# srvk/eesen

Measured on AMD Instinct MI355X. Metric: CTC training frames/sec (whole node), 4x512 BiLSTM, higher is better.
Workload: dtype f32

## Files before the change

eesen_amd/_lib.py:

```python
from __future__ import annotations

import ctypes as C
import os

_DIR = os.path.dirname(os.path.abspath(__file__))
LIB_PATH = os.environ.get("EESEN_HIP_LIBRARY") or os.path.join(_DIR, "lib", "libeesen_hip.so")

OK = 0
LAYER_AFFINE, LAYER_SOFTMAX, LAYER_LSTM_PARALLEL, LAYER_BILSTM_PARALLEL, LAYER_SIGMOID, LAYER_TANH = 1, 2, 3, 4, 5, 6
KIND_OF = {"AffineTransform": LAYER_AFFINE, "Softmax": LAYER_SOFTMAX, "LstmParallel": LAYER_LSTM_PARALLEL,
           "BiLstmParallel": LAYER_BILSTM_PARALLEL, "Lstm": LAYER_LSTM_PARALLEL, "BiLstm": LAYER_BILSTM_PARALLEL,
           "Sigmoid": LAYER_SIGMOID, "Tanh": LAYER_TANH}
NAME_OF = {LAYER_AFFINE: "AffineTransform", LAYER_SOFTMAX: "Softmax", LAYER_LSTM_PARALLEL: "LstmParallel",
           LAYER_BILSTM_PARALLEL: "BiLstmParallel", LAYER_SIGMOID: "Sigmoid", LAYER_TANH: "Tanh"}

_vp, _i, _f, _l = C.c_void_p, C.c_int, C.c_float, C.c_long
_pi, _pf, _pl, _pd = C.POINTER(C.c_int), C.POINTER(C.c_float), C.POINTER(C.c_long), C.POINTER(C.c_double)
SIGNATURES = {
    "eesen_last_error": (C.c_char_p, []),
    "eesen_version": (C.c_char_p, []),
    "eesen_device_count": (_i, [_pi]),
    "eesen_net_create": (_i, [_i, _vp, C.POINTER(_vp)]),
    "eesen_net_destroy": (_i, [_vp]),
    "eesen_net_add_layer": (_i, [_vp, _i, _i, _i, _f, _f]),
    "eesen_net_finalize": (_i, [_vp]),
    "eesen_net_read": (_i, [_vp, C.c_char_p]),
    "eesen_net_write": (_i, [_vp, C.c_char_p, _i]),
    "eesen_net_num_layers": (_i, [_vp, _pi]),
    "eesen_net_layer_info": (_i, [_vp, _i, _pi, _pi, _pi, _pf, _pf]),
    "eesen_net_input_dim": (_i, [_vp, _pi]),
    "eesen_net_output_dim": (_i, [_vp, _pi]),
    "eesen_net_num_params": (_i, [_vp, _pl]),
    "eesen_net_get_params": (_i, [_vp, _vp, _l]),
    "eesen_net_set_params": (_i, [_vp, _vp, _l]),
    "eesen_net_set_train_options": (_i, [_vp, _f, _f]),
    "eesen_net_set_update_algorithm": (_i, [_vp, C.c_char_p]),
    "eesen_net_set_adaptive_options": (_i, [_vp, _f, _f]),
    "eesen_net_get_accumulators": (_i, [_vp, _vp, _l]),
    "eesen_net_set_accumulators": (_i, [_vp, _vp, _l]),
    "eesen_net_set_seq_lengths": (_i, [_vp, _vp, _i]),
    "eesen_net_propagate": (_i, [_vp, _vp, _i, _i, _i, C.POINTER(_vp), _pi, _pi]),
    "eesen_net_get_output": (_i, [_vp, _vp, _l]),
    "eesen_net_backpropagate": (_i, [_vp, _vp, _i, _vp, _i]),
    "eesen_net_grad_buffer": (_i, [_vp, C.POINTER(_vp), _pl]),
    "eesen_net_get_grads": (_i, [_vp, _vp, _l]),
    "eesen_net_update": (_i, [_vp]),
    "eesen_net_set_forward_precision": (_i, [_vp, _i]),
    "eesen_net_bf16_recurrence_layers": (_i, [_vp, _vp]),
    "eesen_net_recurrence_info": (_i, [_vp, _pi]),
    "eesen_net_debug_set_error_word": (_i, [_vp, C.c_uint]),
    "eesen_net_synchronize": (_i, [_vp]),
    "eesen_net_set_profiling": (_i, [_vp, _i]),
    "eesen_net_get_phase_times": (_i, [_vp, _vp]),
    "eesen_net_get_phase_spans": (_i, [_vp, _pi, _pf, _i, _pi]),
    "eesen_device_synchronize": (_i, [_i]),
    "eesen_set_gemm_mode": (_i, [_i]),
    "eesen_get_gemm_mode": (_i, [_pi]),
    "eesen_comm_get_unique_id": (_i, [_vp]),
    "eesen_comm_exchange": (_i, [C.c_char_p, _i, _i, _i, _vp, _i, _i]),
    "eesen_comm_create": (_i, [_i, _vp, _i, _i, C.POINTER(_vp)]),
    "eesen_comm_create_tcp": (_i, [_i, C.c_char_p, _i, _i, _i, _i, C.POINTER(_vp)]),
    "eesen_comm_destroy": (_i, [_vp]),
    "eesen_comm_info": (_i, [_vp, _pi, _pi]),
    "eesen_comm_describe": (_i, [_vp, C.c_char_p, _i]),
    "eesen_net_plan_string": (_i, [_vp, C.c_char_p, _i]),
    "eesen_comm_allreduce_host": (_i, [_vp, _pd, _i, _i]),
    "eesen_net_set_comm": (_i, [_vp, _vp]),
    "eesen_net_allreduce_grads": (_i, [_vp, _vp]),
    "eesen_net_backpropagate_zero": (_i, [_vp]),
    "eesen_net_bucket_order": (_i, [_vp, _pi, _i, _pi]),
    "eesen_net_live_ranks": (_i, [_vp, _pi]),
    "eesen_net_layer_marker": (_i, [_vp, _i, C.c_char_p, _i]),
    "eesen_net_tensor_moments": (_i, [_vp, _i, _i, _pd, _i, _pi]),
    "eesen_ctc_set_guard": (_i, [_vp, _vp]),
    "eesen_ctc_dropped": (_i, [_vp, _pl]),
    "eesen_ctc_create": (_i, [_i, _vp, C.POINTER(_vp)]),
    "eesen_ctc_destroy": (_i, [_vp]),
    "eesen_ctc_eval_parallel": (_i, [_vp, _vp, _i, _vp, _i, _i, _i, _vp, _vp, _vp, _i, _vp]),
    "eesen_ctc_error_rate_mseq": (_i, [_vp, _vp, _i, _vp, _i, _i, _i, _vp, _vp, _pi, _pi]),
    "eesen_ctc_stats": (_i, [_vp, _pd, _pl, _pl, _pl, _pl]),
    "eesen_ctc_get_alpha_beta": (_i, [_vp, _vp, _vp, _pi]),
    "eesen_ctc_set_profiling": (_i, [_vp, _i]),
    "eesen_ctc_set_sequence_out_file": (_i, [_vp, C.c_char_p]),
    "eesen_ctc_get_phase_times": (_i, [_vp, _vp]),
    "eesen_ce_create": (_i, [_i, _vp, C.POINTER(_vp)]),
    "eesen_ce_destroy": (_i, [_vp]),
    "eesen_ce_eval_parallel": (_i, [_vp, _vp, _i, _vp, _i, _i, _i, _vp, _vp, _i, _vp]),
    "eesen_ce_set_report_step": (_i, [_vp, _i]),
    "eesen_ce_stats": (_i, [_vp, _pd, _pl, _pl, _pl]),
    "eesen_ce_report": (_i, [_vp, C.c_char_p, _i]),
    "eesen_ce_progress": (_i, [_vp, _i, C.c_char_p, _i]),
    "eesen_ce_set_guard": (_i, [_vp, _vp]),
    "eesen_ce_dropped": (_i, [_vp, _pl]),
    "eesen_ce_set_profiling": (_i, [_vp, _i]),
    "eesen_ce_get_phase_times": (_i, [_vp, _vp]),
    "eesen_net_set_train_mode": (_i, [_vp, _i]),
    "eesen_net_set_dropout_seed": (_i, [_vp, C.c_ulonglong]),
    "eesen_net_set_layer_dropout": (_i, [_vp, _i, _pf]),
    "eesen_net_get_layer_dropout": (_i, [_vp, _i, _pf]),
    "eesen_net_set_dropout_masks": (_i, [_vp, _i, _vp, _l, _vp, _i, _l, _i]),
    "eesen_net_get_dropout_masks": (_i, [_vp, _i, _vp, _vp, _pi]),
    "eesen_feeder_create": (_i, [_i, _vp, _i, C.POINTER(_vp)]),
    "eesen_feeder_destroy": (_i, [_vp]),
    "eesen_feeder_submit": (_i, [_vp, C.POINTER(_vp), _pi, _pi, _i, _i, _pi]),
    "eesen_feeder_acquire": (_i, [_vp, _i, C.POINTER(_vp), _pi, _pi, _pi]),
    "eesen_feeder_release": (_i, [_vp, _i]),
    "eesen_feeder_set_pipeline": (_i, [_vp, _vp, _i]),
    "eesen_feeder_pipeline_shape": (_i, [_vp, _i, _i, _pi, _pi]),
    "eesen_feeder_submit_raw": (_i, [_vp, C.POINTER(_vp), _pi, _pi, C.POINTER(_vp), _i, _i, _pi]),
    "eesen_cmvn_norm": (_i, [_pd, _i, _i, _i, _pf]),
    "eesen_dev_alloc": (_i, [_i, _l, C.POINTER(_vp)]),
    "eesen_dev_free": (_i, [_i, _vp]),
    "eesen_dev_copy": (_i, [_i, _vp, _vp, _l, _i]),
    "eesen_op_log_sub_prior": (_i, [_i, _vp, _vp, _i, _i, _i, _i, _vp, _f]),
    "eesen_op_amax_rows_cols": (_i, [_i, _vp, C.c_long, _i, _i, _vp, _vp]),
    "eesen_op_gemm_bench": (_i, [_i, _i, _i, _i, _i, _i, _vp, _i, _vp, _i, _vp, _i, _i, _pf]),
    "eesen_op_gemm": (_i, [_i, _vp, _i, _i, _i, _i, _i, _f, _vp, _i, _vp, _i, _f, _vp, _i, _vp]),
    "eesen_op_gemm_async": (_i, [_i, _vp, _i, _i, _i, _i, _i, _vp, _i, _vp, _i, _vp, _i, _vp, C.c_long, _i]),
}


class EesenError(RuntimeError):

    def __init__(self, code: int, msg: str):
        super().__init__(f"[{code}] {msg}")
        self.code = code


_lib = None


def load() -> C.CDLL:
    global _lib
    if _lib is None:
        if not os.path.exists(LIB_PATH):
            raise EesenError(-2, f"{LIB_PATH} is missing: build it with `python -m eesen_amd.build` "
                                 "(there is no CPU fallback for the HIP path)")
        os.environ.setdefault("HSA_ENABLE_IPC_MODE_LEGACY", "0")
        lib = C.CDLL(LIB_PATH)
        for name, (res, args) in SIGNATURES.items():
            fn = getattr(lib, name)
            fn.restype, fn.argtypes = res, args
        _lib = lib
    return _lib


def check(rc: int):
    if rc != OK:
        raise EesenError(rc, load().eesen_last_error().decode(errors="replace"))


def device_count() -> int:
    n = C.c_int(0)
    check(load().eesen_device_count(C.byref(n)))
    return n.value
```

eesen_amd/csrc/capi.cpp:

```cpp
#include <cstdio>
#include <cstring>

#include <algorithm>

#include "guard.h"
#include "net.h"

using namespace eesen;

#include "handles.h"

namespace eesen {
std::string& last_error_slot() {
  thread_local std::string g_err;
  return g_err;
}
}

extern "C" {

const char* eesen_last_error(void) { return last_error_slot().c_str(); }
const char* eesen_version(void) { return "eesen_hip 0.1.0 (gfx950)"; }

int eesen_device_count(int* count) {
// ... 291 lines not shown
    REQ_PTR(ce);
    ce->flush();
    if (obj) *obj = ce->obj;
    if (correct) *correct = ce->correct;
    if (frames) *frames = ce->frames;
    if (sequences) *sequences = ce->sequences;
  });
}
int eesen_ce_report(eesen_ce_t* ce, char* buf, int cap) {
  return guard([&] {
    REQ_PTR(ce); REQ_PTR(buf);
    const std::string s = ce->report();
    EESEN_REQUIRE(cap > (int)s.size(), EESEN_ERR_INVALID, "eesen_ce_report: buffer too small (" + std::to_string(s.size() + 1) + " bytes needed)");
    std::memcpy(buf, s.c_str(), s.size() + 1);
  });
}
int eesen_ce_progress(eesen_ce_t* ce, int wait, char* buf, int cap) {
  return guard([&] {
    REQ_PTR(ce); REQ_PTR(buf);
    EESEN_REQUIRE(cap > 0, EESEN_ERR_INVALID, "eesen_ce_progress: no buffer");
    if (wait) ce->flush();
    if (ce->progress.empty()) { buf[0] = 0; return; }
    const std::string& s = ce->progress.front();
    EESEN_REQUIRE(cap > (int)s.size(), EESEN_ERR_INVALID, "eesen_ce_progress: buffer too small (" + std::to_string(s.size() + 1) + " bytes needed)");
    std::memcpy(buf, s.c_str(), s.size() + 1);
    ce->progress.erase(ce->progress.begin());
  });
}
int eesen_ce_set_guard(eesen_ce_t* ce, eesen_net_t* net) {
  return guard([&] {
    REQ_PTR(ce);
    ce->flush();
    if (net) EESEN_REQUIRE(net->device == ce->device && net->st == ce->st, EESEN_ERR_INVALID, "eesen_ce_set_guard: the CE and the Net must live on the same device and stream");
    if (ce->guard_net) {
      auto& g = ce->guard_net->ce_guards;
      g.erase(std::remove(g.begin(), g.end(), static_cast<CeLoss*>(ce)), g.end());
    }
    ce->guard = net && net->ctl.p ? net->ctl.p + kCtlWords - 1 : nullptr;
    ce->guard_net = ce->guard ? net : nullptr;
    if (ce->guard_net) net->ce_guards.push_back(ce);
  });
}
int eesen_ce_dropped(eesen_ce_t* ce, long* minibatches) {
  return guard([&] { REQ_PTR(ce); REQ_PTR(minibatches); ce->flush(); *minibatches = ce->dropped; });
}
int eesen_ce_set_profiling(eesen_ce_t* ce, int mode) {
  return guard([&] { REQ_PTR(ce); ce->timer.enable(mode == 2); ce->timer.set_accumulate(mode == 2); });
}
int eesen_ce_get_phase_times(eesen_ce_t* ce, float* out1) {
  return guard([&] { REQ_PTR(ce); REQ_PTR(out1); ce->phase_times(out1); });
}

int eesen_dev_alloc(int device, long bytes, void** dev_ptr) {
  return guard([&] {
    REQ_PTR(dev_ptr);
    EESEN_HIP_CHECK(hipSetDevice(device));
    EESEN_HIP_CHECK(hipMalloc(dev_ptr, (size_t)bytes));
  });
}
int eesen_dev_free(int device, void* dev_ptr) {
  return guard([&] {
    EESEN_HIP_CHECK(hipSetDevice(device));
    EESEN_HIP_CHECK(hipFree(dev_ptr));
  });
}
int eesen_dev_copy(int device, void* dst, const void* src, long bytes, int kind) {
  return guard([&] {
    EESEN_HIP_CHECK(hipSetDevice(device));
    const hipMemcpyKind k = kind == 1 ? hipMemcpyHostToDevice : kind == 2 ? hipMemcpyDeviceToHost : hipMemcpyDeviceToDevice;
    EESEN_HIP_CHECK(hipMemcpy(dst, src, (size_t)bytes, k));
  });
}

int eesen_op_gemm(int device, void* stream, int a_kc, int b_kc, int M, int N, int K, float alpha, const float* A, int lda,
                  const float* B, int ldb, float beta, float* C, int ldc, const float* bias) {
  return guard([&] {
    EESEN_HIP_CHECK(hipSetDevice(device));
    hipStream_t st = reinterpret_cast<hipStream_t>(stream);
    DevBuf<float> ws;
    ws.reserve((size_t)8 << 20);
    gemm_f32(st, a_kc != 0, b_kc != 0, M, N, K, alpha, A, lda, B, ldb, beta, C, ldc, bias, ws.p, ws.cap);
    EESEN_HIP_CHECK(hipStreamSynchronize(st));
  });
}

int eesen_op_gemm_async(int device, void* stream, int a_kc, int b_kc, int M, int N, int K, const float* A, int lda, const float* B, int ldb,
                        float* C, int ldc, float* ws, long ws_floats, int extra_lds_bytes) {
  return guard([&] {
    REQ_PTR(A); REQ_PTR(B); REQ_PTR(C);
    EESEN_REQUIRE(ws_floats >= 0 && (ws || ws_floats == 0) && extra_lds_bytes >= 0, EESEN_ERR_INVALID, "bad workspace / LDS cap");
    EESEN_HIP_CHECK(hipSetDevice(device));
    gemm_f32(reinterpret_cast<hipStream_t>(stream), a_kc != 0, b_kc != 0, M, N, K, 1.f, A, lda, B, ldb, 0.f, C, ldc, nullptr, ws, (size_t)ws_floats,
             extra_lds_bytes);
  });
}

int eesen_op_log_sub_prior(int device, void* stream, float* m_dev, int rows, int cols, int ld, int apply_log,
                           const float* log_priors_host, float prior_scale) {
  return guard([&] {
    REQ_PTR(m_dev);
    EESEN_HIP_CHECK(hipSetDevice(device));
    hipStream_t st = reinterpret_cast<hipStream_t>(stream);
    DevBuf<float> pri;
    if (log_priors_host) {
      pri.reserve(cols);
      EESEN_HIP_CHECK(hipMemcpyAsync(pri.p, log_priors_host, sizeof(float) * cols, hipMemcpyHostToDevice, st));
    }
    log_sub_prior(st, m_dev, ld, rows, cols, apply_log != 0, log_priors_host ? pri.p : nullptr, prior_scale);
    EESEN_HIP_CHECK(hipStreamSynchronize(st));
  });
}

int eesen_op_gemm_bench(int device, int a_kc, int b_kc, int M, int N, int K, const float* A, int lda, const float* B, int ldb,
                        float* C, int ldc, int iters, float* avg_ms) {
  return guard([&] {
    REQ_PTR(avg_ms);
    EESEN_HIP_CHECK(hipSetDevice(device));
    DevBuf<float> ws;
    ws.reserve((size_t)16 << 20);
    hipEvent_t e0, e1;
    EESEN_HIP_CHECK(hipEventCreate(&e0));
    EESEN_HIP_CHECK(hipEventCreate(&e1));
    DevBuf<float> am;
    am.reserve((size_t)M + N + (size_t)kAmaxBlocks * 16384);
    GemmBound ba{am.p, 1}, bb{am.p + M, 1};
    float* aws = am.p + M + N;
    if (a_kc) amax_rows_cols(nullptr, A, M, K, lda, am.p, nullptr, nullptr); else amax_rows_cols(nullptr, A, K, M, lda, nullptr, am.p, aws);
    if (b_kc) amax_rows_cols(nullptr, B, N, K, ldb, am.p + M, nullptr, nullptr); else amax_rows_cols(nullptr, B, K, N, ldb, nullptr, am.p + M, aws);
    for (int i = 0; i < 2; ++i) gemm_f32(nullptr, a_kc != 0, b_kc != 0, M, N, K, 1.f, A, lda, B, ldb, 0.f, C, ldc, nullptr, ws.p, ws.cap, 0, false, ba, bb);
    EESEN_HIP_CHECK(hipEventRecord(e0, nullptr));
    for (int i = 0; i < iters; ++i) gemm_f32(nullptr, a_kc != 0, b_kc != 0, M, N, K, 1.f, A, lda, B, ldb, 0.f, C, ldc, nullptr, ws.p, ws.cap, 0, false, ba, bb);
    EESEN_HIP_CHECK(hipEventRecord(e1, nullptr));
    EESEN_HIP_CHECK(hipEventSynchronize(e1));
    float ms = 0.f;
    EESEN_HIP_CHECK(hipEventElapsedTime(&ms, e0, e1));
    *avg_ms = ms / iters;
    (void)hipEventDestroy(e0);
    (void)hipEventDestroy(e1);
  });
}

int eesen_op_amax_rows_cols(int device, const float* m_dev, long rows, int cols, int ld, float* out_rows_dev, float* out_cols_dev) {
  return guard([&] {
    REQ_PTR(m_dev);
    EESEN_REQUIRE(rows > 0 && cols > 0 && ld >= cols, EESEN_ERR_INVALID, "bad matrix shape");
    EESEN_HIP_CHECK(hipSetDevice(device));
    DevBuf<float> ws;
    if (out_cols_dev) ws.reserve((size_t)kAmaxBlocks * 16384);
    amax_rows_cols(nullptr, m_dev, rows, cols, ld, out_rows_dev, out_cols_dev, ws.p);
    EESEN_HIP_CHECK(hipStreamSynchronize(nullptr));
  });
}

}
```

eesen_amd/csrc/gemm.hip:

```cpp
#include <cstring>
#include <mutex>
#include <type_traits>

#include "kernels.h"

namespace eesen {
namespace {

constexpr int BM = 128, BN = 128, BK = 16, LDP = 4;
constexpr int NLD = BM * BK / 4 / 256;
constexpr int KQ_BITS = BK == 16 ? 2 : 3;
typedef float f32x16 __attribute__((ext_vector_type(16)));

struct GemmParams {
  const float* A;
  const float* B;
  float* C;
  const float* bias;
  int M, N, K;
  int lda, ldb, ldc;
  float alpha, beta;
  int splits;
  int k_chunk;
  int tiles_n;
// ... 615 lines not shown
    const long gw = (long)blockIdx.x * kAmaxWaves + wave, nw = (long)gridDim.x * kAmaxWaves;
    const int slab = (int)(gw % nslab);
    const int c0 = slab * 1024 + lane * 4;
    uint4 cm[4];
#pragma unroll
    for (int j = 0; j < 4; ++j) cm[j] = make_uint4(0u, 0u, 0u, 0u);
    const long rstep = nw / nslab;
    for (long r = gw / nslab; r < R; r += 2 * rstep) {
      const bool two = r + rstep < R;
      const float* row0 = P + r * ld;
      const float* row1 = P + (two ? r + rstep : r) * ld;
      uint4 v[8];
#pragma unroll
      for (int j = 0; j < 4; ++j) {
        const int c = c0 + 256 * j;
        v[j] = c < C ? *reinterpret_cast<const uint4*>(row0 + c) : make_uint4(0u, 0u, 0u, 0u);
        v[4 + j] = c < C ? *reinterpret_cast<const uint4*>(row1 + c) : make_uint4(0u, 0u, 0u, 0u);
      }
      unsigned m0 = 0u, m1 = 0u;
#pragma unroll
      for (int j = 0; j < 8; ++j) {
        v[j].x &= 0x7fffffffu; v[j].y &= 0x7fffffffu; v[j].z &= 0x7fffffffu; v[j].w &= 0x7fffffffu;
        const unsigned mj = max(max(v[j].x, v[j].y), max(v[j].z, v[j].w));
        if (j < 4) m0 = max(m0, mj); else m1 = max(m1, mj);
        if (COLS) { uint4& q = cm[j & 3]; q.x = max(q.x, v[j].x); q.y = max(q.y, v[j].y); q.z = max(q.z, v[j].z); q.w = max(q.w, v[j].w); }
      }
      if (ROWS || ALL) {
#pragma unroll
        for (int o = 32; o > 0; o >>= 1) { m0 = max(m0, (unsigned)__shfl_xor((int)m0, o)); m1 = max(m1, (unsigned)__shfl_xor((int)m1, o)); }
        if (ROWS && lane == 0) {
          if (nslab > 1 || row_acc) { atomicMax(&out_rows[r], m0); if (two) atomicMax(&out_rows[r + rstep], m1); }
          else { out_rows[r] = m0; if (two) out_rows[r + rstep] = m1; }
        }
        all = max(all, max(m0, m1));
      }
    }
    if (COLS) {
#pragma unroll
      for (int j = 0; j < 4; ++j) {
        const int c = c0 + 256 * j;
        if (c < C) { atomicMax(&smax[c], cm[j].x); atomicMax(&smax[c + 1], cm[j].y); atomicMax(&smax[c + 2], cm[j].z); atomicMax(&smax[c + 3], cm[j].w); }
      }
    }
  } else {
    for (long r = (long)blockIdx.x * kAmaxWaves + wave; r < R; r += (long)gridDim.x * kAmaxWaves) {
      const float* row = P + r * ld;
      unsigned m = 0u;
      for (int c = lane; c < C; c += 64) {
        const unsigned v = __builtin_bit_cast(unsigned, row[c]) & 0x7fffffffu;
        m = max(m, v);
        if (COLS) atomicMax(&smax[c], v);
      }
      if (ROWS || ALL) {
#pragma unroll
        for (int o = 32; o > 0; o >>= 1) m = max(m, (unsigned)__shfl_xor((int)m, o));
        if (ROWS && lane == 0) { if (row_acc) atomicMax(&out_rows[r], m); else out_rows[r] = m; }
        all = max(all, m);
      }
    }
  }
  if (COLS) {
    __syncthreads();
    for (int c = tid; c < Cp; c += kAmaxWaves * 64) part_cols[(size_t)blockIdx.x * Cp + c] = smax[c];
  }
  if (ALL) {
    unsigned* red = smax + (COLS ? Cp : 0);
    __syncthreads();
    if (lane == 0) red[wave] = all;
    __syncthreads();
    if (tid == 0) {
      unsigned m = 0u;
      for (int w = 0; w < kAmaxWaves; ++w) m = max(m, red[w]);
      if (m) atomicMax(out_all, m);
    }
  }
}
__global__ __launch_bounds__(256) void amax_fold_kernel(const unsigned* __restrict__ part, int nb, int Cp, int C, unsigned* __restrict__ out) {
  __shared__ uint4 red[16][16];
  const int cq = threadIdx.x & 15, g = threadIdx.x >> 4;
  const int c = blockIdx.x * 64 + cq * 4;
  uint4 m = make_uint4(0u, 0u, 0u, 0u);
  if (c < Cp)
    for (int b = g; b < nb; b += 16 * 8) {
      uint4 v[8];
#pragma unroll
      for (int k = 0; k < 8; ++k) v[k] = b + 16 * k < nb ? *reinterpret_cast<const uint4*>(part + (size_t)(b + 16 * k) * Cp + c) : make_uint4(0u, 0u, 0u, 0u);
#pragma unroll
      for (int k = 0; k < 8; ++k) { m.x = max(m.x, v[k].x); m.y = max(m.y, v[k].y); m.z = max(m.z, v[k].z); m.w = max(m.w, v[k].w); }
    }
  red[g][cq] = m;
  __syncthreads();
  if (g == 0 && c < Cp) {
#pragma unroll
    for (int k = 1; k < 16; ++k) { const uint4 o = red[k][cq]; m.x = max(m.x, o.x); m.y = max(m.y, o.y); m.z = max(m.z, o.z); m.w = max(m.w, o.w); }
    if (c + 0 < C) out[c + 0] = m.x;
    if (c + 1 < C) out[c + 1] = m.y;
    if (c + 2 < C) out[c + 2] = m.z;
    if (c + 3 < C) out[c + 3] = m.w;
  }
}

__global__ __launch_bounds__(256) void splitk_reduce_kernel(const float* __restrict__ ws, int splits, int M, int N,
                                                            float alpha, float beta, float* __restrict__ C, int ldc,
                                                            const float* __restrict__ bias) {
  const size_t total = (size_t)M * N;
  for (size_t i = (size_t)blockIdx.x * blockDim.x + threadIdx.x; i < total; i += (size_t)gridDim.x * blockDim.x) {
    float s = 0.f;
    for (int k = 0; k < splits; ++k) s += ws[(size_t)k * total + i];
    const int row = (int)(i / N), col = (int)(i % N);
    float v = alpha * s + (bias ? bias[col] : 0.f);
    float* dst = C + (size_t)row * ldc + col;
    if (beta != 0.f) v += beta * *dst;
    *dst = v;
  }
}

}

static int g_gemm_mode = -1;
int gemm_mode() {
  if (g_gemm_mode >= 0) return g_gemm_mode;
  const char* e = getenv("EESEN_GEMM_MODE");
  if (e && (!strcmp(e, "f32") || !strcmp(e, "0"))) return 0;
  if (e && (!strcmp(e, "split") || !strcmp(e, "1"))) return 1;
  if (e && (!strcmp(e, "half") || !strcmp(e, "2"))) return 2;
  return kDefaultGemmMode;
}
void set_gemm_mode(int mode) { g_gemm_mode = mode; }

void amax_abs(hipStream_t st, const float* P, long rows, int cols, int ld, float* out) {
  EESEN_HIP_CHECK(hipMemsetAsync(out, 0, sizeof(float), st));
  amax_abs_accumulate(st, P, rows, cols, ld, out);
}
static int amax_blocks(long rows, int slabs) { return (int)std::max<long>(1, std::min<long>((rows * slabs + 2 * kAmaxWaves - 1) / (2 * kAmaxWaves), kAmaxBlocks)); }
#define EESEN_AMAX_LAUNCH(R_, C_, A_, LDS)                                                                                                        \
  do {                                                                                                                                            \
    if (vec) hipLaunchKernelGGL((amax_kernel<R_, C_, A_, true>), dim3(nb), dim3(kAmaxWaves * 64), LDS, st, Pc, rows, cc, ld, r, w, a, racc);     \
    else hipLaunchKernelGGL((amax_kernel<R_, C_, A_, false>), dim3(nb), dim3(kAmaxWaves * 64), LDS, st, Pc, rows, cc, ld, r, w, a, racc);        \
  } while (0)
constexpr int kAmaxSlabCols = 16384;
void amax_abs_accumulate(hipStream_t st, const float* P, long rows, int cols, int ld, float* out) {
  if (rows <= 0 || cols <= 0) return;
  if (cols == ld && cols < 1024 && (rows * cols) % 1024 == 0) { rows = rows * cols / 1024; cols = ld = 1024; }
  unsigned *r = nullptr, *w = nullptr, *a = reinterpret_cast<unsigned*>(out);
  const int racc = 0;
  const bool vec = (cols & 3) == 0 && (ld & 3) == 0;
  for (int c0 = 0; c0 < cols; c0 += kAmaxSlabCols) {
    const float* Pc = P + c0;
    const int cc = std::min(kAmaxSlabCols, cols - c0), nb = amax_blocks(rows, vec ? (cc + 1023) / 1024 : 1);
    EESEN_AMAX_LAUNCH(false, false, true, kAmaxWaves * sizeof(unsigned));
  }
  check_launch("amax_abs");
}
void amax_rows_cols(hipStream_t st, const float* P, long rows, int cols, int ld, float* out_rows, float* out_cols, float* ws) {
  if (rows <= 0 || cols <= 0) return;
  EESEN_REQUIRE(!out_cols || ws, EESEN_ERR_INVALID, "amax: column bounds need a workspace");
  unsigned* r = reinterpret_cast<unsigned*>(out_rows);
  unsigned* w = reinterpret_cast<unsigned*>(ws);
  unsigned* a = nullptr;
  const bool vec = (cols & 3) == 0 && (ld & 3) == 0;
  const bool multi = out_rows && ((vec && cols > 1024) || cols > kAmaxSlabCols);
  if (multi) EESEN_HIP_CHECK(hipMemsetAsync(out_rows, 0, (size_t)rows * sizeof(float), st));
  for (int c0 = 0; c0 < cols; c0 += kAmaxSlabCols) {
    const float* Pc = P + c0;
    const int cc = std::min(kAmaxSlabCols, cols - c0), racc = multi ? 1 : 0;
    const int nb = amax_blocks(rows, vec ? (cc + 1023) / 1024 : 1);
    const int cp = (cc + 3) & ~3;
    if (out_rows && out_cols) EESEN_AMAX_LAUNCH(true, true, false, (size_t)cp * sizeof(unsigned));
    else if (out_cols) EESEN_AMAX_LAUNCH(false, true, false, (size_t)cp * sizeof(unsigned));
    else if (out_rows) EESEN_AMAX_LAUNCH(true, false, false, 0);
    check_launch("amax_rows_cols");
    if (out_cols) {
      hipLaunchKernelGGL(amax_fold_kernel, dim3((cp + 63) / 64), dim3(256), 0, st, w, nb, cp, cc, reinterpret_cast<unsigned*>(out_cols) + c0);
      check_launch("amax_fold");
    }
  }
}
#undef EESEN_AMAX_LAUNCH

static GemmBound arena_bound(hipStream_t st, const float* P, bool kc, int R, int K, int ld) {
  constexpr size_t kArena = (size_t)4 << 20, kDevs = 16;
  static std::mutex mu;
  static float* arena[kDevs] = {nullptr};
  static size_t next[kDevs] = {0};
  int dev = 0;
  EESEN_HIP_CHECK(hipGetDevice(&dev));
  EESEN_REQUIRE(dev >= 0 && dev < (int)kDevs, EESEN_ERR_INVALID, "gemm: device index beyond the bounds arena table");
  const size_t need = ((size_t)R + 3) & ~(size_t)3;
  EESEN_REQUIRE(need <= kArena / 8, EESEN_ERR_INVALID, "gemm: operand too large for the bounds arena");
  float* slot;
  {
    std::lock_guard<std::mutex> lk(mu);
    if (!arena[dev]) EESEN_HIP_CHECK(hipMalloc(reinterpret_cast<void**>(&arena[dev]), kArena * sizeof(float)));
    if (next[dev] + need > kArena) next[dev] = 0;
    slot = arena[dev] + next[dev];
    next[dev] += need;
  }
  if (kc) amax_rows_cols(st, P, R, K, ld, slot, nullptr, nullptr);
  else {
    float* ws = nullptr;
    EESEN_HIP_CHECK(hipMallocAsync(reinterpret_cast<void**>(&ws), (size_t)kAmaxBlocks * std::min<size_t>(need, kAmaxSlabCols) * sizeof(float), st));
    amax_rows_cols(st, P, K, R, ld, nullptr, slot, ws);
    EESEN_HIP_CHECK(hipFreeAsync(ws, st));
  }
  return GemmBound{slot, 1};
}

static int xcd_group_rows(int tiles_m, int tiles_n, unsigned* grid_x) {
  if (tiles_m < 8) return 0;
  int gm = 8;
  while (gm > 1 && cdiv(tiles_m, gm) < 16) gm >>= 1;
  const long groups = cdiv(tiles_m, gm), rounds = cdivl(groups, 8);
  const long gx = rounds * 8 * gm * tiles_n;
  if (gx > 0x7fffffffL) return 0;
  *grid_x = (unsigned)gx;
  return gm;
}

void gemm_f32(hipStream_t st, bool a_kc, bool b_kc, int M, int N, int K, float alpha, const float* A, int lda,
              const float* B, int ldb, float beta, float* C, int ldc, const float* bias, float* ws, size_t ws_floats,
              int extra_lds_bytes, bool bf16_operands, GemmBound bound_a, GemmBound bound_b) {
  if (M <= 0 || N <= 0) return;
  EESEN_REQUIRE((lda % 4) == 0 && (ldb % 4) == 0, EESEN_ERR_INVALID, "gemm: leading dimensions must be multiples of 4");
  EESEN_REQUIRE((((uintptr_t)A | (uintptr_t)B) & 15) == 0, EESEN_ERR_INVALID, "gemm: operands must be 16-byte aligned");
  const bool use_split = gemm_mode() >= 1 || bf16_operands;
  const bool half = gemm_mode() == 2 && !bf16_operands;
  GemmParams p;
  p.amax_a = p.amax_b = nullptr;
  p.a_vec = p.b_vec = 0;
  if (half) {
    if (!bound_a.p) bound_a = arena_bound(st, A, a_kc, M, K, lda);
    if (!bound_b.p) bound_b = arena_bound(st, B, b_kc, N, K, ldb);
    p.amax_a = bound_a.p; p.a_vec = bound_a.per_index;
    p.amax_b = bound_b.p; p.b_vec = bound_b.per_index;
  }
  p.A = A; p.B = B; p.C = C; p.bias = bias;
  p.M = M; p.N = N; p.K = K; p.lda = lda; p.ldb = ldb; p.ldc = ldc;
  p.alpha = alpha; p.beta = beta;
  p.gate = GemmGate{nullptr, nullptr, 0, 0, 0, 0, 0, 0};
  p.nprod = bf16_operands ? 1 : 6;
  const bool big = use_split && !bf16_operands && extra_lds_bytes == 0 && M % 256 == 0 && N % 256 == 0 && K % 16 == 0 &&
                   (long)(M / 256) * (N / 256) >= 16;
  const int TB = big ? 256 : BM;
  p.bm = p.bn = TB;
  const int tiles_m = cdiv(M, TB), tiles_n = cdiv(N, TB);
  p.tiles_n = tiles_n;
  p.tiles_m = tiles_m;
  const long tiles = (long)tiles_m * tiles_n;
  int splits = 1;
  const int target = big ? 256 : 1024;
  if (ws && tiles < target && K >= 2048) {
    splits = (int)std::min<long>((target + tiles - 1) / tiles, K / 1024);
    splits = std::max(1, std::min(splits, 64));
    while (splits > 1 && (size_t)splits * M * N > ws_floats) --splits;
  }
  int k_chunk = cdiv(cdiv(K, splits), 16) * 16;
  if (k_chunk < BK) k_chunk = BK;
  splits = std::max(1, cdiv(K, k_chunk));
  p.splits = splits;
  p.k_chunk = k_chunk;
  if (splits > 1) p.C = ws;
  unsigned gx = 0;
  p.gm = xcd_group_rows(tiles_m, tiles_n, &gx);
  dim3 grid(p.gm ? gx : (unsigned)tiles, (unsigned)splits), block(big ? 512 : 256);
  const bool guard = (M % BM) != 0 || (N % BN) != 0 || (K % k_chunk) != 0 || (k_chunk % BK) != 0 || !(a_kc && b_kc);
#define EESEN_GEMM_LAUNCH(AK, BKC)                                                                        \
  do {                                                                                                    \
    if (guard) hipLaunchKernelGGL((gemm_f32_mfma_kernel<AK, BKC, true>), grid, block, extra_lds_bytes, st, p); \
    else hipLaunchKernelGGL((gemm_f32_mfma_kernel<AK, BKC, false>), grid, block, extra_lds_bytes, st, p);     \
  } while (0)
  if (big && half) {
    if (a_kc && b_kc) hipLaunchKernelGGL((gemm_f32_split_f16_big_kernel<true, true>), grid, block, 0, st, p);
    else if (a_kc && !b_kc) hipLaunchKernelGGL((gemm_f32_split_f16_big_kernel<true, false>), grid, block, 0, st, p);
    else if (!a_kc && b_kc) hipLaunchKernelGGL((gemm_f32_split_f16_big_kernel<false, true>), grid, block, 0, st, p);
    else hipLaunchKernelGGL((gemm_f32_split_f16_big_kernel<false, false>), grid, block, 0, st, p);
  } else if (big) {
    if (a_kc && b_kc) hipLaunchKernelGGL((gemm_f32_split_bf16_big_kernel<true, true>), grid, block, 0, st, p);
    else if (a_kc && !b_kc) hipLaunchKernelGGL((gemm_f32_split_bf16_big_kernel<true, false>), grid, block, 0, st, p);
    else if (!a_kc && b_kc) hipLaunchKernelGGL((gemm_f32_split_bf16_big_kernel<false, true>), grid, block, 0, st, p);
    else hipLaunchKernelGGL((gemm_f32_split_bf16_big_kernel<false, false>), grid, block, 0, st, p);
  } else if (use_split) {
    const int extra = extra_lds_bytes > 0 ? std::max(0, extra_lds_bytes + 33792 - 2 * (half ? GeoSmallH::STAGE : GeoSmall::STAGE)) : 0;
    const bool sg = (M % BM) != 0 || (N % BN) != 0 || (K % k_chunk) != 0 || (k_chunk % 16) != 0;
#define EESEN_SPLIT_LAUNCH(AK, BKC)                                                                                   \
  do {                                                                                                                \
    if (half && sg) hipLaunchKernelGGL((gemm_f32_split_f16_kernel<AK, BKC, true>), grid, block, extra, st, p);        \
    else if (half) hipLaunchKernelGGL((gemm_f32_split_f16_kernel<AK, BKC, false>), grid, block, extra, st, p);        \
    else if (sg) hipLaunchKernelGGL((gemm_f32_split_bf16_kernel<AK, BKC, true>), grid, block, extra, st, p);          \
    else hipLaunchKernelGGL((gemm_f32_split_bf16_kernel<AK, BKC, false>), grid, block, extra, st, p);                 \
  } while (0)
    if (a_kc && b_kc) EESEN_SPLIT_LAUNCH(true, true);
    else if (a_kc && !b_kc) EESEN_SPLIT_LAUNCH(true, false);
    else if (!a_kc && b_kc) EESEN_SPLIT_LAUNCH(false, true);
    else EESEN_SPLIT_LAUNCH(false, false);
#undef EESEN_SPLIT_LAUNCH
  } else if (a_kc && b_kc) EESEN_GEMM_LAUNCH(true, true);
  else if (a_kc && !b_kc) EESEN_GEMM_LAUNCH(true, false);
  else if (!a_kc && b_kc) EESEN_GEMM_LAUNCH(false, true);
  else EESEN_GEMM_LAUNCH(false, false);
#undef EESEN_GEMM_LAUNCH
  check_launch("gemm_f32_mfma");
  if (splits > 1) {
    const size_t total = (size_t)M * N;
    const int blocks = (int)std::min<size_t>((total + 255) / 256, 2048);
    hipLaunchKernelGGL(splitk_reduce_kernel, dim3(blocks), dim3(256), 0, st, (const float*)ws, splits, M, N, alpha, beta,
                       C, ldc, bias);
    check_launch("splitk_reduce");
  }
}

void gemm_f32_nt_gated(hipStream_t st, int M, int N, int K, const float* A, int lda, const float* B, int ldb, float* C,
                       int ldc, const float* bias, const GemmGate& gate, GemmBound bound_a, GemmBound bound_b) {
  EESEN_REQUIRE((M % BM) == 0 && (N % BN) == 0 && (K % BK) == 0, EESEN_ERR_INVALID, "gated GEMM needs whole tiles");
  EESEN_REQUIRE(gate.ndir * gate.nz * kShards <= 64, EESEN_ERR_INVALID, "gated GEMM: too many counter groups");
  GemmParams p;
// ... 20 lines not shown
```

eesen_amd/csrc/kernels.h:

```cpp
#pragma once
#include "common.h"

namespace eesen {

struct GemmBound {
  const float* p = nullptr;
  int per_index = 0;
};
void gemm_f32(hipStream_t st, bool a_kc, bool b_kc, int M, int N, int K, float alpha, const float* A, int lda,
              const float* B, int ldb, float beta, float* C, int ldc, const float* bias, float* ws,
              size_t ws_floats, int extra_lds_bytes = 0,
              bool bf16_operands = false,
              GemmBound bound_a = {}, GemmBound bound_b = {});

constexpr int kDefaultGemmMode = 2;
int gemm_mode();
void set_gemm_mode(int mode);
void amax_abs(hipStream_t st, const float* P, long rows, int cols, int ld, float* out);
void amax_abs_accumulate(hipStream_t st, const float* P, long rows, int cols, int ld, float* out);
constexpr int kAmaxBlocks = 512;
void amax_rows_cols(hipStream_t st, const float* P, long rows, int cols, int ld, float* out_rows, float* out_cols, float* ws);

#ifndef EESEN_SHARDS
#define EESEN_SHARDS 8
#endif
constexpr int kShards = EESEN_SHARDS, kShardStride = 32;
constexpr int kCtlHalf = 2048 * kShards;

struct GemmGate {
  const unsigned* cnt;
  unsigned* err;
  int ndir, nz, nblk;
  int T, S;
  int spin_limit;
};
void gemm_f32_nt_gated(hipStream_t st, int M, int N, int K, const float* A, int lda, const float* B, int ldb, float* C,
                       int ldc, const float* bias, const GemmGate& gate, GemmBound bound_a = {}, GemmBound bound_b = {});

struct LstmLayerDev {
  int T, S, H, ndir;
  float* G;
  float* C;
  float* Y;
  float* X = nullptr;
  const float* Wm;
  const float* WmT;
  const float* peep;
  const int* lens;
  const float* rmask = nullptr;
  int drop_mode = 0;
  int s_begin = 0, s_count = 0;
  float* PX = nullptr;
  size_t px_floats = 0;
  int poll_delay = 0;
  int poll_raw = 0;
  unsigned* milestone = nullptr;
  int milestone_step = 0;
  int xcd_map = 1, fwd_mux = 1, bwd_q4 = 1, bwd_ksplit = 1, bwd_mux = 1;
  int fwd_t16_small = 1;
  int fwd_narrow2 = 1;
  int bwd_q4_st8 = 1;
  int fwd_bf16 = 0;
  int fwd_split = 0;
  int fwd_f16 = 0;
  const float* wm_amax = nullptr;
  int bwd_f16 = 0;
  unsigned char* DGH = nullptr;
  float* EX = nullptr;
};
float handoff_flight_ns();
void set_gpu_share(int n);
int gpu_share_value();
void wait_for_word(hipStream_t st, const unsigned* word, unsigned target, unsigned* err, double limit_s = 2.0);
void lstm_fwd_step(hipStream_t st, const LstmLayerDev& L, int step);
void lstm_bwd_step(hipStream_t st, const LstmLayerDev& L, int step, const float* dY, int lddy, float* DG, float* DCF);
void dropout_mask(hipStream_t st, float* out, long rows, int cols, int ld, float p, unsigned long long seed, bool per_column);
void activation_rows(hipStream_t st, bool tanh_, const float* x, int ldx, float* y, int ldy, long rows, int cols);
void activation_diff_rows(hipStream_t st, bool tanh_, const float* y, int ldy, float* d, int ldd, long rows, int cols);
void mul_elements(hipStream_t st, const float* a, int lda, const float* m, int ldm, float* out, int ldo, long rows, int cols);
enum { kRecNone = 0, kRecFwdBf = 1, kRecFwdMux = 2, kRecFwdF32 = 3, kRecBwdQ4 = 4, kRecBwdKsplit = 5, kRecBwdKsplitMux = 6, kRecBwdGeneric = 7 };
struct RecPlan {
  int kind = kRecNone;
  const char* kernel = "";
  int seq_tile = 0;
  int units = 0;
  int windows = 0;
  int grid[3] = {0, 0, 0};
  int wgs = 0;
  int wgs_per_cu = 0;
  int vgprs = 0, lds = 0;
  int free_vgprs = -1;
  int seq_tiles = 1;
  bool one_window = false;
  bool leaves_room = false;
  bool bf16 = false;
  bool light = false;
  size_t need_px = 0, need_ex = 0;
  bool need_dgh = false;
  size_t ctl_words = 0;
  int chunk = 0;
  const void* fn = nullptr;
};
RecPlan lstm_fwd_plan(const LstmLayerDev& L);
RecPlan lstm_bwd_plan(const LstmLayerDev& L);
void lstm_fwd_launch(hipStream_t st, const RecPlan& plan, const LstmLayerDev& L, unsigned* cnt, unsigned* err, int spin_limit,
                     unsigned long long* trace = nullptr, hipEvent_t after_reset = nullptr);
void lstm_bwd_launch(hipStream_t st, const RecPlan& plan, const LstmLayerDev& L, const float* dY, int lddy, float* DG, unsigned* cnt,
                     unsigned* err, int spin_limit, unsigned long long* trace = nullptr);
void lstm_bias_peep_grads(hipStream_t st, const LstmLayerDev& L, const float* DG, float* bias_grad, float* peep_grad,
                          float* ws, size_t ws_floats);
size_t lstm_bias_peep_ws_floats(int T, int S, int H, int ndir);

void col_sums(hipStream_t st, const float* M, int rows, int cols, int ld, float* out, float* ws, size_t ws_floats);
size_t col_sums_ws_floats(int rows, int cols);

void softmax_rows(hipStream_t st, const float* x, int ldx, float* y, int ldy, int rows, int K);
void log_rows(hipStream_t st, const float* in, int ldi, float* out, int ldo, int rows, int K);
void ctc_alpha_beta(hipStream_t st, const float* logp, int ld, int T, int S, int Lpad, const int* labx, const int* lens,
                    const int* lablens, float* alpha, float* beta, float* pzx, int waves = 0);
int ctc_sweep_waves(int Lpad, int waves = 0);
void ctc_error_diff(hipStream_t st, const float* probs, int ld, int T, int S, int K, int Lpad, int Lmax, const int* lens,
                    const int* lablens, const int* labx, const float* alpha, const float* beta,
                    const float* pzx, float* diff, int ldd);
void log_sub_prior(hipStream_t st, float* m, int ld, int rows, int K, bool apply_log, const float* log_prior, float prior_scale);
void row_argmax(hipStream_t st, const float* m, int ld, int rows, int K, int* ids);

struct CeSums {
  double obj;
  long long correct;
};
int ce_eval_blocks(int rows);
void ce_eval(hipStream_t st, const float* y, int ld, int rows, int K, int S, const int* lens, const int* tgt, float* diff,
             int ldd, CeSums* part, CeSums* out);

void sgd_update(hipStream_t st, float* param, float* corr, const float* fresh, long n, float mmt, float lr_coef,
                float max_grad, const unsigned* skip = nullptr, const float* live = nullptr);
void zero_if_set(hipStream_t st, float* p, long n, const unsigned* word);
void adaptive_update(hipStream_t st, float* param, float* corr, const float* fresh, float* accu, long n, float mmt, float lr,
                     float max_grad, float eps, float rho, float one_minus_rho, bool rmsprop, const unsigned* skip = nullptr,
                     const float* live = nullptr);
void tensor_moments(hipStream_t st, const float* base, long rows, int cols, long ld, double* out6, double* ws,
                    int nb = 0, int hf = 0, int hi = 0);
void transpose2d(hipStream_t st, const float* src, int rows, int cols, float* dst);
void copy2d(hipStream_t st, const float* src, int lds, float* dst, int ldd, int rows, int cols);

}
```

eesen_amd/csrc/net.cpp:

```cpp
#include "net.h"

#include <algorithm>
#include <cmath>
#include <cstdio>
#include <cstring>

namespace eesen {


PhaseTimer::~PhaseTimer() {
  for (auto& s : spans_) {
    (void)hipEventDestroy(s.a);
    (void)hipEventDestroy(s.b);
  }
}
int PhaseTimer::begin(hipStream_t st, int phase) {
  if (!on_) return -1;
  if (used_ == spans_.size()) {
    Span s;
    EESEN_HIP_CHECK(hipEventCreate(&s.a));
    EESEN_HIP_CHECK(hipEventCreate(&s.b));
    spans_.push_back(s);
  }
  spans_[used_].phase = phase;
  EESEN_HIP_CHECK(hipEventRecord(spans_[used_].a, st));
  return (int)used_++;
}
void PhaseTimer::end(hipStream_t st, int idx) {
  if (!on_ || idx < 0) return;
  EESEN_HIP_CHECK(hipEventRecord(spans_[idx].b, st));
}
void PhaseTimer::collect(float* out, int nphase) {
  for (int i = 0; i < nphase; ++i) out[i] = 0.f;
  for (size_t i = 0; i < used_; ++i) {
    EESEN_HIP_CHECK(hipEventSynchronize(spans_[i].b));
    float ms = 0.f;
    EESEN_HIP_CHECK(hipEventElapsedTime(&ms, spans_[i].a, spans_[i].b));
    if (spans_[i].phase >= 0 && spans_[i].phase < nphase) out[spans_[i].phase] += ms * 1e-3f;
  }
  if (accumulate_) used_ = 0;
}

int PhaseTimer::spans(int* phases, float* secs, int cap) {
  for (size_t i = 0; i < used_ && (int)i < cap; ++i) {
    EESEN_HIP_CHECK(hipEventSynchronize(spans_[i].b));
    float ms = 0.f;
    EESEN_HIP_CHECK(hipEventElapsedTime(&ms, spans_[i].a, spans_[i].b));
    if (phases) phases[i] = spans_[i].phase;
    if (secs) secs[i] = ms * 1e-3f;
  }
  return (int)used_;
}

long Layer::file_params() const {
  if (is_lstm()) return (long)ndir * ((long)4 * Hf * din_f + (long)4 * Hf * Hf + 4 * Hf + 3 * Hf);
  if (kind == EESEN_LAYER_AFFINE) return (long)dout_f * din_f + dout_f;
  return 0;
}

const char* Layer::marker() const {
  switch (kind) {
    case EESEN_LAYER_BILSTM_PARALLEL: return nonparallel ? "<BiLstm>" : "<BiLstmParallel>";
    case EESEN_LAYER_LSTM_PARALLEL: return nonparallel ? "<Lstm>" : "<LstmParallel>";
    case EESEN_LAYER_AFFINE: return "<AffineTransform>";
    case EESEN_LAYER_SOFTMAX: return "<Softmax>";
    case EESEN_LAYER_SIGMOID: return "<Sigmoid>";
    case EESEN_LAYER_TANH: return "<Tanh>";
  }
  return "<Unknown>";
}

template <class F>
static void for_each_param(const Layer& L, F f) {
  long fi = 0;
  if (L.is_lstm()) {
    const int H = L.H, Hf = L.Hf, D = L.din_f, D4 = pad4(L.din);
    for (int dir = 0; dir < L.ndir; ++dir) {
      for (int r = 0; r < 4 * Hf; ++r) {
        const int q = r / Hf, u = r % Hf;
        for (int d = 0; d < D; ++d) f(fi++, L.off_wx + ((size_t)dir * 4 * H + u * 4 + q) * D4 + L.in_col(d));
      }
      for (int r = 0; r < 4 * Hf; ++r) {
        const int q = r / Hf, u = r % Hf;
        for (int k = 0; k < Hf; ++k) f(fi++, L.off_wm + ((size_t)dir * 4 * H + u * 4 + q) * H + k);
      }
      for (int r = 0; r < 4 * Hf; ++r) f(fi++, L.off_bias + (size_t)dir * 4 * H + (r % Hf) * 4 + r / Hf);
      for (int g = 0; g < 3; ++g)
        for (int u = 0; u < Hf; ++u) f(fi++, L.off_peep + ((size_t)dir * 3 + g) * H + u);
    }
  } else if (L.kind == EESEN_LAYER_AFFINE) {
    const int D4 = pad4(L.din);
    for (int r = 0; r < L.dout; ++r)
      for (int d = 0; d < L.din_f; ++d) f(fi++, L.off_w + (size_t)r * D4 + L.in_col(d));
    for (int r = 0; r < L.dout; ++r) f(fi++, L.off_b + r);
  }
}

Net::Net(int dev, void* stream) : device(dev) {
  int n = 0;
  hipError_t e = hipGetDeviceCount(&n);
  if (e != hipSuccess || n <= 0)
    throw Error(EESEN_ERR_HIP, "no HIP device available: this library has no CPU fallback (hipGetDeviceCount: " +
                                   std::string(e == hipSuccess ? "0 devices" : hipGetErrorString(e)) + ")");
  EESEN_REQUIRE(dev >= 0 && dev < n, EESEN_ERR_INVALID, "device index out of range");
  EESEN_HIP_CHECK(hipSetDevice(dev));
  st = reinterpret_cast<hipStream_t>(stream);
  int lo = 0, hi = 0;
  EESEN_HIP_CHECK(hipDeviceGetStreamPriorityRange(&lo, &hi));
  EESEN_HIP_CHECK(hipStreamCreateWithPriority(&st2, hipStreamNonBlocking, lo));
  EESEN_HIP_CHECK(hipEventCreateWithFlags(&ev_rec, hipEventDisableTiming));
  for (auto& e : ev_grad) EESEN_HIP_CHECK(hipEventCreateWithFlags(&e, hipEventDisableTiming));
  EESEN_HIP_CHECK(hipEventCreateWithFlags(&ev_gate_reset, hipEventDisableTiming));
  EESEN_HIP_CHECK(hipEventCreateWithFlags(&ev_gate_done, hipEventDisableTiming));
  tn = Tuning::from_env();
  persistent = tn.persistent;
  gate_fwd = tn.gate_fwd >= 0 ? tn.gate_fwd != 0 : gemm_mode() == 0;
  overlap = tn.overlap >= 0 ? tn.overlap != 0 : persistent != 0;
  spin_limit = tn.spin_limit;
  if (tn.trace) {
    trace.reserve(1280);
    EESEN_HIP_CHECK(hipMemset(trace.p, 0, 1280 * sizeof(unsigned long long)));
  }
  ctl.reserve(kCtlWords);
  EESEN_HIP_CHECK(hipMemset(ctl.p, 0, kCtlWords * sizeof(unsigned)));
  {
    constexpr float kFwdNs = 400.f, kBwdNs = 280.f, kBwdSideNs = 420.f, kRefFlightNs = 400.f;
    flight_ns = handoff_flight_ns();
    const float fscale = flight_ns >= 300.f && flight_ns <= 700.f ? 1.f : flight_ns / kRefFlightNs;
    auto ticks = [&](float ns) { return std::min(300, std::max(0, (int)std::lround(fscale * ns / 10.f))); };
    delay_fwd = ticks(kFwdNs); delay_bwd = ticks(kBwdNs); delay_bwd_side = ticks(kBwdSideNs);
    if (const char* e = tn.poll_ns) {
      int a = -1, b2 = -1;
      if (sscanf(e, "%d,%d", &a, &b2) == 2) { delay_fwd = a / 10; delay_bwd = delay_bwd_side = b2 / 10; poll_raw = 1; }
    }
    if (tn.print_flight)
      fprintf(stderr, "eesen_hip: increment flight %.0f ns; first-poll delays forward %d0, backward %d0 (beside side-stream GEMMs %d0) ns\n", flight_ns, delay_fwd, delay_bwd, delay_bwd_side);
  }
}

Net::~Net() {
  (void)hipSetDevice(device);
  (void)hipStreamSynchronize(st);
  for (Ctc* c : guards) {
    (void)hipStreamSynchronize(c->st);
    c->guard = nullptr;
    c->guard_net = nullptr;
  }
  for (CeLoss* c : ce_guards) {
    (void)hipStreamSynchronize(c->st);
    c->guard = nullptr;
    c->guard_net = nullptr;
  }
  if (trace.p) {
    std::vector<unsigned long long> h(1280);
    if (hipMemcpy(h.data(), trace.p, h.size() * 8, hipMemcpyDeviceToHost) == hipSuccess)
      for (int pass = 0; pass < 2; ++pass) {
        double seg[5] = {0, 0, 0, 0, 0};
        int n = 0;
        for (int s = 8; s < 120; ++s) {
          const unsigned long long* a = h.data() + pass * 640 + s * 5;
          if (!a[0] || !a[5]) continue;
          seg[0] += (double)(a[1] - a[0]); seg[1] += (double)(a[2] - a[1]); seg[2] += (double)(a[3] - a[2]);
          seg[3] += (double)(a[4] - a[3]); seg[4] += (double)(a[5] - a[4]);
          ++n;
        }
        if (n) fprintf(stderr, "EESEN_TRACE %s: wait %.0f | A-load+MFMA+reduce %.0f | epilogue %.0f | drain+barrier %.0f | publish->next %.0f ticks/step (%d steps)\n",
                       pass ? "bwd" : "fwd", seg[0] / n, seg[1] / n, seg[2] / n, seg[3] / n, seg[4] / n, n);
      }
  }
  if (lens_pin) (void)hipHostFree(lens_pin);
  if (err_pin) (void)hipHostFree(err_pin);
  if (live_pin) (void)hipHostFree(live_pin);
  for (auto& h : in_stage) { if (h.p) (void)hipHostFree(h.p); if (h.ev) (void)hipEventDestroy(h.ev); }
  if (lens_ev) (void)hipEventDestroy(lens_ev);
  if (err_ev) (void)hipEventDestroy(err_ev);
  if (st2) { (void)hipStreamSynchronize(st2); (void)hipStreamDestroy(st2); }
  if (ev_rec) (void)hipEventDestroy(ev_rec);
  for (auto& e : ev_grad) if (e) (void)hipEventDestroy(e);
  if (ev_gate_reset) (void)hipEventDestroy(ev_gate_reset);
  if (ev_gate_done) (void)hipEventDestroy(ev_gate_done);
  for (auto& e : ev_ready) if (e) (void)hipEventDestroy(e);
  for (auto& e : ev_bucket) if (e) (void)hipEventDestroy(e);
  if (ev_bwd_done) (void)hipEventDestroy(ev_bwd_done);
  if (own_stream) (void)hipStreamDestroy(st);
}

void Net::sync() {
  EESEN_HIP_CHECK(hipSetDevice(device));
  EESEN_HIP_CHECK(hipStreamSynchronize(st));
  wait_buckets_host();
  comm_check_alive(comm);
  check_device_error(true);
}

void Net::check_device_error(bool consumer) {
  if (!ctl.p) return;
  unsigned e = 0;
  EESEN_HIP_CHECK(hipMemcpy(&e, ctl.p + kCtlWords - 1, sizeof(unsigned), hipMemcpyDeviceToHost));
  if (!e) { steps_since_clean = 0; return; }
  EESEN_HIP_CHECK(hipStreamSynchronize(st));
  EESEN_HIP_CHECK(hipMemset(ctl.p + kCtlWords - 1, 0, sizeof(unsigned)));
  const bool only_waiter = e == 2 && tn.fwd_mid;
  if (only_waiter) tn.fwd_mid = 0;
  else { persistent = 0; gate_fwd = false; overlap = false; }
  ++recoveries;
  const int lost = std::max(1, steps_since_clean);
  steps_since_clean = 0;
  const bool rerun = consumer && propagated && input.p && rows > 0;
  const char* what = comm ? "contributed a ZERO gradient to the data-parallel sum (the ranks' models stay identical)" : "were NOT applied";
  if (only_waiter)
    fprintf(stderr, "WARNING (eesen_hip) the side stream's wait for a forward-recurrence milestone gave up (kernels serialised by a tool?): "
                    "%d minibatch(es) in flight %s%s; continuing without the early input GEMM (EESEN_FWD_MID=0)\n", lost, what,
            rerun ? " and the last forward pass is re-run" : "");
  else
    fprintf(stderr, "WARNING (eesen_hip) a persistent recurrence kernel gave up waiting for a peer workgroup (GPU shared or preempted?): "
                    "%d minibatch(es) in flight %s%s; continuing with the one-launch-per-step kernels\n", lost, what,
            rerun ? " and the last forward pass is re-run" : "");
  if (rerun) {
    forward_pass();
    EESEN_HIP_CHECK(hipStreamSynchronize(st));
  }
}

void Net::arm_device_error_poll() {
  if (!ctl.p) return;
  if (!err_pin) {
    EESEN_HIP_CHECK(hipHostMalloc(reinterpret_cast<void**>(&err_pin), sizeof(unsigned), hipHostMallocDefault));
    *err_pin = 0;
    EESEN_HIP_CHECK(hipEventCreateWithFlags(&err_ev, hipEventDisableTiming));
  }
  EESEN_HIP_CHECK(hipMemcpyAsync(err_pin, ctl.p + kCtlWords - 1, sizeof(unsigned), hipMemcpyDeviceToHost, st));
  EESEN_HIP_CHECK(hipEventRecord(err_ev, st));
  err_armed = true;
}

void Net::poll_device_error() {
  if (!err_armed || hipEventQuery(err_ev) != hipSuccess) return;
  err_armed = false;
  if (*err_pin) check_device_error(false);
  else steps_since_clean = 0;
}

void Net::add_layer(int kind, int din, int dout, float coef, float max_grad) {
  EESEN_REQUIRE(!finalized, EESEN_ERR_STATE, "net already finalized");
  EESEN_REQUIRE(din > 0 && dout > 0, EESEN_ERR_INVALID, "layer dimensions must be positive");
  const Layer* prev = layers.empty() ? nullptr : &layers.back();
  if (prev)
    EESEN_REQUIRE(prev->dout_f == din, EESEN_ERR_INVALID, "Dimensionality mismatch between consecutive layers");
  Layer L;
  L.kind = kind; L.coef = coef; L.max_grad = max_grad;
  L.din_f = din; L.dout_f = dout;
  L.din = prev ? prev->dout : din;
  if (prev) { L.in_nb = prev->out_nb; L.in_hf = prev->out_hf; L.in_hi = prev->out_hi; }
  L.dout = dout;
  const char* sees_pad = "directly on an LSTM layer whose cell count per direction is not a multiple of 4 is not supported: it would see the "
                         "zero cells the library pads such a layer with";
  switch (kind) {
    case EESEN_LAYER_BILSTM_PARALLEL:
      EESEN_REQUIRE(dout % 2 == 0, EESEN_ERR_INVALID, "<CellDim> of a BiLstm layer must be even");
      L.ndir = 2; L.Hf = dout / 2;
      break;
    case EESEN_LAYER_LSTM_PARALLEL:
      L.ndir = 1; L.Hf = dout;
      break;
    case EESEN_LAYER_AFFINE:
      break;
    case EESEN_LAYER_SOFTMAX:
      EESEN_REQUIRE(din == dout, EESEN_ERR_INVALID, "Softmax needs InputDim == OutputDim");
      if (L.in_nb) throw Error(EESEN_ERR_INVALID, std::string("a <Softmax> ") + sees_pad);
      break;
    case EESEN_LAYER_SIGMOID:
    case EESEN_LAYER_TANH:
      EESEN_REQUIRE(din == dout, EESEN_ERR_INVALID, "an activation layer needs InputDim == OutputDim");
      if (L.in_nb && kind == EESEN_LAYER_SIGMOID) throw Error(EESEN_ERR_INVALID, std::string("a <Sigmoid> ") + sees_pad + " (sigmoid(0) = 1/2)");
      L.dout = L.din;
      L.out_nb = L.in_nb; L.out_hf = L.in_hf; L.out_hi = L.in_hi;
      break;
    default:
      throw Error(EESEN_ERR_INVALID, "unsupported layer kind " + std::to_string(kind));
  }
  if (L.is_lstm()) {
    L.H = pad4(L.Hf);
    L.dout = L.ndir * L.H;
    if (L.H != L.Hf) { L.out_nb = L.ndir; L.out_hf = L.Hf; L.out_hi = L.H; }
  }
  layers.push_back(std::move(L));
}

void Net::finalize() {
  EESEN_REQUIRE(!finalized, EESEN_ERR_STATE, "net already finalized");
  EESEN_REQUIRE(!layers.empty(), EESEN_ERR_INVALID, "empty net");
  EESEN_HIP_CHECK(hipSetDevice(device));
  size_t off = 0;
  for (Layer& L : layers) {
    L.p_off = off;
    size_t n = 0;
    if (L.is_lstm()) {
      const size_t H = L.H, D4 = pad4(L.din), nd = L.ndir;
      L.off_wx = n;   n += nd * 4 * H * D4;
      L.off_bias = n; n += nd * 4 * H;
      L.off_wm = n;   n += nd * 4 * H * H;
      L.off_peep = n; n += nd * 3 * H;
      L.WmT.reserve(nd * H * 4 * H);
    } else if (L.kind == EESEN_LAYER_AFFINE) {
      L.off_w = n; n += (size_t)L.dout * pad4(L.din);
      L.off_b = n; n += pad4(L.dout);
    }
    L.p_n = (n + 3) & ~(size_t)3;
    off += L.p_n;
  }
  P = off;
  if (P) {
    params.reserve(P); corr.reserve(P); fresh.reserve(P + kLiveWords);
    EESEN_HIP_CHECK(hipMemsetAsync(params.p, 0, P * sizeof(float), st));
    EESEN_HIP_CHECK(hipMemsetAsync(corr.p, 0, P * sizeof(float), st));
    EESEN_HIP_CHECK(hipMemsetAsync(fresh.p, 0, (P + kLiveWords) * sizeof(float), st));
  }
  if (tn.overlap < 0)
    for (const Layer& L : layers)
      if (L.is_lstm() && L.H > 512) overlap = false;
  amax.reserve(1 + layers.size());
  EESEN_HIP_CHECK(hipMemsetAsync(amax.p, 0, amax.cap * sizeof(float), st));
  EESEN_HIP_CHECK(hipMemsetD32Async(reinterpret_cast<hipDeviceptr_t>(amax.p), 0x3f800000, 1, st));
  finalized = true;
  refresh_derived();
  sync();
}

void Net::measure(const float* Pm, long nrows, int cols, int ld, DevBuf<float>& out_rows, DevBuf<float>& out_cols) {
  out_rows.reserve((size_t)nrows);
  out_cols.reserve((size_t)cols);
  amax_ws.reserve((size_t)kAmaxBlocks * std::min(16384, (cols + 3) & ~3));
  amax_rows_cols(st, Pm, nrows, cols, ld, out_rows.p, out_cols.p, amax_ws.p);
}
bool Net::x_is_bounded(int li) const {
  if (li == 0) return false;
  const Layer& Pv = layers[li - 1];
  return (Pv.is_lstm() && !Pv.cur_fwd_drop) || Pv.is_activation() || Pv.kind == EESEN_LAYER_SOFTMAX;
}
void Net::ensure_weight_amax() {
  const bool mode2 = gemm_mode() == 2;
  const bool need_w = mode2 && !wamax_valid;
  if (wm_valid && !need_w) return;
  if (!wm_valid) EESEN_HIP_CHECK(hipMemsetAsync(am_wm(0), 0, layers.size() * sizeof(float), st));
  for (size_t li = 0; li < layers.size(); ++li) {
    Layer& L = layers[li];
    if (L.is_lstm()) {
      if (need_w) measure(params.p + L.p_off + L.off_wx, (long)L.ndir * 4 * L.H, pad4(L.din), pad4(L.din), L.bw.rows, L.bw.cols);
      if (!wm_valid) amax_abs_accumulate(st, params.p + L.p_off + L.off_wm, (long)L.ndir * 4 * L.H, L.H, L.H, am_wm((int)li));
    } else if (L.kind == EESEN_LAYER_AFFINE && need_w) measure(params.p + L.p_off + L.off_w, L.dout, pad4(L.din), pad4(L.din), L.bw.rows, L.bw.cols);
  }
  wm_valid = true;
  if (mode2) wamax_valid = true;
}

long Net::num_params() const {
  long n = 0;
  for (const Layer& L : layers) n += L.file_params();
  return n;
}

void Net::init_accu() {
  if (accu_init) return;
  accu.reserve(P);
  EESEN_HIP_CHECK(hipMemsetAsync(accu.p, 0, P * sizeof(float), st));
  accu_init = true;
}

void Net::refresh_derived() {
  wamax_valid = wm_valid = false;
  for (Layer& L : layers)
    if (L.is_lstm())
      for (int dir = 0; dir < L.ndir; ++dir)
        transpose2d(st, params.p + L.p_off + L.off_wm + (size_t)dir * 4 * L.H * L.H, 4 * L.H, L.H,
                    L.WmT.p + (size_t)dir * L.H * 4 * L.H);
}

int Net::tensor_moments(int which, int layer, double* out6_host, int cap_tensors) {
  EESEN_REQUIRE(finalized, EESEN_ERR_STATE, "net not finalized");
  EESEN_REQUIRE(layer >= 0 && layer < (int)layers.size(), EESEN_ERR_INVALID, "layer index out of range");
  EESEN_REQUIRE(which >= 0 && which <= 2, EESEN_ERR_INVALID, "which: 0 parameters, 1 momentum buffers, 2 accumulators");
  const Layer& L = layers[layer];
  struct Region { size_t off; long rows; int cols; long ld; int nb, hf, hi; };
  std::vector<Region> reg;
  if (L.is_lstm()) {
    const int H = L.H, Hf = L.Hf, D4 = pad4(L.din);
    for (int dir = 0; dir < L.ndir; ++dir) {
      reg.push_back({L.off_wx + (size_t)dir * 4 * H * D4, 4L * Hf, L.din_f, D4, L.in_nb, L.in_hf, L.in_hi});
      reg.push_back({L.off_wm + (size_t)dir * 4 * H * H, 4L * Hf, Hf, H, 0, 0, 0});
      reg.push_back({L.off_bias + (size_t)dir * 4 * H, 1, 4 * Hf, 4L * H, 0, 0, 0});
      for (int g = 0; g < 3; ++g) reg.push_back({L.off_peep + ((size_t)dir * 3 + g) * H, 1, Hf, H, 0, 0, 0});
    }
  } else if (L.kind == EESEN_LAYER_AFFINE) {
    reg.push_back({L.off_w, L.dout, L.din_f, pad4(L.din), L.in_nb, L.in_hf, L.in_hi});
    reg.push_back({L.off_b, 1, L.dout, L.dout, 0, 0, 0});
  }
  const int n = (int)reg.size();
  if (!out6_host || n == 0) return n;
  EESEN_REQUIRE(cap_tensors >= n, EESEN_ERR_INVALID, "moments buffer too small");
  EESEN_HIP_CHECK(hipSetDevice(device));
  if (which == 2) init_accu();
  sync();
  const float* base = (which == 0 ? params.p : which == 1 ? corr.p : accu.p) + L.p_off;
  DevBuf<double> d;
  d.reserve((size_t)n * 6 + 8);
  for (int i = 0; i < n; ++i)
    eesen::tensor_moments(st, base + reg[i].off, reg[i].rows, reg[i].cols, reg[i].ld, d.p + (size_t)i * 6, d.p + (size_t)n * 6, reg[i].nb, reg[i].hf, reg[i].hi);
  EESEN_HIP_CHECK(hipStreamSynchronize(st));
  EESEN_HIP_CHECK(hipMemcpy(out6_host, d.p, (size_t)n * 6 * sizeof(double), hipMemcpyDeviceToHost));
  return n;
}

static void upload_flat(Net& net, DevBuf<float>& dst, const float* host, long n) {
  EESEN_REQUIRE(net.finalized, EESEN_ERR_STATE, "net not finalized");
  EESEN_REQUIRE(n == net.num_params(), EESEN_ERR_INVALID, "parameter count mismatch");
  EESEN_HIP_CHECK(hipSetDevice(net.device));
  std::vector<float> h(net.P, 0.f);
  long base = 0;
  for (const Layer& L : net.layers) {
    for_each_param(L, [&](long fi, size_t io) { h[L.p_off + io] = host[base + fi]; });
    base += L.file_params();
  }
  net.sync();
  if (net.P) EESEN_HIP_CHECK(hipMemcpy(dst.p, h.data(), net.P * sizeof(float), hipMemcpyHostToDevice));
}

void Net::set_params(const float* host, long n) {
  upload_flat(*this, params, host, n);
  refresh_derived();
  sync();
}

void Net::set_accu(const float* host, long n) {
  init_accu();
  upload_flat(*this, accu, host, n);
}

void Net::get_flat(const DevBuf<float>& buf, float* host, long n) {
  EESEN_REQUIRE(finalized, EESEN_ERR_STATE, "net not finalized");
  EESEN_REQUIRE(n == num_params(), EESEN_ERR_INVALID, "parameter count mismatch");
  sync();
  std::vector<float> h(P);
  if (P) EESEN_HIP_CHECK(hipMemcpy(h.data(), buf.p, P * sizeof(float), hipMemcpyDeviceToHost));
  long base = 0;
  for (const Layer& L : layers) {
    for_each_param(L, [&](long fi, size_t io) { host[base + fi] = h[L.p_off + io]; });
    base += L.file_params();
  }
}

void Net::set_seq_lengths(const int* l, int s) {
  EESEN_REQUIRE(s > 0, EESEN_ERR_INVALID, "need at least one sequence");
  EESEN_HIP_CHECK(hipSetDevice(device));
  lens.assign(l, l + s);
  for (int v : lens) EESEN_REQUIRE(v >= 0, EESEN_ERR_INVALID, "negative sequence length");
  poll_device_error();
  lens_d.reserve(s);
  if ((size_t)s > lens_pin_cap) {
    if (lens_pin) { EESEN_HIP_CHECK(hipStreamSynchronize(st)); EESEN_HIP_CHECK(hipHostFree(lens_pin)); }
    lens_pin = nullptr;
    lens_pin_cap = std::max<size_t>(64, (size_t)s * 2);
    EESEN_HIP_CHECK(hipHostMalloc(reinterpret_cast<void**>(&lens_pin), lens_pin_cap * sizeof(int), hipHostMallocDefault));
  }
  if (!lens_ev) EESEN_HIP_CHECK(hipEventCreateWithFlags(&lens_ev, hipEventDisableTiming));
  else EESEN_HIP_CHECK(hipEventSynchronize(lens_ev));
  std::copy(lens.begin(), lens.end(), lens_pin);
  EESEN_HIP_CHECK(hipMemcpyAsync(lens_d.p, lens_pin, s * sizeof(int), hipMemcpyHostToDevice, st));
  EESEN_HIP_CHECK(hipEventRecord(lens_ev, st));
  S = s;
  propagated = false;
}

static LstmLayerDev lstm_view(const Net& net, const Layer& L, int T) {
  LstmLayerDev d;
  d.T = T; d.S = net.S; d.H = L.H; d.ndir = L.ndir;
  d.G = L.G.p; d.C = L.C.p; d.Y = L.Y.p;
  d.X = L.X.p;
  d.Wm = net.params.p + L.p_off + L.off_wm;
  d.WmT = L.WmT.p;
  d.peep = net.params.p + L.p_off + L.off_peep;
  d.lens = net.lens_d.p;
  d.rmask = L.cur_drop_mode ? L.rmask.p : nullptr;
  d.drop_mode = L.cur_drop_mode;
  d.fwd_bf16 = net.fwd_bf16_rec ? 1 : 0;
  d.fwd_split = net.tn.fwd_split;
  d.fwd_f16 = net.tn.fwd_f16 && net.tn.fwd_split;
  d.bwd_f16 = net.tn.bwd_f16 && net.tn.fwd_split;
  d.wm_amax = net.amax.p ? const_cast<Net&>(net).am_wm((int)(&L - net.layers.data())) : nullptr;
  d.xcd_map = net.tn.xcd_map; d.fwd_mux = net.tn.fwd_mux; d.bwd_q4 = net.tn.bwd_q4; d.bwd_q4_st8 = net.tn.bwd_q4_st8; d.fwd_narrow2 = net.tn.fwd_narrow2; d.fwd_t16_small = net.tn.fwd_t16_small; d.bwd_ksplit = net.tn.bwd_ksplit; d.bwd_mux = net.tn.bwd_mux;
  return d;
}

void Net::set_layer_dropout(int layer, const float* nine) {
  EESEN_REQUIRE(layer >= 0 && layer < (int)layers.size(), EESEN_ERR_INVALID, "layer index out of range");
  Layer& L = layers[layer];
  bool any = false;
  for (int k = 0; k < 9; ++k) any |= nine[k] != 0.f;
  EESEN_REQUIRE(!any || L.kind == EESEN_LAYER_BILSTM_PARALLEL, EESEN_ERR_INVALID, "dropout options exist on BiLstm layers only");
  EESEN_REQUIRE(nine[0] >= 0.f && nine[0] < 1.f && nine[7] >= 0.f && nine[7] < 1.f, EESEN_ERR_INVALID, "dropout factor outside [0, 1)");
  for (int k = 0; k < 9; ++k) L.drop[k] = (k == 0 || k == 7) ? nine[k] : (nine[k] != 0.f ? 1.f : 0.f);
}

void Net::get_layer_dropout(int layer, float* nine) const {
  EESEN_REQUIRE(layer >= 0 && layer < (int)layers.size(), EESEN_ERR_INVALID, "layer index out of range");
  for (int k = 0; k < 9; ++k) nine[k] = layers[layer].drop[k];
}

static void widen_mask(const Layer& L, const float* src, long n, std::vector<float>& dst, const char* what) {
  dst.clear();
  if (!src) return;
  const long wf = (long)L.ndir * L.Hf, wi = (long)L.ndir * L.H;
  EESEN_REQUIRE(n > 0 && n % wf == 0, EESEN_ERR_INVALID, std::string(what) + ": the float count is not a multiple of the layer's ndir * H columns");
  if (wf == wi) { dst.assign(src, src + n); return; }
  const long rows = n / wf;
  dst.assign((size_t)rows * wi, 0.f);
  for (long r = 0; r < rows; ++r)
    for (int d = 0; d < L.ndir; ++d)
      std::copy(src + r * wf + (long)d * L.Hf, src + r * wf + (long)(d + 1) * L.Hf, dst.begin() + r * wi + (long)d * L.H);
}

void Net::set_dropout_masks(int layer, const float* fwd, long fwd_n, const float* rec, int rec_rows, long rec_n, int coin) {
  EESEN_REQUIRE(layer >= 0 && layer < (int)layers.size() && layers[layer].is_lstm(), EESEN_ERR_INVALID, "not an LSTM layer");
  Layer& L = layers[layer];
  if (rec) EESEN_REQUIRE(rec_rows > 0 && rec_n == (long)rec_rows * L.ndir * L.Hf, EESEN_ERR_INVALID, "recurrent mask: rec_floats must be rec_rows x ndir * H");
  widen_mask(L, fwd, fwd ? fwd_n : 0, L.inj_fmask, "forward mask");
  widen_mask(L, rec, rec ? rec_n : 0, L.inj_rmask, "recurrent mask");
  L.inj_rmask_rows = rec ? rec_rows : 0;
  L.inj_coin = coin;
}

void Net::get_dropout_masks(int layer, float* fwd_host, float* rec_host, int* info4) {
  EESEN_REQUIRE(layer >= 0 && layer < (int)layers.size() && layers[layer].is_lstm(), EESEN_ERR_INVALID, "not an LSTM layer");
  EESEN_REQUIRE(propagated, EESEN_ERR_STATE, "no Propagate yet");
  Layer& L = layers[layer];
  EESEN_HIP_CHECK(hipSetDevice(device));
  sync();
  const size_t ldY = (size_t)L.ndir * L.H, wf = (size_t)L.ndir * L.Hf;
  auto fetch = [&](float* host, const float* dev, size_t nrows) {
    if (wf == ldY) { EESEN_HIP_CHECK(hipMemcpy(host, dev, nrows * ldY * sizeof(float), hipMemcpyDeviceToHost)); return; }
    std::vector<float> tmp(nrows * ldY);
    EESEN_HIP_CHECK(hipMemcpy(tmp.data(), dev, tmp.size() * sizeof(float), hipMemcpyDeviceToHost));
    for (size_t r = 0; r < nrows; ++r)
      for (int d = 0; d < L.ndir; ++d)
        std::copy(tmp.begin() + r * ldY + (size_t)d * L.H, tmp.begin() + r * ldY + (size_t)d * L.H + L.Hf, host + r * wf + (size_t)d * L.Hf);
  };
  if (fwd_host && L.cur_fwd_drop) fetch(fwd_host, L.fmask.p, (size_t)rows);
  if (rec_host && L.cur_drop_mode) fetch(rec_host, L.rmask.p, (size_t)(T + 2) * S);
  if (info4) { info4[0] = L.cur_fwd_drop; info4[1] = L.cur_drop_mode; info4[2] = L.cur_twiddle_coin; info4[3] = (int)wf; }
}

static void prepare_dropout(Net& net, Layer& L) {
  L.cur_fwd_drop = false; L.cur_drop_mode = 0; L.cur_twiddle_coin = false;
  const bool want = net.in_train && L.has_dropout();
  if (!want) { L.inj_fmask.clear(); L.inj_rmask.clear(); L.inj_rmask_rows = 0; L.inj_coin = -1; return; }
  const float fwd_p = L.drop[0], rec_p = L.drop[7];
  const bool fw_seq = L.drop[2] != 0.f, rec_step = L.drop[3] != 0.f, rec_seq = L.drop[4] != 0.f;
  const bool rnndrop = L.drop[5] != 0.f, nml = L.drop[6] != 0.f, twiddle = L.drop[8] != 0.f;
  const int T = net.T, S = net.S, ldY = L.ndir * L.H;
  bool coin = false;
  if (twiddle) {
    if (L.inj_coin >= 0) coin = L.inj_coin != 0;
    else {
      unsigned long long z = net.drop_seed + (++net.drop_counter) * 0x9E3779B97F4A7C15ull;
      z = (z ^ (z >> 30)) * 0xBF58476D1CE4E5B9ull; z = (z ^ (z >> 27)) * 0x94D049BB133111EBull; z ^= z >> 31;
      coin = (z >> 63) != 0;
    }
  }
  L.cur_twiddle_coin = coin;
  const bool rec = (rnndrop || nml) && (!twiddle || !coin);
  const bool fwd = fwd_p > 0.f && (!twiddle || coin);
  if (rec) {
    EESEN_REQUIRE(rec_step != rec_seq, EESEN_ERR_INVALID,
                  "recurrent dropout needs exactly one of RecurrentTimeStepDropout / RecurrentSequenceDropout (bilstm-layer.h:102-113)");
    EESEN_REQUIRE(!(rnndrop && nml), EESEN_ERR_INVALID, "RNNDrop and NoMemLossDropout are mutually exclusive");
    const long mrows = (long)(T + 2) * S;
    L.rmask.reserve((size_t)mrows * ldY);
    if (!L.inj_rmask.empty()) {
      EESEN_REQUIRE((L.inj_rmask_rows == mrows || L.inj_rmask_rows == S) && (long)L.inj_rmask.size() == (long)L.inj_rmask_rows * ldY,
                    EESEN_ERR_INVALID, "injected recurrent mask has the wrong shape");
      const size_t chunk = (size_t)L.inj_rmask_rows * ldY;
      for (long r0 = 0; r0 < mrows; r0 += L.inj_rmask_rows)
        EESEN_HIP_CHECK(hipMemcpyAsync(L.rmask.p + (size_t)r0 * ldY, L.inj_rmask.data(), chunk * sizeof(float), hipMemcpyHostToDevice, net.st));
      EESEN_HIP_CHECK(hipStreamSynchronize(net.st));
    } else {
      dropout_mask(net.st, L.rmask.p, mrows, ldY, ldY, rec_p, net.drop_seed + (++net.drop_counter) * 0x632BE59BD9B4E019ull, rec_seq);
    }
    L.cur_drop_mode = rnndrop ? 2 : 1;
  }
  if (fwd) {
    L.fmask.reserve((size_t)net.rows * ldY);
    L.Yd.reserve((size_t)net.rows * ldY);
    if (!L.inj_fmask.empty()) {
      EESEN_REQUIRE((long)L.inj_fmask.size() == (long)net.rows * ldY, EESEN_ERR_INVALID, "injected forward mask has the wrong shape");
      EESEN_HIP_CHECK(hipMemcpyAsync(L.fmask.p, L.inj_fmask.data(), L.inj_fmask.size() * sizeof(float), hipMemcpyHostToDevice, net.st));
      EESEN_HIP_CHECK(hipStreamSynchronize(net.st));
    } else {
      dropout_mask(net.st, L.fmask.p, net.rows, ldY, ldY, fwd_p, net.drop_seed + (++net.drop_counter) * 0x632BE59BD9B4E019ull, fw_seq);
    }
    L.cur_fwd_drop = true;
  }
  L.inj_fmask.clear(); L.inj_rmask.clear(); L.inj_rmask_rows = 0; L.inj_coin = -1;
}

void Net::propagate(const float* in, int nrows, int ld, bool is_device) {
  EESEN_REQUIRE(finalized, EESEN_ERR_STATE, "net not finalized");
  EESEN_REQUIRE(S > 0, EESEN_ERR_STATE, "SetSeqLengths must precede Propagate");
  EESEN_REQUIRE(nrows > 0 && nrows % S == 0, EESEN_ERR_INVALID, "row count must be a positive multiple of the sequence count");
  const int D = layers[0].din, D4 = pad4(D);
  EESEN_REQUIRE(ld >= D, EESEN_ERR_INVALID, "input leading dimension smaller than InputDim");
  EESEN_HIP_CHECK(hipSetDevice(device));
  rows = nrows;
  T = rows / S;
  for (int v : lens) EESEN_REQUIRE(v <= T, EESEN_ERR_INVALID, "sequence length exceeds the number of frames");
  timer.reset();

  if (input.reserve((size_t)rows * D4) || D4 != D) EESEN_HIP_CHECK(hipMemsetAsync(input.p, 0, (size_t)rows * D4 * sizeof(float), st));
  if (is_device) {
    EESEN_HIP_CHECK(hipMemcpy2DAsync(input.p, (size_t)D4 * sizeof(float), in, (size_t)ld * sizeof(float), (size_t)D * sizeof(float), rows,
                                     hipMemcpyDeviceToDevice, st));
  } else {
    HostStage& hs = in_stage[in_stage_idx++ & 1];
    const size_t bytes = (size_t)rows * D * sizeof(float);
    if (!hs.ev) EESEN_HIP_CHECK(hipEventCreateWithFlags(&hs.ev, hipEventDisableTiming));
    if (hs.busy) { EESEN_HIP_CHECK(hipEventSynchronize(hs.ev)); hs.busy = false; }
    if (bytes > hs.cap) {
      if (hs.p) EESEN_HIP_CHECK(hipHostFree(hs.p));
      hs.p = nullptr;
      hs.cap = bytes + bytes / 4;
      EESEN_HIP_CHECK(hipHostMalloc(reinterpret_cast<void**>(&hs.p), hs.cap, hipHostMallocDefault));
    }
    for (int r = 0; r < rows; ++r) std::memcpy(hs.p + (size_t)r * D, in + (size_t)r * ld, (size_t)D * sizeof(float));
    EESEN_HIP_CHECK(hipMemcpy2DAsync(input.p, (size_t)D4 * sizeof(float), hs.p, (size_t)D * sizeof(float), (size_t)D * sizeof(float), rows,
                                     hipMemcpyHostToDevice, st));
    EESEN_HIP_CHECK(hipEventRecord(hs.ev, st));
    hs.busy = true;
  }
  forward_pass();
}

void Net::forward_pass() {
  const float* x = input.p;
  int ldx = pad4(layers[0].din);
  ++steps_since_clean;
  info_fwd_persistent = info_lstm_layers = info_fwd_bf16 = 0;
  bool g_gated = false;
  int gated_rows = 0;
  int mid_r0 = 0, mid_r1 = 0;
  const bool half = gemm_mode() == 2;
  ensure_weight_amax();
  amx_valid = half;
  for (Layer& L : layers) {
    const int li_ = (int)(&L - layers.data());
    GemmBound x_amax, w_amax;
    if (half && L.trainable()) {
      if (x_is_bounded(li_)) x_amax = bound_one();
      else { measure(x, rows, L.din, ldx, L.bx.rows, L.bx.cols); x_amax = GemmBound{L.bx.rows.p, 1}; }
      w_amax = GemmBound{L.bw.rows.p, 1};
    }
    if (L.is_lstm()) {
      const int H = L.H, nd = L.ndir, ldY = nd * H, ldG = nd * 4 * H;
      L.G.reserve((size_t)rows * ldG);
      const size_t state = (size_t)(T + 2) * S * ldY;
      L.C.reserve(state);
      L.Y.reserve(state);
      if (persistent && H % 32 == 0) L.X.reserve((size_t)T * nd * ((S + 15) / 16) * (size_t)(H / 32) * 768);
      const size_t blk = (size_t)S * ldY * sizeof(float);
      EESEN_HIP_CHECK(hipMemsetAsync(L.C.p, 0, blk, st));
      EESEN_HIP_CHECK(hipMemsetAsync(L.Y.p, 0, blk, st));
      EESEN_HIP_CHECK(hipMemsetAsync(L.C.p + (size_t)(T + 1) * S * ldY, 0, blk, st));
      EESEN_HIP_CHECK(hipMemsetAsync(L.Y.p + (size_t)(T + 1) * S * ldY, 0, blk, st));
      prepare_dropout(*this, L);
      if (g_gated) {
        if (gated_rows < rows) {
          const int ti_ = timer.begin(st, 0);
          gemm_f32(st, true, true, rows - gated_rows, ldG, L.din, 1.f, x + (size_t)gated_rows * ldx, ldx, params.p + L.p_off + L.off_wx,
                   pad4(L.din), 0.f, L.G.p + (size_t)gated_rows * ldG, ldG, params.p + L.p_off + L.off_bias, nullptr, 0, 0, fwd_bf16, x_amax, w_amax);
          timer.end(st, ti_);
        }
        EESEN_HIP_CHECK(hipStreamWaitEvent(st, ev_gate_done, 0));
        g_gated = false;
      } else if (mid_r1 > mid_r0) {
        const int ti_ = timer.begin(st, 0);
        const int parts[2][2] = {{0, mid_r0}, {mid_r1, rows}};
        for (const auto& pr : parts)
          if (pr[1] > pr[0])
            gemm_f32(st, true, true, pr[1] - pr[0], ldG, L.din, 1.f, x + (size_t)pr[0] * ldx, ldx, params.p + L.p_off + L.off_wx, pad4(L.din),
                     0.f, L.G.p + (size_t)pr[0] * ldG, ldG, params.p + L.p_off + L.off_bias, nullptr, 0, 0, fwd_bf16, x_amax, w_amax);
        timer.end(st, ti_);
        EESEN_HIP_CHECK(hipStreamWaitEvent(st, ev_gate_done, 0));
        mid_r0 = mid_r1 = 0;
      } else {
        const int ti_ = timer.begin(st, 0);
        gemm_f32(st, true, true, rows, ldG, L.din, 1.f, x, ldx, params.p + L.p_off + L.off_wx, pad4(L.din), 0.f, L.G.p, ldG,
                 params.p + L.p_off + L.off_bias, nullptr, 0, 0, fwd_bf16, x_amax, w_amax);
        timer.end(st, ti_);
      }
      Layer* nxt = (&L - layers.data()) + 1 < (long)layers.size() ? &layers[(&L - layers.data()) + 1] : nullptr;
      LstmLayerDev v = lstm_view(*this, L, T);
      const RecPlan fp = persistent ? lstm_fwd_plan(v) : RecPlan{};
      const bool pers = fp.kind != kRecNone;
      const bool plan_gate = pers && overlap && gate_fwd && !fwd_bf16 && !L.cur_fwd_drop && fp.units <= 8 && nxt && nxt->is_lstm() && T >= 2 && rows >= 128 &&
                             fp.one_window &&
                             (nxt->ndir * 4 * nxt->H) % 128 == 0 && ldY % 16 == 0 && nd * fp.seq_tiles * kShards <= 64;
      const int mile_step = (3 * T) / 4;
      const bool plan_mid = pers && overlap && tn.fwd_mid && !plan_gate && !L.cur_fwd_drop && fp.leaves_room && nd == 2 && nxt && nxt->is_lstm() &&
                            T >= 32 && mile_step + 1 < T && fp.one_window;
      { const int ti_ = timer.begin(st, 1);
      v.poll_delay = delay_fwd;
      v.poll_raw = poll_raw;
      if (plan_mid) {
        mile.reserve(32);
        EESEN_HIP_CHECK(hipMemsetAsync(mile.p, 0, 2 * sizeof(unsigned), st));
        EESEN_HIP_CHECK(hipEventRecord(ev_gate_reset, st));
        v.milestone = mile.p;
        v.milestone_step = mile_step;
      }
      if (pers) lstm_fwd_launch(st, fp, v, ctl.p, ctl.p + kCtlWords - 1, spin_limit, trace.p, plan_gate ? ev_gate_reset : nullptr);
      else
        for (int step = 0; step < T; ++step) lstm_fwd_step(st, v, step);
      info_fwd_persistent += pers ? 1 : 0;
      info_fwd_bf16 += fp.bf16 ? 1 : 0;
      ++info_lstm_layers;
      check_launch("lstm_fwd");
      timer.end(st, ti_);
      if (pers && plan_gate) {
        const int ldG2 = nxt->ndir * 4 * nxt->H;
        nxt->G.reserve((size_t)rows * ldG2);
        EESEN_HIP_CHECK(hipStreamWaitEvent(st2, ev_gate_reset, 0));
        const int tj_ = timer.begin(st2, 0);
        GemmGate gate{ctl.p, ctl.p + kCtlWords - 1, nd, fp.seq_tiles, fp.grid[0], T, S, spin_limit};
        gated_rows = rows / 128 * 128;
        gemm_f32_nt_gated(st2, gated_rows, ldG2, ldY, L.Y.p + (size_t)S * ldY, ldY, params.p + nxt->p_off + nxt->off_wx, pad4(nxt->din),
                          nxt->G.p, ldG2, params.p + nxt->p_off + nxt->off_bias, gate, half ? bound_one() : GemmBound{}, half ? GemmBound{nxt->bw.rows.p, 1} : GemmBound{});
        timer.end(st2, tj_);
        EESEN_HIP_CHECK(hipEventRecord(ev_gate_done, st2));
        g_gated = true;
      }
      if (plan_mid) {
        EESEN_HIP_CHECK(hipMemsetD32Async(reinterpret_cast<hipDeviceptr_t>(mile.p + 1), 1, 1, st));
        const int ldG2 = nxt->ndir * 4 * nxt->H;
        nxt->G.reserve((size_t)rows * ldG2);
        mid_r0 = ((T - 1 - mile_step) * S + 255) / 256 * 256;
        mid_r1 = (mile_step + 1) * S / 256 * 256;
        if (mid_r1 <= mid_r0) mid_r0 = mid_r1 = 0;
      }
      if (plan_mid && mid_r1 > mid_r0) {
        const int ldG2 = nxt->ndir * 4 * nxt->H;
        EESEN_HIP_CHECK(hipStreamWaitEvent(st2, ev_gate_reset, 0));
        wait_for_word(st2, mile.p + 1, 1u, ctl.p + kCtlWords - 1, 2.0 * std::max(1.0, T / 1000.0) * std::max(1.0, spin_limit / 400000.0));
        const int tj_ = timer.begin(st2, 0);
        gemm_f32(st2, true, true, mid_r1 - mid_r0, ldG2, nxt->din, 1.f, L.Y.p + (size_t)S * ldY + (size_t)mid_r0 * ldY, ldY,
                 params.p + nxt->p_off + nxt->off_wx, pad4(nxt->din), 0.f, nxt->G.p + (size_t)mid_r0 * ldG2, ldG2,
                 params.p + nxt->p_off + nxt->off_bias, nullptr, 0,  64, fwd_bf16,
                 half ? bound_one() : GemmBound{}, half ? GemmBound{nxt->bw.rows.p, 1} : GemmBound{});
        timer.end(st2, tj_);
        EESEN_HIP_CHECK(hipEventRecord(ev_gate_done, st2));
      } }
      if (L.cur_fwd_drop)
        mul_elements(st, L.Y.p + (size_t)S * ldY, ldY, L.fmask.p, ldY, L.Yd.p, ldY, rows, ldY);
      x = L.output(S);
      ldx = ldY;
    } else if (L.kind == EESEN_LAYER_AFFINE) {
      const int ldo = pad4(L.dout);
      if (L.out.reserve((size_t)rows * ldo)) EESEN_HIP_CHECK(hipMemsetAsync(L.out.p, 0, L.out.cap * sizeof(float), st));
      { const int ti_ = timer.begin(st, 2);
      gemm_f32(st, true, true, rows, L.dout, L.din, 1.f, x, ldx, params.p + L.p_off + L.off_w, pad4(L.din), 0.f, L.out.p, ldo,
               params.p + L.p_off + L.off_b, nullptr, 0, 0, fwd_bf16, x_amax, w_amax);
      timer.end(st, ti_); }
      x = L.out.p;
      ldx = ldo;
    } else if (L.is_activation()) {
      const int ldo = pad4(L.dout);
      if (L.out.reserve((size_t)rows * ldo)) EESEN_HIP_CHECK(hipMemsetAsync(L.out.p, 0, L.out.cap * sizeof(float), st));
      { const int ti_ = timer.begin(st, 2);
      activation_rows(st, L.kind == EESEN_LAYER_TANH, x, ldx, L.out.p, ldo, rows, L.dout);
      timer.end(st, ti_); }
      x = L.out.p;
      ldx = ldo;
    } else {
      const int ldo = pad4(L.dout);
      if (L.out.reserve((size_t)rows * ldo)) EESEN_HIP_CHECK(hipMemsetAsync(L.out.p, 0, L.out.cap * sizeof(float), st));
      { const int ti_ = timer.begin(st, 2);
      softmax_rows(st, x, ldx, L.out.p, ldo, rows, L.dout);
      timer.end(st, ti_); }
      x = L.out.p;
      ldx = ldo;
    }
  }
  out_ptr = x;
  out_cols = layers.back().dout;
  out_ld = ldx;
  if (const Layer& Lb = layers.back(); Lb.out_nb) {
    const int ldo = pad4(Lb.dout_f);
    if (out_f.reserve((size_t)rows * ldo) && ldo != Lb.dout_f) EESEN_HIP_CHECK(hipMemsetAsync(out_f.p, 0, out_f.cap * sizeof(float), st));
    for (int b = 0; b < Lb.out_nb; ++b) copy2d(st, x + (size_t)b * Lb.out_hi, ldx, out_f.p + (size_t)b * Lb.out_hf, ldo, rows, Lb.out_hf);
    out_ptr = out_f.p; out_cols = Lb.dout_f; out_ld = ldo;
  }
  propagated = true;
  if (persistent) arm_device_error_poll();
}

void Net::backpropagate(const float* out_diff, int ldd, float* in_diff, int ldi) {
  bucket_log.clear();
  deferred_buckets.clear();
  try {
    backpropagate_impl(out_diff, ldd, in_diff, ldi);
  } catch (...) {
    fail_step_buckets();
    throw;
  }
}

void Net::backpropagate_impl(const float* out_diff, int ldd, float* in_diff, int ldi) {
  EESEN_REQUIRE(propagated, EESEN_ERR_STATE, "Backpropagate needs a preceding Propagate");
  EESEN_HIP_CHECK(hipSetDevice(device));
  int maxdim = 0, max_g = 0, max_y = 0;
  size_t need_ws = 0;
  for (const Layer& L : layers) {
    maxdim = std::max(maxdim, std::max(pad4(L.din), pad4(L.dout)));
    if (L.is_lstm()) {
      max_g = std::max(max_g, L.ndir * 4 * L.H);
      max_y = std::max(max_y, L.ndir * L.H);
      need_ws = std::max(need_ws, lstm_bias_peep_ws_floats(T, S, L.H, L.ndir));
    }
    need_ws = std::max(need_ws, col_sums_ws_floats(rows, L.dout));
  }
  need_ws = std::max(need_ws, (size_t)16 << 20);
  ws.reserve(need_ws);
  ws_floats = need_ws;
  dA.reserve((size_t)rows * maxdim);
  dB.reserve((size_t)rows * maxdim);
  if (max_g) {
    DGb[0].reserve((size_t)rows * max_g);
    DGb[1].reserve((size_t)rows * max_g);
  }
  if (max_y) DCF.reserve((size_t)S * max_y);
  ws2.reserve(need_ws);
  int dg_slot = 0;
  bool side_pending[2] = {false, false};
  deferred_buckets.clear();
  const std::vector<RecPlan> bwd = bwd_plans(T);
  const bool overlap = overlap_for_minibatch(bwd);
  exchange_deferred = comm && exchange_deferred_for_minibatch(bwd);
  bucket_log.clear();
  info_bwd_persistent = 0;
  live_valid = comm != nullptr;
  if (comm) {
    comm_check_alive(comm);
    EESEN_HIP_CHECK(hipMemsetD32Async(reinterpret_cast<hipDeviceptr_t>(fresh.p + P), 0x3f800000, 1, st));
  }

  const int Kout = layers.back().dout;
  float* d = dA.p;
  int ld_d = pad4(Kout);
  float* dn = dB.p;
  const bool half = gemm_mode() == 2;
  ensure_weight_amax();
  auto x_cols = [&](int li) -> GemmBound {
    if (!half || !amx_valid) return GemmBound{};
    return x_is_bounded(li) ? bound_one() : GemmBound{layers[li].bx.cols.p, 1};
  };
  if (const Layer& Lb = layers.back(); Lb.out_nb) {
    EESEN_HIP_CHECK(hipMemsetAsync(d, 0, (size_t)rows * ld_d * sizeof(float), st));
    for (int b = 0; b < Lb.out_nb; ++b) copy2d(st, out_diff + (size_t)b * Lb.out_hf, ldd, d + (size_t)b * Lb.out_hi, ld_d, rows, Lb.out_hf);
  } else {
    if (ld_d != Kout) EESEN_HIP_CHECK(hipMemsetAsync(d, 0, (size_t)rows * ld_d * sizeof(float), st));
    copy2d(st, out_diff, ldd, d, ld_d, rows, Kout);
  }

  for (int li = (int)layers.size() - 1; li >= 0; --li) {
    Layer& L = layers[li];
    const float* x;
    int ldx;
    if (li == 0) { x = input.p; ldx = pad4(L.din); }
    else {
      const Layer& Pv = layers[li - 1];
      if (Pv.is_lstm()) { ldx = Pv.ndir * Pv.H; x = Pv.output(S); }
      else { ldx = pad4(Pv.dout); x = Pv.out.p; }
    }
    const bool want_in = li > 0 || in_diff != nullptr;
    const int ld_n = pad4(L.din);
    float* fr = fresh.p + L.p_off;
    if (L.kind == EESEN_LAYER_SOFTMAX) {
      continue;
    } else if (L.is_activation()) {
      { const int ti_ = timer.begin(st, 4);
      activation_diff_rows(st, L.kind == EESEN_LAYER_TANH, L.out.p, pad4(L.dout), d, ld_d, rows, L.dout);
      timer.end(st, ti_); }
      continue;
    } else if (L.kind == EESEN_LAYER_AFFINE) {
      { const int ti_ = timer.begin(st, 4);
      if (half) measure(d, rows, L.dout, ld_d, L.bd.rows, L.bd.cols);
      if (want_in) {
        if (ld_n != L.din) EESEN_HIP_CHECK(hipMemsetAsync(dn, 0, (size_t)rows * ld_n * sizeof(float), st));
        gemm_f32(st, true, false, rows, L.din, L.dout, 1.f, d, ld_d, params.p + L.p_off + L.off_w, pad4(L.din), 0.f, dn, ld_n,
                 nullptr, nullptr, 0, 0, false, half ? GemmBound{L.bd.rows.p, 1} : GemmBound{}, half ? GemmBound{L.bw.cols.p, 1} : GemmBound{});
      }
      gemm_f32(st, false, false, L.dout, L.din, rows, 1.f, d, ld_d, x, ldx, 0.f, fr + L.off_w, pad4(L.din), nullptr, ws.p, ws_floats, 0, false,
               half ? GemmBound{L.bd.cols.p, 1} : GemmBound{}, x_cols(li));
      col_sums(st, d, rows, L.dout, ld_d, fr + L.off_b, ws.p, ws_floats);
      timer.end(st, ti_); }
      bucket_allreduce(li, st);
    } else {
      const int H = L.H, nd = L.ndir, ldG = nd * 4 * H, ldY = nd * H;
      LstmLayerDev v = lstm_view(*this, L, T);
      v.poll_delay = overlap ? delay_bwd_side : delay_bwd;
      v.poll_raw = poll_raw;
      const RecPlan& bp = bwd[li];
      if (bp.need_px) { bwd_px.reserve(bp.need_px); v.PX = bwd_px.p; v.px_floats = bwd_px.cap; }
      if (bp.need_dgh) {
        bwd_dgh.reserve((size_t)rows * ldG);
        bwd_ex.reserve(bp.need_ex);
        v.DGH = reinterpret_cast<unsigned char*>(bwd_dgh.p);
        v.EX = bwd_ex.p;
      }
      EESEN_REQUIRE(in_train || !L.has_dropout(), EESEN_ERR_STATE, "Can't backpropagate a dropout layer in test mode (bilstm-parallel-layer.h:425)");
      if (L.cur_fwd_drop) mul_elements(st, d, ld_d, L.fmask.p, ldY, d, ld_d, rows, ldY);
      float* DGl = DGb[dg_slot].p;
      if (side_pending[dg_slot]) {
        EESEN_HIP_CHECK(hipStreamWaitEvent(st, ev_grad[dg_slot], 0));
        side_pending[dg_slot] = false;
      }
      { const int ti_ = timer.begin(st, 3);
      if (bp.kind != kRecNone) {
        lstm_bwd_launch(st, bp, v, d, ld_d, DGl, ctl.p + kCtlHalf, ctl.p + kCtlWords - 1, spin_limit, trace.p ? trace.p + 640 : nullptr);
        ++info_bwd_persistent;
      } else
        for (int step = 0; step < T; ++step) lstm_bwd_step(st, v, step, d, ld_d, DGl, DCF.p);
      check_launch("lstm_bwd");
      timer.end(st, ti_); }
      if (half) { const int ti_ = timer.begin(st, 4); measure(DGl, rows, ldG, ldG, L.bd.rows, L.bd.cols); timer.end(st, ti_); }
      EESEN_HIP_CHECK(hipEventRecord(ev_rec, st));
      if (want_in) {
        const int ti_ = timer.begin(st, 4);
        if (ld_n != L.din) EESEN_HIP_CHECK(hipMemsetAsync(dn, 0, (size_t)rows * ld_n * sizeof(float), st));
        gemm_f32(st, true, false, rows, L.din, ldG, 1.f, DGl, ldG, params.p + L.p_off + L.off_wx, pad4(L.din), 0.f, dn, ld_n,
                 nullptr, nullptr, 0, 0, false, half ? GemmBound{L.bd.rows.p, 1} : GemmBound{}, half ? GemmBound{L.bw.cols.p, 1} : GemmBound{});
        timer.end(st, ti_);
        EESEN_HIP_CHECK(hipEventRecord(ev_rec, st));
      }
      hipStream_t sg = overlap ? st2 : st;
      const int side_lds_env = (tn.side_lds_kb >= 0 ? tn.side_lds_kb : (gemm_mode() >= 1 ? 48 : 32)) * 1024;
      bool lstm_below = false;
      for (int lj = 0; lj < li; ++lj) lstm_below |= layers[lj].is_lstm();
      const int side_lds = overlap && lstm_below ? side_lds_env : 0;
      if (overlap) EESEN_HIP_CHECK(hipStreamWaitEvent(st2, ev_rec, 0));
      { const int ti_ = timer.begin(sg, 4);
      gemm_f32(sg, false, false, ldG, L.din, rows, 1.f, DGl, ldG, x, ldx, 0.f, fr + L.off_wx, pad4(L.din), nullptr, ws2.p, need_ws, side_lds, false,
               half ? GemmBound{L.bd.cols.p, 1} : GemmBound{}, x_cols(li));
      for (int dir = 0; dir < nd; ++dir)
        gemm_f32(sg, false, false, 4 * H, H, rows, 1.f, DGl + (size_t)dir * 4 * H, ldG,
                 L.Y.p + (size_t)(dir == 0 ? 0 : 2 * S) * ldY + (size_t)dir * H, ldY, 0.f,
                 fr + L.off_wm + (size_t)dir * 4 * H * H, H, nullptr, ws2.p, need_ws, side_lds, false,
                 half ? GemmBound{L.bd.cols.p + (size_t)dir * 4 * H, 1} : GemmBound{}, half ? bound_one() : GemmBound{});
      lstm_bias_peep_grads(sg, v, DGl, fr + L.off_bias, fr + L.off_peep, ws2.p, need_ws);
      timer.end(sg, ti_); }
      bucket_allreduce(li, sg);
      if (overlap) {
        EESEN_HIP_CHECK(hipEventRecord(ev_grad[dg_slot], st2));
        side_pending[dg_slot] = true;
      }
      dg_slot ^= 1;
    }
    if (want_in) {
      std::swap(d, dn);
      ld_d = ld_n;
    }
  }
  if (in_diff) copy2d(st, d, ld_d, in_diff, ldi, rows, layers[0].din);
  flush_deferred_buckets();
  for (int k = 0; k < 2; ++k)
    if (side_pending[k]) EESEN_HIP_CHECK(hipStreamWaitEvent(st, ev_grad[k], 0));
}

std::vector<RecPlan> Net::bwd_plans(int T) const {
  std::vector<RecPlan> plans(layers.size());
  for (size_t li = 0; li < layers.size(); ++li)
    if (persistent && layers[li].is_lstm()) plans[li] = lstm_bwd_plan(lstm_view(*this, layers[li], T));
  return plans;
}
bool Net::overlap_for_minibatch(const std::vector<RecPlan>& bwd) const {
  bool ov = overlap;
  if (ov && tn.overlap < 0 && persistent)
    for (size_t li = 0; li < layers.size(); ++li)
      if (const Layer& L = layers[li]; L.is_lstm() && L.H > 320 && L.H <= 512 && S > 32 && !bwd[li].light) ov = false;
  return ov;
}
bool Net::exchange_deferred_for_minibatch(const std::vector<RecPlan>& bwd) const {
  if (tn.comm_defer >= 0) return tn.comm_defer != 0;
  if (!persistent) return false;
  for (const RecPlan& bp : bwd)
    if (bp.kind != kRecNone && bp.free_vgprs < kRcclVgprsPerSimdLane) return true;
  return false;
}

std::string Net::plan_string() const {
  EESEN_REQUIRE(finalized, EESEN_ERR_STATE, "net not finalized");
  EESEN_REQUIRE(S > 0, EESEN_ERR_STATE, "call eesen_net_set_seq_lengths first: the plan depends on the minibatch shape");
  EESEN_HIP_CHECK(hipSetDevice(device));
  int T = this->T;
  if (!propagated) { T = 0; for (int v : lens) T = std::max(T, v); }
  auto one = [](const RecPlan& P) {
    char b[512];
    if (P.kind == kRecNone) { snprintf(b, sizeof(b), "{\"kernel\": \"per-step kernels (lstm.hip)\", \"persistent\": false}"); return std::string(b); }
    snprintf(b, sizeof(b), "{\"kernel\": \"%s\", \"persistent\": true, \"sequences_per_workgroup\": %d, \"units_per_workgroup\": %d, \"grid\": [%d, %d, %d], "
             "\"workgroups\": %d, \"workgroups_per_cu\": %d, \"launches\": %d, \"vgprs\": %d, \"lds_bytes\": %d, \"free_vgprs_per_simd_lane\": %d}",
             P.kernel, P.seq_tile, P.units, P.grid[0], P.grid[1], P.grid[2], P.wgs, P.wgs_per_cu, P.windows, P.vgprs, P.lds, P.free_vgprs);
    return std::string(b);
  };
  const std::vector<RecPlan> bwd = bwd_plans(T);
  std::string o = "{\"T\": " + std::to_string(T) + ", \"S\": " + std::to_string(S) + ", \"persistent\": " + (persistent ? "true" : "false") + ", \"layers\": [";
  bool first = true;
  for (size_t li = 0; li < layers.size(); ++li) {
    const Layer& L = layers[li];
    if (!L.is_lstm()) continue;
    const RecPlan fp = persistent && T >= 1 ? lstm_fwd_plan(lstm_view(*this, L, T)) : RecPlan{}, &bp = bwd[li];
    o += std::string(first ? "" : ", ") + "{\"layer\": " + std::to_string(li) + ", \"cells\": " + std::to_string(L.H) + ", \"directions\": " + std::to_string(L.ndir) +
         ", \"forward\": " + one(fp) + ", \"backward\": " + one(bp) + "}";
    first = false;
  }
  const bool ov = overlap_for_minibatch(bwd);
  o += std::string("], \"weight_gradient_gemms\": \"") + (ov ? "side stream, under the next-lower recurrence" : "main stream, serial") + "\"";
  o += std::string(", \"gemm_arithmetic\": \"") + (gemm_mode() == 2 ? "two fp16 planes, three products (fp32-class)" : gemm_mode() == 1 ? "3-way bf16 split (fp32-class)" : "f32-input MFMA") + "\"";
  o += std::string(", \"exchange\": ") + (comm ? (exchange_deferred_for_minibatch(bwd) ? "\"deferred: every bucket behind the backward pass's last recurrence\""
                                                                                      : "\"overlapped: each bucket as soon as its layer's gradients are enqueued\"") : "null");
  o += std::string(", \"exchange_rule\": \"") + (tn.comm_defer >= 0 ? "EESEN_COMM_DEFER" : "auto: deferred when a persistent backward grid leaves < 256 registers per SIMD lane") + "\"";
  o += ", \"gpu_share\": " + std::to_string(gpu_share_value()) + "}";
  return o;
}

void Net::update() {
  EESEN_REQUIRE(finalized, EESEN_ERR_STATE, "net not finalized");
  EESEN_HIP_CHECK(hipSetDevice(device));
  const unsigned* skip = persistent && !grads_sanitized ? ctl.p + kCtlWords - 1 : nullptr;
  const float* live = comm && live_valid ? fresh.p + P : nullptr;
  comm_check_alive(comm);
  { const int ti_ = timer.begin(st, 5);
  for (int li = (int)layers.size() - 1; li >= 0; --li) {
    Layer& L = layers[li];
    if (L.p_n) {
      if (comm && li < (int)bucket_pending.size() && bucket_pending[li]) {
        const int tw_ = timer.begin(st, 7);
        EESEN_HIP_CHECK(hipStreamWaitEvent(st, ev_bucket[li], 0));
        timer.end(st, tw_);
        bucket_pending[li] = 0;
      }
      if (rule == 0) {
        sgd_update(st, params.p + L.p_off, corr.p + L.p_off, fresh.p + L.p_off, (long)L.p_n, mmt, lr * L.coef, L.max_grad, skip, live);
      } else {
        init_accu();
        adaptive_update(st, params.p + L.p_off, corr.p + L.p_off, fresh.p + L.p_off, accu.p + L.p_off, (long)L.p_n, mmt, lr,
                        L.max_grad, ada_eps, rms_rho, rms_one_minus_rho, rule == 2, skip, live);
      }
    }
  }
  refresh_derived();
  timer.end(st, ti_); }
  grads_sanitized = false;
  live_valid = false;
  if (persistent) arm_device_error_poll();
}

}
```

eesen_amd/csrc/net.h:

```cpp
#pragma once
#include <string>
#include <vector>

#include "kernels.h"
#include "tuning.h"

namespace eesen {

inline int pad4(int x) { return (x + 3) & ~3; }
constexpr size_t kCtlWords = 2 * kCtlHalf + 32;

struct Layer {
  int kind = 0, din = 0, dout = 0;
  float coef = 1.f, max_grad = 0.f;
  size_t p_off = 0, p_n = 0;
  int H = 0, ndir = 0;
  int din_f = 0, dout_f = 0, Hf = 0;
  int in_nb = 0, in_hf = 0, in_hi = 0, out_nb = 0, out_hf = 0, out_hi = 0;
  int in_col(int d) const { return in_nb ? (d / in_hf) * in_hi + d % in_hf : d; }
  size_t off_wx = 0, off_bias = 0, off_wm = 0, off_peep = 0;
  DevBuf<float> WmT;
  DevBuf<float> G, C, Y;
  DevBuf<float> X;
  size_t off_w = 0, off_b = 0;
  DevBuf<float> out;
  struct Bounds { DevBuf<float> rows, cols; } bw, bx, bd;
  float drop[9] = {0, 0, 0, 0, 0, 0, 0, 0, 0};
  bool has_dropout() const { return drop[0] > 0.f || drop[5] != 0.f || drop[6] != 0.f; }
  DevBuf<float> fmask;
  DevBuf<float> rmask;
  DevBuf<float> Yd;
  bool cur_fwd_drop = false;
  int cur_drop_mode = 0;
  bool cur_twiddle_coin = false;
  std::vector<float> inj_fmask, inj_rmask;
  int inj_rmask_rows = 0, inj_coin = -1;
  const float* output(int S) const { return cur_fwd_drop ? Yd.p : Y.p + (size_t)S * ndir * H; }
  bool is_lstm() const { return kind == EESEN_LAYER_LSTM_PARALLEL || kind == EESEN_LAYER_BILSTM_PARALLEL; }
  bool nonparallel = false;
  bool is_activation() const { return kind == EESEN_LAYER_SIGMOID || kind == EESEN_LAYER_TANH; }
  bool trainable() const { return is_lstm() || kind == EESEN_LAYER_AFFINE; }
  long file_params() const;
  const char* marker() const;
};

class PhaseTimer {
 public:
  ~PhaseTimer();
  void enable(bool on) { on_ = on; }
  bool enabled() const { return on_; }
  void set_accumulate(bool a) { accumulate_ = a; used_ = 0; }
  void reset() { if (!accumulate_) used_ = 0; }
  int begin(hipStream_t st, int phase);
  void end(hipStream_t st, int idx);
  void collect(float* out, int nphase);
  int spans(int* phases, float* secs, int cap);
 private:
  struct Span { hipEvent_t a, b; int phase; };
  std::vector<Span> spans_;
  size_t used_ = 0;
  bool on_ = false, accumulate_ = false;
};

struct Comm;
void comm_check_alive(const Comm* c);
constexpr size_t kLiveWords = 4;
constexpr int kRcclVgprsPerSimdLane = 256;

struct Net {
  int device = 0;
  hipStream_t st = nullptr;
  bool own_stream = false;
  std::vector<Layer> layers;
  bool finalized = false;
  size_t P = 0;
  DevBuf<float> params, corr, fresh;
  float lr = 0.f, mmt = 0.f;
  int rule = 0;
  float ada_eps = 1e-6f, rms_rho = 0.9f, rms_one_minus_rho = 0.1f;
  DevBuf<float> accu;
  bool accu_init = false;
  void init_accu();
  void set_accu(const float* host, long n);
  std::vector<int> lens;
  DevBuf<int> lens_d;
  int T = 0, S = 0, rows = 0;
  bool propagated = false;
  DevBuf<float> input;
  struct HostStage { float* p = nullptr; size_t cap = 0; hipEvent_t ev = nullptr; bool busy = false; } in_stage[2];
  unsigned in_stage_idx = 0;
  const float* out_ptr = nullptr;
  int out_cols = 0, out_ld = 0;
  DevBuf<float> out_f;
  DevBuf<float> DGb[2], DCF, dA, dB, ws, ws2;
  DevBuf<float> bwd_px;
  DevBuf<float> bwd_dgh, bwd_ex;
  hipStream_t st2 = nullptr;
  hipEvent_t ev_rec = nullptr, ev_grad[2] = {nullptr, nullptr};
  bool overlap = true;
  hipEvent_t ev_gate_reset = nullptr, ev_gate_done = nullptr;
  DevBuf<unsigned> mile;
  bool gate_fwd = true;
  bool fwd_bf16 = false;
  bool fwd_bf16_rec = false;
  int info_fwd_bf16 = 0;
  DevBuf<unsigned> ctl;
  Tuning tn;
  int persistent = 1;
  int info_fwd_persistent = 0, info_bwd_persistent = 0, info_lstm_layers = 0;
  int spin_limit = 400000;
  float flight_ns = 0.f;
  int delay_fwd = 61, delay_bwd = 43, delay_bwd_side = 64, poll_raw = 0;
  int recoveries = 0;
  DevBuf<unsigned long long> trace;
  void check_device_error(bool consumer);
  int steps_since_clean = 0;
  int* lens_pin = nullptr;
  size_t lens_pin_cap = 0;
  hipEvent_t lens_ev = nullptr, err_ev = nullptr;
  unsigned* err_pin = nullptr;
  bool err_armed = false;
  void poll_device_error();
  void arm_device_error_poll();
  bool in_train = true;
  unsigned long long drop_seed = 777, drop_counter = 0;
  void set_train_mode(bool train) { in_train = train; }
  void set_layer_dropout(int layer, const float* nine);
  void get_layer_dropout(int layer, float* nine) const;
  void set_dropout_masks(int layer, const float* fwd, long fwd_n, const float* rec, int rec_rows, long rec_n, int coin);
  void get_dropout_masks(int layer, float* fwd_host, float* rec_host, int* info4);
  size_t ws_floats = 0;
  DevBuf<float> amax, amax_ws;
  bool wamax_valid = false, wm_valid = false;
  bool amx_valid = false;
  float* am_wm(int li) { return amax.p + 1 + li; }
  GemmBound bound_one() const { return GemmBound{amax.p, 0}; }
  bool x_is_bounded(int li) const;
  void measure(const float* P, long rows, int cols, int ld, DevBuf<float>& out_rows, DevBuf<float>& out_cols);
  void ensure_weight_amax();
  PhaseTimer timer;
  Comm* comm = nullptr;
  std::vector<hipEvent_t> ev_ready, ev_bucket;
  std::vector<char> bucket_pending;
  std::vector<int> deferred_buckets;
  bool exchange_deferred = false;
  std::vector<RecPlan> bwd_plans(int T) const;
  bool overlap_for_minibatch(const std::vector<RecPlan>& bwd) const;
  bool exchange_deferred_for_minibatch(const std::vector<RecPlan>& bwd) const;
  std::string plan_string() const;
  hipEvent_t ev_bwd_done = nullptr;
  void issue_bucket(int li);
  void fail_step_buckets() noexcept;
  void flush_deferred_buckets();
  std::vector<struct Ctc*> guards;
  std::vector<struct CeLoss*> ce_guards;
  bool grads_sanitized = false;
  bool live_valid = false;
  std::vector<int> bucket_log;
  float* live_pin = nullptr;
  void set_comm(Comm* c);
  int top_trainable() const;
  int live_ranks();
  void bucket_allreduce(int li, hipStream_t producer);
  void wait_buckets_host();
  void backpropagate_zero();
  void allreduce_grads(Comm* c);

  Net(int device, void* stream);
  ~Net();
  void add_layer(int kind, int din, int dout, float coef, float max_grad);
  void finalize();
  long num_params() const;
  void set_params(const float* host, long n);
  void get_flat(const DevBuf<float>& buf, float* host, long n);
  void set_seq_lengths(const int* lens, int S);
  void propagate(const float* in, int rows, int ld, bool is_device);
  void forward_pass();
  void backpropagate(const float* out_diff, int ldd, float* in_diff, int ldi);
  void backpropagate_impl(const float* out_diff, int ldd, float* in_diff, int ldi);
  void update();
  void refresh_derived();
  int tensor_moments(int which, int layer, double* out6_host, int cap_tensors);
  void read(const std::string& path);
  void write(const std::string& path, bool binary);
  void sync();
};

struct Ctc {
  int device = 0;
  hipStream_t st = nullptr;
  bool own_stream = false;
  DevBuf<float> logp, alpha, beta, pzx_d;
  DevBuf<int> labx, lens_d, lablens_d, cls_off, cls_pos, ids_d;
  std::vector<int> last_lens;
  int last_T = 0, last_S = 0, last_Lpad = 0, last_Lprime = 0;
  int sweep_waves = 0;
  double obj_sum = 0;
  long sequences = 0, frames = 0, err_tokens = 0, ref_tokens = 0;
  hipEvent_t ev[4] = {nullptr, nullptr, nullptr, nullptr};
  PhaseTimer timer;
  struct Pin {
    void* p = nullptr;
    size_t cap = 0;
    hipEvent_t ev = nullptr;
    bool busy = false;
  };
  Pin stage[2];
  unsigned stage_idx = 0;
  struct PendingPzx { Pin pin; int S = 0; long nframes = 0; bool active = false; } ppzx[2];
  struct PendingErr { Pin pin, probs; int S = 0, K = 0, rows = 0; bool active = false, with_probs = false, guarded = false; std::vector<int> frames, ids, off; } perr[2];
  const unsigned* guard = nullptr;
  struct Net* guard_net = nullptr;
  long dropped = 0;
  std::string seq_out;
  unsigned ppzx_idx = 0, perr_idx = 0;
  static void* pin_reserve(Pin& pin, size_t bytes);
  void flush_pzx(PendingPzx& q);
  void flush_err(PendingErr& q, int* num_err, int* num_ref);
  void flush();

  Ctc(int device, void* stream);
  ~Ctc();
  void eval_parallel(const int* frame_num_utt, int S, const float* net_out, int rows, int K, int ld, const int* label_ids,
                     const int* label_off, float* diff, int ldd, float* pzx_host);
  void error_rate_mseq(const int* frame_num_utt, int S, const float* net_out, int rows, int K, int ld,
                       const int* label_ids, const int* label_off, int* num_err, int* num_ref);
  void get_alpha_beta(float* alpha_host, float* beta_host, int* Lprime);
  void phase_times(float* out3);
};

struct CeLoss {
  int device = 0;
  hipStream_t st = nullptr;
  DevBuf<int> tg;
  DevBuf<CeSums> part, res;
  Ctc::Pin stage[2];
  unsigned stage_idx = 0;
  struct Pending { Ctc::Pin pin; int S = 0; long rows = 0; bool active = false; } pend[2];
  unsigned pend_idx = 0;
  double obj = 0, obj_progress = 0;
  long correct = 0, frames = 0, sequences = 0, correct_progress = 0, frames_progress = 0, sequences_progress = 0;
  int report_step = 100;
  std::vector<std::string> progress;
  const unsigned* guard = nullptr;
  struct Net* guard_net = nullptr;
  long dropped = 0;
  hipEvent_t ev[2] = {nullptr, nullptr};
  PhaseTimer timer;

  CeLoss(int device, void* stream);
  ~CeLoss();
  void fold(Pending& q, double* obj_out);
  void flush();
  void eval_parallel(const int* frame_num_utt, int S, const float* net_out, int rows, int K, int ld, const int* targets,
                     float* diff, int ldd, double* obj_host);
  std::string report();
  void phase_times(float* out1);
};

}
```

eesen_amd/csrc/optim.hip:

```cpp
#include "kernels.h"

namespace eesen {
namespace {

__global__ __launch_bounds__(256) void sgd_update_kernel(float* __restrict__ param, float* __restrict__ corr,
                                                         const float* __restrict__ fresh, long n, float mmt,
                                                         float lr_coef, float max_grad, const unsigned* __restrict__ skip,
                                                         const float* __restrict__ live) {
  if (skip && *skip) return;
  if (live && *live == 0.f) return;
  const long n4 = n >> 2;
  const long stride = (long)gridDim.x * blockDim.x;
  for (long i = (long)blockIdx.x * blockDim.x + threadIdx.x; i < n4; i += stride) {
    float4 p = reinterpret_cast<float4*>(param)[i];
    float4 c = reinterpret_cast<float4*>(corr)[i];
    const float4 g = reinterpret_cast<const float4*>(fresh)[i];
    c.x = mmt * c.x + g.x; c.y = mmt * c.y + g.y; c.z = mmt * c.z + g.z; c.w = mmt * c.w + g.w;
    if (max_grad > 0.f) {
      c.x = fminf(fmaxf(c.x, -max_grad), max_grad); c.y = fminf(fmaxf(c.y, -max_grad), max_grad);
      c.z = fminf(fmaxf(c.z, -max_grad), max_grad); c.w = fminf(fmaxf(c.w, -max_grad), max_grad);
    }
    p.x -= lr_coef * c.x; p.y -= lr_coef * c.y; p.z -= lr_coef * c.z; p.w -= lr_coef * c.w;
    reinterpret_cast<float4*>(corr)[i] = c;
    reinterpret_cast<float4*>(param)[i] = p;
  }
  for (long i = (n4 << 2) + (long)blockIdx.x * blockDim.x + threadIdx.x; i < n; i += stride) {
    float c = mmt * corr[i] + fresh[i];
    if (max_grad > 0.f) c = fminf(fmaxf(c, -max_grad), max_grad);
    corr[i] = c;
    param[i] -= lr_coef * c;
  }
}

__global__ __launch_bounds__(256) void adaptive_update_kernel(float* __restrict__ param, float* __restrict__ corr,
                                                              const float* __restrict__ fresh, float* __restrict__ accu,
                                                              long n, float mmt, float lr, float max_grad, float eps,
                                                              float rho, float one_minus_rho, int rmsprop,
                                                              const unsigned* __restrict__ skip, const float* __restrict__ live) {
  if (skip && *skip) return;
  if (live && *live == 0.f) return;
  const long stride = (long)gridDim.x * blockDim.x;
  for (long i = (long)blockIdx.x * blockDim.x + threadIdx.x; i < n; i += stride) {
    float c = mmt * corr[i] + fresh[i];
    if (max_grad > 0.f) c = fminf(fmaxf(c, -max_grad), max_grad);
    const float g2 = c * c;
    float a = accu[i];
    a = rmsprop ? (rho * a + one_minus_rho * g2) : (a + g2);
    const float scale = 1.0f / sqrtf(a + eps);
    corr[i] = c;
    accu[i] = a;
    param[i] += -lr * scale * c;
  }
}

__global__ __launch_bounds__(256) void zero_if_set_kernel(float* __restrict__ p, long n, const unsigned* __restrict__ word) {
  if (*word == 0u) return;
  const long stride = (long)gridDim.x * blockDim.x;
  for (long i = (long)blockIdx.x * blockDim.x + threadIdx.x; i < n; i += stride) p[i] = 0.f;
}

__global__ __launch_bounds__(256) void transpose2d_kernel(const float* __restrict__ src, int rows, int cols,
                                                          float* __restrict__ dst) {
  __shared__ float tile[32][33];
  const int tx = threadIdx.x & 31, ty = threadIdx.x >> 5;
  const int c0 = blockIdx.x * 32, r0 = blockIdx.y * 32;
#pragma unroll
  for (int i = 0; i < 32; i += 8) {
    const int r = r0 + ty + i, c = c0 + tx;
    if (r < rows && c < cols) tile[ty + i][tx] = src[(size_t)r * cols + c];
  }
  __syncthreads();
#pragma unroll
  for (int i = 0; i < 32; i += 8) {
    const int c = c0 + ty + i, r = r0 + tx;
    if (r < rows && c < cols) dst[(size_t)c * rows + r] = tile[tx][ty + i];
  }
}

__global__ __launch_bounds__(256) void copy2d_kernel(const float* __restrict__ src, int lds, float* __restrict__ dst,
                                                     int ldd, int rows, int cols) {
  const size_t total = (size_t)rows * cols;
  for (size_t i = (size_t)blockIdx.x * blockDim.x + threadIdx.x; i < total; i += (size_t)gridDim.x * blockDim.x) {
    const size_t r = i / cols, c = i % cols;
    dst[r * ldd + c] = src[r * lds + c];
  }
}

}

void sgd_update(hipStream_t st, float* param, float* corr, const float* fresh, long n, float mmt, float lr_coef,
                float max_grad, const unsigned* skip, const float* live) {
  if (n <= 0) return;
  const int blocks = (int)std::min<long>(cdivl(n / 4 + 1, 256), 2048);
  hipLaunchKernelGGL(sgd_update_kernel, dim3(blocks), dim3(256), 0, st, param, corr, fresh, n, mmt, lr_coef, max_grad, skip, live);
  check_launch("sgd_update");
}

void zero_if_set(hipStream_t st, float* p, long n, const unsigned* word) {
  if (n <= 0 || !word) return;
  hipLaunchKernelGGL(zero_if_set_kernel, dim3(256), dim3(256), 0, st, p, n, word);
  check_launch("zero_if_set");
}

void adaptive_update(hipStream_t st, float* param, float* corr, const float* fresh, float* accu, long n, float mmt, float lr,
                     float max_grad, float eps, float rho, float one_minus_rho, bool rmsprop, const unsigned* skip, const float* live) {
  if (n <= 0) return;
  const int blocks = (int)std::min<long>(cdivl(n, 256), 4096);
  hipLaunchKernelGGL(adaptive_update_kernel, dim3(blocks), dim3(256), 0, st, param, corr, fresh, accu, n, mmt, lr, max_grad, eps,
                     rho, one_minus_rho, rmsprop ? 1 : 0, skip, live);
  check_launch("adaptive_update");
}

void transpose2d(hipStream_t st, const float* src, int rows, int cols, float* dst) {
  hipLaunchKernelGGL(transpose2d_kernel, dim3(cdiv(cols, 32), cdiv(rows, 32)), dim3(256), 0, st, src, rows, cols, dst);
  check_launch("transpose2d");
}

void copy2d(hipStream_t st, const float* src, int lds, float* dst, int ldd, int rows, int cols) {
  if (rows <= 0 || cols <= 0) return;
  const size_t total = (size_t)rows * cols;
  const int blocks = (int)std::min<size_t>((total + 255) / 256, 4096);
  hipLaunchKernelGGL(copy2d_kernel, dim3(blocks), dim3(256), 0, st, src, lds, dst, ldd, rows, cols);
  check_launch("copy2d");
}


namespace {
__device__ __forceinline__ float hash_uniform(unsigned long long seed, unsigned long long idx) {
  unsigned long long z = seed + (idx + 1ull) * 0x9E3779B97F4A7C15ull;
  z = (z ^ (z >> 30)) * 0xBF58476D1CE4E5B9ull;
  z = (z ^ (z >> 27)) * 0x94D049BB133111EBull;
  z ^= z >> 31;
  return (float)(z >> 40) * (1.0f / 16777216.0f);
}
__global__ __launch_bounds__(256) void dropout_mask_kernel(float* __restrict__ out, long rows, int cols, int ld, float p, float scale,
                                                           unsigned long long seed, int per_column) {
  const long n = rows * cols;
  for (long i = (long)blockIdx.x * blockDim.x + threadIdx.x; i < n; i += (long)gridDim.x * blockDim.x) {
    const long r = i / cols;
    const int c = (int)(i % cols);
    const float u = hash_uniform(seed, per_column ? (unsigned long long)c : (unsigned long long)i);
    out[r * ld + c] = (u - p > 0.f) ? scale : 0.f;
  }
}
__global__ __launch_bounds__(256) void mul_elements_kernel(const float* __restrict__ a, int lda, const float* __restrict__ m, int ldm,
                                                           float* __restrict__ out, int ldo, long rows, int cols) {
  const long n = rows * cols;
  for (long i = (long)blockIdx.x * blockDim.x + threadIdx.x; i < n; i += (long)gridDim.x * blockDim.x) {
    const long r = i / cols;
    const int c = (int)(i % cols);
    out[r * ldo + c] = a[r * lda + c] * m[r * ldm + c];
  }
}
template <bool TANH>
__global__ __launch_bounds__(256) void activation_kernel(const float* __restrict__ x, int ldx, float* __restrict__ y, int ldy, long rows, int cols) {
  const long n = rows * cols;
  for (long i = (long)blockIdx.x * blockDim.x + threadIdx.x; i < n; i += (long)gridDim.x * blockDim.x) {
    const long r = i / cols;
    const int c = (int)(i % cols);
    const float v = x[r * ldx + c];
    float o;
    if (TANH) {
      const float e = expf(2.0f * v);
      o = isinf(e) ? 1.0f : (e - 1.0f) / (e + 1.0f);
    } else {
      o = 1.0f / (1.0f + expf(-v));
    }
    y[r * ldy + c] = o;
  }
}
template <bool TANH>
__global__ __launch_bounds__(256) void activation_diff_kernel(const float* __restrict__ y, int ldy, float* __restrict__ d, int ldd, long rows, int cols) {
  const long n = rows * cols;
  for (long i = (long)blockIdx.x * blockDim.x + threadIdx.x; i < n; i += (long)gridDim.x * blockDim.x) {
    const long r = i / cols;
    const int c = (int)(i % cols);
    const float o = y[r * ldy + c];
    d[r * ldd + c] *= TANH ? (1.0f - o * o) : o * (1.0f - o);
  }
}
}

void activation_rows(hipStream_t st, bool tanh_, const float* x, int ldx, float* y, int ldy, long rows, int cols) {
  if (rows <= 0 || cols <= 0) return;
  const int blocks = (int)std::min<long>(cdivl(rows * cols, 256), 256L * 16);
  if (tanh_) hipLaunchKernelGGL(activation_kernel<true>, dim3(blocks), dim3(256), 0, st, x, ldx, y, ldy, rows, cols);
  else hipLaunchKernelGGL(activation_kernel<false>, dim3(blocks), dim3(256), 0, st, x, ldx, y, ldy, rows, cols);
  check_launch("activation_rows");
}

void activation_diff_rows(hipStream_t st, bool tanh_, const float* y, int ldy, float* d, int ldd, long rows, int cols) {
  if (rows <= 0 || cols <= 0) return;
  const int blocks = (int)std::min<long>(cdivl(rows * cols, 256), 256L * 16);
  if (tanh_) hipLaunchKernelGGL(activation_diff_kernel<true>, dim3(blocks), dim3(256), 0, st, y, ldy, d, ldd, rows, cols);
  else hipLaunchKernelGGL(activation_diff_kernel<false>, dim3(blocks), dim3(256), 0, st, y, ldy, d, ldd, rows, cols);
  check_launch("activation_diff_rows");
}

void dropout_mask(hipStream_t st, float* out, long rows, int cols, int ld, float p, unsigned long long seed, bool per_column) {
  if (rows <= 0 || cols <= 0) return;
  const int blocks = (int)std::min<long>(cdivl(rows * cols, 256), 256L * 16);
  hipLaunchKernelGGL(dropout_mask_kernel, dim3(blocks), dim3(256), 0, st, out, rows, cols, ld, p, 1.0f / (1.0f - p), seed, per_column ? 1 : 0);
  check_launch("dropout_mask");
}

void mul_elements(hipStream_t st, const float* a, int lda, const float* m, int ldm, float* out, int ldo, long rows, int cols) {
  if (rows <= 0 || cols <= 0) return;
  const int blocks = (int)std::min<long>(cdivl(rows * cols, 256), 256L * 16);
  hipLaunchKernelGGL(mul_elements_kernel, dim3(blocks), dim3(256), 0, st, a, lda, m, ldm, out, ldo, rows, cols);
  check_launch("mul_elements");
}

namespace {
template <int PASS>
__global__ __launch_bounds__(1024) void tensor_moments_kernel(const float* __restrict__ base, long rows, int cols, long ld,
                                                              double* __restrict__ out6, double* __restrict__ ws, int nb, int hf, int hi) {
  __shared__ double red[4][16];
  const long n = rows * cols;
  const int tid = threadIdx.x, lane = tid & 63, wave = tid >> 6;
  double a = PASS == 0 ? 1e300 : 0.0, b = PASS == 0 ? -1e300 : 0.0, c = 0.0, d = 0.0;
  const double mean = PASS == 1 ? ws[2] / (double)n : 0.0;
  for (long i = tid; i < n; i += 1024) {
    const int cf = (int)(i % cols);
    const double v = (double)base[(i / cols) * ld + (nb ? (cf / hf) * hi + cf % hf : cf)];
    if (PASS == 0) { a = fmin(a, v); b = fmax(b, v); c += v; }
    else { const double e = v - mean, e2 = e * e; a += e2; b += e2 * e; c += e2 * e2; }
  }
  for (int off = 32; off > 0; off >>= 1) {
    const double a2 = __shfl_down(a, off), b2 = __shfl_down(b, off), c2 = __shfl_down(c, off);
    if (PASS == 0) { a = fmin(a, a2); b = fmax(b, b2); c += c2; }
    else { a += a2; b += b2; c += c2; }
  }
  if (lane == 0) { red[0][wave] = a; red[1][wave] = b; red[2][wave] = c; red[3][wave] = d; }
  __syncthreads();
  if (tid == 0) {
    for (int w = 1; w < 16; ++w) {
      if (PASS == 0) { a = fmin(a, red[0][w]); b = fmax(b, red[1][w]); c += red[2][w]; }
      else { a += red[0][w]; b += red[1][w]; c += red[2][w]; }
    }
    if (PASS == 0) { ws[0] = a; ws[1] = b; ws[2] = c; }
    else {
      const double var = a / (double)n;
      out6[0] = ws[0]; out6[1] = ws[1]; out6[2] = mean; out6[3] = var;
      out6[4] = b / pow(var, 1.5) / (double)n;
      out6[5] = c / (var * var) / (double)n - 3.0;
    }
  }
}
}

void tensor_moments(hipStream_t st, const float* base, long rows, int cols, long ld, double* out6, double* ws, int nb, int hf, int hi) {
  hipLaunchKernelGGL(tensor_moments_kernel<0>, dim3(1), dim3(1024), 0, st, base, rows, cols, ld, out6, ws, nb, hf, hi);
  hipLaunchKernelGGL(tensor_moments_kernel<1>, dim3(1), dim3(1024), 0, st, base, rows, cols, ld, out6, ws, nb, hf, hi);
  check_launch("tensor_moments");
}

}
```

eesen_amd/csrc/rec_plan.cpp:

```cpp
#include "rec_kernels.h"

#include <atomic>
#include <map>
#include <mutex>
#include <tuple>

namespace eesen {
namespace {

constexpr int NW = kRecWaves;

std::atomic<int> g_share_override{0};
int gpu_share() {
  static const int env = [] { const char* e = getenv("EESEN_GPU_SHARE"); const int v = e && *e ? atoi(e) : 0; return v < 1 ? 0 : v; }();
  if (env) return env;
  const int o = g_share_override.load(std::memory_order_relaxed);
  return o > 0 ? o : 1;
}
int share_of_cus() {
  int ncu = 256, dev = 0;
  (void)hipGetDevice(&dev);
  (void)hipDeviceGetAttribute(&ncu, hipDeviceAttributeMultiprocessorCount, dev);
  return std::max(1, ncu / gpu_share());
}

template <class... Args>
void plan_launch(hipStream_t st, const void* fn, int wgs, Args... args) {
  void* argv[] = {static_cast<void*>(&args)...};
  EESEN_HIP_CHECK(hipLaunchKernel(fn, dim3(wgs), dim3(NW * 64), argv, 0, st));
}

bool bf_census(const RecKernel& k, int wgs) {
  static std::mutex mu;
  static std::map<std::tuple<int, const void*, int>, bool> seen;
  int dev = 0;
  if (hipGetDevice(&dev) != hipSuccess) return false;
  if (gpu_share() > 1) return false;
  std::lock_guard<std::mutex> lock(mu);
  const auto key = std::make_tuple(dev, k.fn, wgs);
  if (auto it = seen.find(key); it != seen.end()) return it->second;
  bool ok = false;
  unsigned* w = nullptr;
  if (hipDeviceSynchronize() == hipSuccess && hipMalloc(reinterpret_cast<void**>(&w), 2 * sizeof(unsigned)) == hipSuccess) {
    for (int take = 0; take < 3 && !ok; ++take) {
      if (hipMemset(w, 0, 2 * sizeof(unsigned)) != hipSuccess) break;
      LstmLayerDev L{};
      L.T = -1;
      unsigned* err = w + 1;
      int spin_limit = 0;
      unsigned long long* trace = nullptr;
      RecRole role{1, 1, 1, 0};
      void* argv[] = {&L, &w, &err, &spin_limit, &trace, &role};
      if (hipLaunchKernel(k.fn, dim3(wgs), dim3(NW * 64), argv, 0, nullptr) != hipSuccess) { (void)hipGetLastError(); break; }
      unsigned e = 1;
      ok = hipMemcpy(&e, w + 1, sizeof(unsigned), hipMemcpyDeviceToHost) == hipSuccess && e == 0;
    }
    (void)hipFree(w);
  }
  seen[key] = ok;
  if (getenv("EESEN_PRINT_PLAN")) fprintf(stderr, "LOG (eesen_hip) residency census: %d workgroups of %s on device %d: %s\n", wgs, k.name, dev, ok ? "seen co-resident" : "NOT seen");
  return ok;
}

bool fits(const RecKernel& k, dim3 grid, bool census = false) {
  int dev = 0, ncu = 0, nb = 0;
  if (hipGetDevice(&dev) != hipSuccess) return false;
  if (hipDeviceGetAttribute(&ncu, hipDeviceAttributeMultiprocessorCount, dev) != hipSuccess) return false;
  {
    static std::mutex mu;
    static std::map<std::pair<int, const void*>, int> cache;
    std::lock_guard<std::mutex> lock(mu);
    const auto key = std::make_pair(dev, k.fn);
    auto it = cache.find(key);
    if (it == cache.end()) {
      if (hipOccupancyMaxActiveBlocksPerMultiprocessor(&nb, k.fn, NW * 64, 0) != hipSuccess) return false;
      it = cache.emplace(key, nb).first;
    }
    nb = it->second;
  }
  const long wgs = (long)grid.x * grid.y * grid.z;
  if (wgs <= (long)ncu * std::max(1, nb - 1) / gpu_share()) return true;
  return census && wgs <= (long)ncu * nb / gpu_share() && bf_census(k, (int)wgs);
}


size_t ctl_words(size_t groups) { return groups * kShards * kShardStride; }

bool line_aligned(int seqs, int cols) { return ((size_t)seqs * cols * sizeof(float)) % 128 == 0; }

template <class F>
int pick_windows(int S, int seq_tile, F fits_with) {
  for (int nwin = 1; nwin <= 8; nwin *= 2) {
    if (S % nwin != 0 || (S / nwin) % seq_tile != 0) { if (nwin == 1 && fits_with(S)) return 1; continue; }
    if (fits_with(S / nwin)) return nwin;
  }
  return 0;
}

void take(RecPlan& P, const RecKernel& k, const dim3& grid, size_t words, int seq_tile, int units, int windows) {
  P.kind = k.kind; P.fn = k.fn; P.kernel = k.name;
  P.seq_tile = seq_tile; P.units = units; P.windows = windows; P.ctl_words = words;
  P.grid[0] = (int)grid.x; P.grid[1] = (int)grid.y; P.grid[2] = (int)grid.z;
  P.wgs = (int)(grid.x * grid.y * grid.z);
  P.wgs_per_cu = std::max(1, cdiv(P.wgs, share_of_cus()));
  static std::mutex mu;
  static std::map<const void*, std::pair<int, int>> cache;
  std::lock_guard<std::mutex> lock(mu);
  auto it = cache.find(P.fn);
  if (it == cache.end()) {
    hipFuncAttributes a{};
    if (hipFuncGetAttributes(&a, P.fn) != hipSuccess) { (void)hipGetLastError(); return; }
    it = cache.emplace(P.fn, std::make_pair((int)a.numRegs, (int)a.sharedSizeBytes)).first;
  }
  P.vgprs = it->second.first;
  P.lds = it->second.second;
  if (P.vgprs > 0) P.free_vgprs = 512 - P.wgs_per_cu * (NW / 4) * ((P.vgprs + 7) & ~7);
}

struct FwdTile { int mt, nt; };
struct BfPlan { bool on; int cpw, nt, ap, wp; bool f16; };

bool small_xchg(const LstmLayerDev& L, int bytes_per_unit_row) {
  return (size_t)L.T * L.ndir * cdiv(L.S, 16) * (size_t)(L.H / 32) * bytes_per_unit_row < ((size_t)1 << 31);
}
bool bf_fits(const LstmLayerDev& L, const BfPlan& P, int Sw) {
  const RecKernel* k = rec_kernel(kFwdBf, P.cpw, P.nt, P.ap, P.wp, P.f16);
  return k && fits(*k, dim3(L.H / (4 * P.nt), L.ndir, cdiv(Sw, 16)),  true);
}
bool narrow2_ok(const LstmLayerDev& L, int need) {
  const bool f16 = L.fwd_f16 && L.wm_amax != nullptr;
  if (!L.fwd_narrow2 || !(L.fwd_split || f16) || L.fwd_bf16 || L.X == nullptr || L.drop_mode || L.T < 2 || L.H % 32 != 0) return false;
  if (!small_xchg(L, 1024 * 3)) return false;
  return bf_fits(L, f16 ? BfPlan{true, need, 2, 2, 2, true} : BfPlan{true, need, 2, 3, 3, false}, L.S);
}
FwdTile fwd_tile(const LstmLayerDev& L) {
  const int need = ((L.H + 31) / 32 + NW - 1) / NW;
  const int ncu = share_of_cus();
  const bool t16_ok = L.H % 8 == 0 && (L.S > 16 || need > 2 || (L.fwd_t16_small && L.fwd_split && !L.drop_mode && L.X && L.H % 32 == 0));
  const long narrow_wgs = (long)(L.H / 8) * L.ndir * cdiv(L.S, 16);
  const bool narrow_full = narrow_wgs > ncu && !(narrow_wgs <= 2L * ncu && need <= 2 && narrow2_ok(L, need));
  if (t16_ok && L.H % 16 == 0 && need <= 4 && (need > 2 || narrow_full)) return {1, 4};
  if (t16_ok && need <= 2) return {1, 2};
  return {2, 1};
}

BfPlan bf_plan_shape(const LstmLayerDev& L, const FwdTile& ft) {
  const BfPlan off{false, 0, 0, 0, 0, false};
  if (L.X == nullptr || L.drop_mode || L.T < 2 || L.H % 32 != 0) return off;
  if (L.fwd_bf16) {
    if (L.H % 256 != 0 || L.H / 256 > 4 || !small_xchg(L, 1024)) return off;
    return {true, L.H / 256, 4, 1, 2, false};
  }
  const bool f16 = L.fwd_f16 && L.wm_amax != nullptr;
  if (L.fwd_split || f16) {
    const int need = (L.H / 32 + NW - 1) / NW;
    if (f16 && ft.mt == 1 && ft.nt == 4 && L.H % 256 == 0 && L.H / 256 <= 4 && small_xchg(L, 1024 * 2)) return {true, L.H / 256, 4, 2, 2, true};
    if (ft.mt != 1 || ft.nt != 2 || need > 2 || L.H % 8 != 0 || !small_xchg(L, 1024 * 3)) return off;
    if (f16) return {true, need, 2, 2, 2, true};
    if (L.fwd_split) return {true, need, 2, 3, 3, false};
  }
  return off;
}

bool bwd_ksplit_shape(const LstmLayerDev& L, int stile) {
  return L.bwd_ksplit && stile == 16 && !L.drop_mode && L.H % 256 == 0 && L.H >= 768 && L.H <= 1024 && L.T >= 2;
}
bool bwd_planes_shape(const LstmLayerDev& L, int stile) {
  const int cpw = L.H / (32 * NW);
  return L.bwd_f16 && L.wm_amax != nullptr && bwd_ksplit_shape(L, stile) && (cpw == 2 || cpw == 4) && L.H % (32 * NW) == 0;
}

}

void set_gpu_share(int n) { g_share_override.store(n < 1 ? 1 : n, std::memory_order_relaxed); }
int gpu_share_value() { return gpu_share(); }

float handoff_flight_ns() {
  static float cache[64] = {0};
  static std::mutex mu;
  std::lock_guard<std::mutex> lock(mu);
  int dev = 0;
  if (hipGetDevice(&dev) != hipSuccess || dev < 0 || dev >= 64) return 0.f;
  if (cache[dev] > 0.f) return cache[dev];
  unsigned* flags = nullptr;
  unsigned long long* out = nullptr;
  EESEN_HIP_CHECK(hipMalloc(reinterpret_cast<void**>(&flags), 64 * sizeof(unsigned)));
  EESEN_HIP_CHECK(hipMalloc(reinterpret_cast<void**>(&out), sizeof(unsigned long long)));
  int rounds = 2000;
  double ns[5];
  for (int rep = 0; rep < 5; ++rep) {
    EESEN_HIP_CHECK(hipMemset(flags, 0, 64 * sizeof(unsigned)));
    void* argv[] = {&flags, &out, &rounds};
    (void)hipLaunchKernel(handoff_pingpong_fn(), dim3(2), dim3(64), argv, 0, nullptr);
    unsigned long long ticks = 0;
    EESEN_HIP_CHECK(hipMemcpy(&ticks, out, sizeof(ticks), hipMemcpyDeviceToHost));
    ns[rep] = ticks ? 10.0 * (double)ticks / (2.0 * rounds) : 500.0;
  }
  std::sort(ns, ns + 5);
  (void)hipFree(flags);
  (void)hipFree(out);
  cache[dev] = (float)std::min(2000.0, std::max(100.0, ns[2]));
  return cache[dev];
}

void wait_for_word(hipStream_t st, const unsigned* word, unsigned target, unsigned* err, double limit_s) {
  unsigned long long ticks = (unsigned long long)(std::max(0.05, limit_s) * 1e8);
  void* argv[] = {&word, &target, &err, &ticks};
  (void)hipLaunchKernel(wait_for_word_fn(), dim3(1), dim3(64), argv, 0, st);
  check_launch("wait_for_word");
}

RecPlan lstm_fwd_plan(const LstmLayerDev& L) {
  RecPlan P;
  const int need = ((L.H + 31) / 32 + NW - 1) / NW;
  const FwdTile ft = fwd_tile(L);
  if (need > 4 || (ft.nt == 2 && need > 2) || L.H % (4 * ft.nt) != 0 || L.T < 2) return P;
  if (!line_aligned(L.S, L.ndir * L.H)) return P;
  if ((size_t)(L.T + 2) * L.S * L.ndir * L.H * sizeof(float) >= ((size_t)1 << 31)) return P;
  BfPlan B = bf_plan_shape(L, ft);
  const bool drop = L.drop_mode != 0;
  const int cpw32 = ft.nt == 2 ? std::min(need, 2) : need <= 2 ? need : 4;
  int nwin = B.on ? pick_windows(L.S, 16, [&](int Sw) { return bf_fits(L, B, Sw); }) : 0;
  if (nwin == 0) {
    B.on = false;
    const RecKernel* probe = rec_kernel(kFwdF32, cpw32, ft.mt, ft.nt, drop, false);
    nwin = pick_windows(L.S, 16 * ft.mt, [&](int Sw) { return probe && fits(*probe, dim3(L.H / (4 * ft.nt), L.ndir, cdiv(Sw, 16 * ft.mt))); });
  }
  if (nwin == 0) return P;
  if (nwin > 1 && !line_aligned(L.S / nwin, L.ndir * L.H)) return P;
  const int mt = B.on ? 1 : ft.mt, nt = B.on ? B.nt : ft.nt, nz = cdiv(L.S, 16 * mt);
  auto answer = [&](const RecKernel& k, const dim3& grid, size_t words, int seq_tile, int windows, bool one_window) {
    take(P, k, grid, words, seq_tile, 4 * nt, windows);
    P.seq_tiles = nz;
    P.one_window = one_window;
    P.leaves_room = nt <= 2 && (!B.on || (long)(L.H / (4 * nt)) * L.ndir * nz <= share_of_cus());
    P.bf16 = L.fwd_bf16 && k.kind == kRecFwdBf;
  };
  const dim3 grid(L.H / (4 * nt), L.ndir, cdiv(L.S / nwin, 16 * mt));
  const size_t words = ctl_words(grid.y * grid.z);
  if (B.on) {
    if (words <= (size_t)kCtlHalf) answer(*rec_kernel(kFwdBf, B.cpw, B.nt, B.ap, B.wp, B.f16), grid, words, 16, nwin, nwin == 1);
    return P;
  }
  const bool xchg = L.X != nullptr && ft.mt == 1 && L.H % 32 == 0 && !drop && small_xchg(L, 2048);
  if (L.fwd_mux && nwin == 2 && ft.mt == 1 && ft.nt == 4 && need > 2 && need <= 4 && !drop && L.H % 32 == 0) {
    const RecKernel& k = *rec_kernel(kFwdMux, 4, 4, xchg);
    const dim3 mgrid(L.H / 16, L.ndir, cdiv(nz, 2));
    if (fits(k, mgrid) && ctl_words((size_t)L.ndir * nz) <= (size_t)kCtlHalf) {
      answer(k, mgrid, ctl_words((size_t)L.ndir * nz), 32, 1, false);
      return P;
    }
  }
  if (words > (size_t)kCtlHalf) return P;
  const RecKernel* k = rec_kernel(kFwdF32, cpw32, ft.mt, ft.nt, drop, xchg);
  EESEN_REQUIRE(k != nullptr, EESEN_ERR_STATE, "no instantiation of the fp32 forward tile for this plan");
  answer(*k, grid, words, 16 * ft.mt, nwin, nwin == 1);
  return P;
}

void lstm_fwd_launch(hipStream_t st, const RecPlan& P, const LstmLayerDev& L0, unsigned* cnt, unsigned* err, int spin_limit,
                     unsigned long long* trace, hipEvent_t after_reset) {
  EESEN_REQUIRE(P.kind == kRecFwdBf || P.kind == kRecFwdMux || P.kind == kRecFwdF32, EESEN_ERR_STATE, "not a forward recurrence plan");
  const RecRole role{P.grid[0], P.grid[1], P.grid[2], L0.xcd_map};
  for (int w = 0; w < P.windows; ++w) {
    LstmLayerDev L = L0;
    if (P.kind == kRecFwdMux) { L.s_begin = 0; L.s_count = 0; }
    else { L.s_count = L0.S / P.windows; L.s_begin = w * L.s_count; }
    if (P.kind != kRecFwdMux && P.wgs_per_cu >= 2 && !L0.poll_raw) L.poll_delay = L0.poll_delay * 7 / 4;
    EESEN_HIP_CHECK(hipMemsetAsync(cnt, 0, sizeof(unsigned) * P.ctl_words, st));
    if (after_reset && P.one_window) EESEN_HIP_CHECK(hipEventRecord(after_reset, st));
    if (P.kind == kRecFwdMux) plan_launch(st, P.fn, P.wgs, L, cnt, err, spin_limit, role);
    else plan_launch(st, P.fn, P.wgs, L, cnt, err, spin_limit, trace, role);
  }
}

RecPlan lstm_bwd_plan(const LstmLayerDev& L) {
  RecPlan P;
  const int need = ((4 * L.H + 31) / 32 + NW - 1) / NW;
  const int ldG = L.ndir * 4 * L.H;
  const long blocks16 = (long)cdiv(L.H, 16) * L.ndir * cdiv(L.S, 16);
  const int stile = 2 * blocks16 <= share_of_cus() && L.S > 8 ? 8 : 16;
  P.light = stile == 8;
  if (need > 16 || L.T < 2) return P;
  if (!line_aligned(L.S, ldG)) return P;
  const size_t blk_bytes = (size_t)L.S * ldG * sizeof(float);
  const long max_blocks = (long)((((size_t)1 << 31) - 1) / blk_bytes);
  if (max_blocks < 3) return P;
  int chunk = (int)std::min<long>(L.T, max_blocks - 1);
  if (chunk < L.T) { int p2 = 1; while (p2 * 2 <= chunk) p2 *= 2; chunk = p2; }
  P.chunk = chunk;
  auto in_windows = [&](const RecKernel* k, int gx, int seq_tile, int units, int quarters) {
    if (!k) return false;
    auto grid_of = [&](int Sw) { return dim3(gx, L.ndir, cdiv(Sw, seq_tile)); };
    auto words_of = [&](const dim3& g) { return ctl_words((size_t)g.y * g.z * quarters); };
    const int nwin = pick_windows(L.S, seq_tile, [&](int Sw) { return words_of(grid_of(Sw)) <= (size_t)kCtlHalf && fits(*k, grid_of(Sw)); });
    if (nwin == 0 || (nwin > 1 && !line_aligned(L.S / nwin, ldG))) return false;
    take(P, *k, grid_of(L.S / nwin), words_of(grid_of(L.S / nwin)), seq_tile, units, nwin);
    return true;
  };
  for (int pass = 0; pass < 2; ++pass) {
    const int stq = (L.bwd_q4_st8 == 2) == (pass == 0) ? 8 : 4;
    if (!L.bwd_q4 || L.drop_mode || L.H % 32 != 0 || L.H > 512 || chunk < L.T) break;
    if (stq == 4 && stile != 8) continue;
    if (stq == 8 && !(L.bwd_q4_st8 && L.S > 8)) continue;
    const int cpw = 2 * ((L.H + 127) / 128);
    const dim3 grid(L.H / 32, L.ndir, cdiv(L.S, stq));
    const size_t words = ctl_words((size_t)grid.y * grid.z);
    const RecKernel& k = *rec_kernel(kBwdQ4, cpw, stq);
    if (fits(k, grid) && words <= (size_t)kCtlHalf) {
      take(P, k, grid, words, stq, 32, 1);
      return P;
    }
  }
  if (bwd_ksplit_shape(L, stile)) {
    const int cpw = L.H / (32 * NW), gx = L.H / 64 * 4;
    const size_t px = (size_t)2 * L.ndir * cdiv(L.S, 16) * (size_t)(L.H / 64) * 4096 * 2;
    if (bwd_planes_shape(L, stile) && in_windows(rec_kernel(kBwdKsplitH, cpw), gx, 16, 64, 4)) {
      P.need_px = px; P.need_dgh = true;
      P.need_ex = (size_t)L.T * L.ndir * cdiv(L.S, 16) * (size_t)(L.H / 16) * 16;
      return P;
    }
    const RecKernel* k = rec_kernel(kBwdKsplit, cpw);
    const int nwin = !k ? 0 : pick_windows(L.S, 16, [&](int Sw) {
      const dim3 grid(gx, L.ndir, cdiv(Sw, 16));
      return ctl_words((size_t)grid.y * grid.z * 4) <= (size_t)kCtlHalf && fits(*k, grid);
    });
    if (nwin == 2 && L.bwd_mux && cpw >= 2 && cpw <= 4) {
      const int nz = cdiv(L.S, 16);
      const dim3 grid(gx, L.ndir, cdiv(nz, 2));
      const size_t words = ctl_words((size_t)L.ndir * nz * 4);
      const RecKernel& km = *rec_kernel(kBwdKsplitMux, cpw);
      if (words <= (size_t)kCtlHalf && fits(km, grid)) {
        take(P, km, grid, words, 32, 64, 1);
        P.need_px = px;
        return P;
      }
    }
    if (nwin > 0 && (nwin == 1 || line_aligned(L.S / nwin, ldG))) {
      const dim3 grid(gx, L.ndir, cdiv(L.S / nwin, 16));
      take(P, *k, grid, ctl_words((size_t)grid.y * grid.z * 4), 16, 64, nwin);
      P.need_px = px;
      return P;
    }
  }
  in_windows(rec_kernel(kBwdGeneric, need <= 1 ? 1 : need <= 2 ? 2 : need <= 4 ? 4 : need <= 8 ? 8 : 16, stile, L.drop_mode != 0), cdiv(L.H, 16), stile, 16, 1);
  return P;
}

void lstm_bwd_launch(hipStream_t st, const RecPlan& P, const LstmLayerDev& L0, const float* dY, int lddy, float* DG, unsigned* cnt,
                     unsigned* err, int spin_limit, unsigned long long* trace) {
  EESEN_REQUIRE(P.kind == kRecBwdQ4 || P.kind == kRecBwdKsplit || P.kind == kRecBwdKsplitMux || P.kind == kRecBwdGeneric, EESEN_ERR_STATE, "not a backward recurrence plan");
  EESEN_REQUIRE(!P.need_px || (L0.PX && L0.px_floats >= P.need_px), EESEN_ERR_STATE, "the backward plan's partial-sum exchange space (RecPlan::need_px) was not handed over");
  EESEN_REQUIRE(!P.need_dgh || (L0.DGH && L0.EX), EESEN_ERR_STATE, "the backward plan's plane and exponent buffers (RecPlan::need_dgh, need_ex) were not handed over");
  const RecRole role{P.grid[0], P.grid[1], P.grid[2], L0.xcd_map};
  const bool whole_batch = P.kind == kRecBwdQ4 || P.kind == kRecBwdKsplitMux;
  unsigned long long* px = reinterpret_cast<unsigned long long*>(L0.PX);
  int chunk = P.chunk;
  for (int w = 0; w < P.windows; ++w) {
    LstmLayerDev L = L0;
    if (whole_batch) { L.s_begin = 0; L.s_count = 0; }
    else { L.s_count = L0.S / P.windows; L.s_begin = w * L.s_count; }
    EESEN_HIP_CHECK(hipMemsetAsync(cnt, 0, sizeof(unsigned) * P.ctl_words, st));
    if (P.need_px) EESEN_HIP_CHECK(hipMemsetAsync(L.PX, 0, sizeof(float) * P.need_px, st));
    if (P.kind == kRecBwdQ4) plan_launch(st, P.fn, P.wgs, L, dY, lddy, DG, cnt, err, spin_limit, trace, role);
    else if (P.kind == kRecBwdKsplitMux) plan_launch(st, P.fn, P.wgs, L, dY, lddy, DG, px, cnt, err, spin_limit, role, chunk);
    else if (P.kind == kRecBwdKsplit) plan_launch(st, P.fn, P.wgs, L, dY, lddy, DG, px, cnt, err, spin_limit, role, chunk, trace);
    else plan_launch(st, P.fn, P.wgs, L, dY, lddy, DG, cnt, err, spin_limit, trace, role, chunk);
  }
}

}
```

include/eesen_hip.h:

```cpp
#ifndef EESEN_HIP_H_
#define EESEN_HIP_H_

#ifdef __cplusplus
extern "C" {
#endif

#define EESEN_OK 0
#define EESEN_ERR_INVALID -1
#define EESEN_ERR_HIP -2
#define EESEN_ERR_STATE -3
#define EESEN_ERR_IO -4
#define EESEN_ERR_COMM -5

#define EESEN_LAYER_AFFINE 1
#define EESEN_LAYER_SOFTMAX 2
#define EESEN_LAYER_LSTM_PARALLEL 3
#define EESEN_LAYER_BILSTM_PARALLEL 4
#define EESEN_LAYER_SIGMOID 5
#define EESEN_LAYER_TANH 6

typedef struct eesen_net eesen_net_t;
typedef struct eesen_ctc eesen_ctc_t;
typedef struct eesen_ce eesen_ce_t;

const char* eesen_last_error(void);
const char* eesen_version(void);
int eesen_device_count(int* count);

int eesen_set_gemm_mode(int mode);
int eesen_get_gemm_mode(int* mode);

int eesen_net_create(int device, void* stream, eesen_net_t** out);
int eesen_net_destroy(eesen_net_t* net);
int eesen_net_add_layer(eesen_net_t* net, int kind, int in_dim, int out_dim,
                        float learn_rate_coef, float max_grad);
int eesen_net_finalize(eesen_net_t* net);
int eesen_net_read(eesen_net_t* net, const char* path);
int eesen_net_write(eesen_net_t* net, const char* path, int binary);

int eesen_net_num_layers(eesen_net_t* net, int* n);
int eesen_net_layer_info(eesen_net_t* net, int idx, int* kind, int* in_dim, int* out_dim,
                         float* learn_rate_coef, float* max_grad);
int eesen_net_layer_marker(eesen_net_t* net, int idx, char* buf, int cap);
int eesen_net_tensor_moments(eesen_net_t* net, int which, int layer, double* out6_host, int cap_tensors, int* n_tensors);
int eesen_net_input_dim(eesen_net_t* net, int* dim);
int eesen_net_output_dim(eesen_net_t* net, int* dim);
int eesen_net_num_params(eesen_net_t* net, long* n);
int eesen_net_get_params(eesen_net_t* net, float* host_flat, long n);
int eesen_net_set_params(eesen_net_t* net, const float* host_flat, long n);

int eesen_net_set_train_options(eesen_net_t* net, float learn_rate, float momentum);
int eesen_net_set_update_algorithm(eesen_net_t* net, const char* name);
int eesen_net_set_adaptive_options(eesen_net_t* net, float adagrad_epsilon, float rmsprop_rho);
int eesen_net_get_accumulators(eesen_net_t* net, float* host_flat, long n);
int eesen_net_set_accumulators(eesen_net_t* net, const float* host_flat, long n);
int eesen_net_set_seq_lengths(eesen_net_t* net, const int* lens, int S);

int eesen_net_propagate(eesen_net_t* net, const float* in, int rows, int in_ld, int in_is_device,
                        const float** out_dev, int* out_cols, int* out_ld);
int eesen_net_get_output(eesen_net_t* net, float* host_out, long n);

int eesen_net_backpropagate(eesen_net_t* net, const float* out_diff_dev, int out_diff_ld,
                            float* in_diff_dev, int in_diff_ld);
int eesen_net_grad_buffer(eesen_net_t* net, float** dev_ptr, long* n);
int eesen_net_get_grads(eesen_net_t* net, float* host_flat, long n);
int eesen_net_update(eesen_net_t* net);
int eesen_net_set_forward_precision(eesen_net_t* net, int mode);
int eesen_net_bf16_recurrence_layers(eesen_net_t* net, int* layers);
int eesen_net_recurrence_info(eesen_net_t* net, int* out4);
int eesen_net_plan_string(eesen_net_t* net, char* json, int cap);
int eesen_net_debug_set_error_word(eesen_net_t* net, unsigned value);
int eesen_net_synchronize(eesen_net_t* net);
int eesen_net_set_profiling(eesen_net_t* net, int on);
int eesen_net_get_phase_times(eesen_net_t* net, float* out6);
int eesen_net_get_phase_spans(eesen_net_t* net, int* phases, float* seconds, int cap, int* n);

typedef struct eesen_comm eesen_comm_t;
int eesen_comm_get_unique_id(char* id128);
int eesen_comm_exchange(const char* addr, int port, int rank, int world, char* buf, int nbytes, int timeout_s);
int eesen_comm_create(int device, const char* id128, int rank, int world, eesen_comm_t** out);
int eesen_comm_create_tcp(int device, const char* addr, int port, int rank, int world, int timeout_s, eesen_comm_t** out);
int eesen_comm_destroy(eesen_comm_t* comm);
int eesen_comm_info(eesen_comm_t* comm, int* rank, int* world);
int eesen_comm_describe(eesen_comm_t* comm, char* json, int cap);
int eesen_comm_allreduce_host(eesen_comm_t* comm, double* values, int n, int op);
int eesen_net_set_comm(eesen_net_t* net, eesen_comm_t* comm);
int eesen_net_allreduce_grads(eesen_net_t* net, eesen_comm_t* comm);
int eesen_net_backpropagate_zero(eesen_net_t* net);
int eesen_net_live_ranks(eesen_net_t* net, int* live);
int eesen_net_bucket_order(eesen_net_t* net, int* layers_out, int cap, int* n);
int eesen_device_synchronize(int device);

int eesen_ctc_create(int device, void* stream, eesen_ctc_t** out);
int eesen_ctc_destroy(eesen_ctc_t* ctc);
int eesen_ctc_eval_parallel(eesen_ctc_t* ctc, const int* frame_num_utt, int S, const float* net_out_dev,
                            int rows, int K, int ld, const int* label_ids, const int* label_off,
                            float* diff_dev, int diff_ld, float* pzx_host);
int eesen_ctc_error_rate_mseq(eesen_ctc_t* ctc, const int* frame_num_utt, int S, const float* net_out_dev,
                              int rows, int K, int ld, const int* label_ids, const int* label_off,
                              int* num_err, int* num_ref);
int eesen_ctc_set_sequence_out_file(eesen_ctc_t* ctc, const char* path);
int eesen_ctc_set_guard(eesen_ctc_t* ctc, eesen_net_t* net);
int eesen_ctc_dropped(eesen_ctc_t* ctc, long* minibatches);
int eesen_ctc_stats(eesen_ctc_t* ctc, double* obj_sum, long* sequences, long* frames, long* err_tokens,
                    long* ref_tokens);
int eesen_ctc_get_alpha_beta(eesen_ctc_t* ctc, float* alpha_host, float* beta_host, int* Lprime);
int eesen_ctc_set_profiling(eesen_ctc_t* ctc, int mode);
int eesen_ctc_get_phase_times(eesen_ctc_t* ctc, float* out3);

int eesen_ce_create(int device, void* stream, eesen_ce_t** out);
int eesen_ce_destroy(eesen_ce_t* ce);
int eesen_ce_eval_parallel(eesen_ce_t* ce, const int* frame_num_utt, int S, const float* net_out_dev, int rows, int K, int ld,
                           const int* targets_host, float* diff_dev, int diff_ld, double* obj_host);
int eesen_ce_set_report_step(eesen_ce_t* ce, int report_step);
int eesen_ce_stats(eesen_ce_t* ce, double* obj, long* correct, long* frames, long* sequences);
int eesen_ce_report(eesen_ce_t* ce, char* buf, int cap);
int eesen_ce_progress(eesen_ce_t* ce, int wait, char* buf, int cap);
int eesen_ce_set_guard(eesen_ce_t* ce, eesen_net_t* net);
int eesen_ce_dropped(eesen_ce_t* ce, long* minibatches);
int eesen_ce_set_profiling(eesen_ce_t* ce, int mode);
int eesen_ce_get_phase_times(eesen_ce_t* ce, float* out1);

int eesen_net_set_train_mode(eesen_net_t* net, int train);
int eesen_net_set_dropout_seed(eesen_net_t* net, unsigned long long seed);
int eesen_net_set_layer_dropout(eesen_net_t* net, int layer, const float* nine);
int eesen_net_get_layer_dropout(eesen_net_t* net, int layer, float* nine);
int eesen_net_set_dropout_masks(eesen_net_t* net, int layer, const float* fwd_mask_host, long fwd_floats,
                                const float* rec_mask_host, int rec_rows, long rec_floats, int twiddle_coin);
int eesen_net_get_dropout_masks(eesen_net_t* net, int layer, float* fwd_mask_host, float* rec_mask_host, int* info4);

typedef struct eesen_feeder eesen_feeder_t;
int eesen_feeder_create(int device, void* compute_stream, int slots, eesen_feeder_t** out);
int eesen_feeder_destroy(eesen_feeder_t* f);
int eesen_feeder_submit(eesen_feeder_t* f, const float* const* utts, const int* frames, const int* strides, int S, int D,
                        int* slot);
int eesen_feeder_acquire(eesen_feeder_t* f, int slot, float** feats_dev, int* T, int* S, int* ld);
int eesen_feeder_release(eesen_feeder_t* f, int slot);

#define EESEN_FEAT_CMVN 1
#define EESEN_FEAT_SPLICE 2
#define EESEN_FEAT_SUBSAMPLE 3
#define EESEN_FEAT_DELTAS 4
typedef struct eesen_feat_stage { int kind, a, b; } eesen_feat_stage_t;
int eesen_feeder_set_pipeline(eesen_feeder_t* f, const eesen_feat_stage_t* stages, int n_stages);
int eesen_feeder_pipeline_shape(eesen_feeder_t* f, int D_in, int frames_in, int* D_out, int* frames_out);
int eesen_feeder_submit_raw(eesen_feeder_t* f, const float* const* utts, const int* frames, const int* strides,
                            const float* const* cmvn, int S, int D_in, int* slot);
int eesen_cmvn_norm(const double* stats, int rows, int cols, int norm_vars, float* offset_scale);

int eesen_dev_alloc(int device, long bytes, void** dev_ptr);
int eesen_dev_free(int device, void* dev_ptr);
int eesen_dev_copy(int device, void* dst, const void* src, long bytes, int kind );

int eesen_op_gemm(int device, void* stream, int a_kc, int b_kc, int M, int N, int K, float alpha,
                  const float* A, int lda, const float* B, int ldb, float beta, float* C, int ldc,
                  const float* bias);

int eesen_op_gemm_async(int device, void* stream, int a_kc, int b_kc, int M, int N, int K, const float* A, int lda, const float* B, int ldb,
                        float* C, int ldc, float* ws, long ws_floats, int extra_lds_bytes);

int eesen_op_log_sub_prior(int device, void* stream, float* m_dev, int rows, int cols, int ld, int apply_log,
                           const float* log_priors_host, float prior_scale);

int eesen_op_gemm_bench(int device, int a_kc, int b_kc, int M, int N, int K, const float* A, int lda,
                        const float* B, int ldb, float* C, int ldc, int iters, float* avg_ms);

int eesen_op_amax_rows_cols(int device, const float* m_dev, long rows, int cols, int ld, float* out_rows_dev, float* out_cols_dev);

#ifdef __cplusplus
}
#endif
#endif
```

Baseline: 1.012 million.

## Batch memsets into fill kernel, fuse weight transpose with amax, overlap affine grads

Replaces many small hipMemsetAsync calls (state borders, recurrence counters, milestones) with one batched multi-range fill kernel. The per-direction recurrent-weight transposes and the weight bound (amax) computation are merged into a single table-driven kernel. The affine weight-gradient GEMM and column sums move to the side stream, with events guarding reuse of the gradient buffers. Together these cut launch count and let gradient work overlap the recurrence, at the cost of extra event synchronisation and more complex buffer-hazard tracking.

Measured after the change: 1.021 million (median of 6 runs). About the same (+0.9%).

```diff
diff --git a/eesen_amd/_lib.py b/eesen_amd/_lib.py
--- a/eesen_amd/_lib.py
+++ b/eesen_amd/_lib.py
@@ -114,6 +114,8 @@
     "eesen_dev_copy": (_i, [_i, _vp, _vp, _l, _i]),
     "eesen_op_log_sub_prior": (_i, [_i, _vp, _vp, _i, _i, _i, _i, _vp, _f]),
     "eesen_op_amax_rows_cols": (_i, [_i, _vp, C.c_long, _i, _i, _vp, _vp]),
+    "eesen_op_fill_ranges": (_i, [_i, _vp, _vp, _vp, _vp, _i]),
+    "eesen_op_weights_derived": (_i, [_i, _i, _vp, _vp, _vp, _vp, _vp, _vp, _vp]),
     "eesen_op_gemm_bench": (_i, [_i, _i, _i, _i, _i, _i, _vp, _i, _vp, _i, _vp, _i, _i, _pf]),
     "eesen_op_gemm": (_i, [_i, _vp, _i, _i, _i, _i, _i, _f, _vp, _i, _vp, _i, _f, _vp, _i, _vp]),
     "eesen_op_gemm_async": (_i, [_i, _vp, _i, _i, _i, _i, _i, _vp, _i, _vp, _i, _vp, _i, _vp, C.c_long, _i]),
diff --git a/eesen_amd/csrc/capi.cpp b/eesen_amd/csrc/capi.cpp
--- a/eesen_amd/csrc/capi.cpp
+++ b/eesen_amd/csrc/capi.cpp
@@ -467,4 +467,49 @@
   });
 }
 
-}
+int eesen_op_fill_ranges(int device, void* stream, void* const* ptrs_dev, const long* dwords, const unsigned* values, int n) {
+  return guard([&] {
+    EESEN_REQUIRE(n >= 0, EESEN_ERR_INVALID, "negative range count");
+    if (n) { REQ_PTR(ptrs_dev); REQ_PTR(dwords); REQ_PTR(values); }
+    EESEN_HIP_CHECK(hipSetDevice(device));
+    hipStream_t st = reinterpret_cast<hipStream_t>(stream);
+    std::vector<FillRange> r((size_t)n);
+    for (int i = 0; i < n; ++i) {
+      EESEN_REQUIRE(dwords[i] >= 0 && dwords[i] <= 0x7fffffffL, EESEN_ERR_INVALID, "fill range length out of range");
+      r[i] = FillRange{ptrs_dev[i], (unsigned)dwords[i], values[i]};
+    }
+    fill_ranges(st, r.data(), n);
+    EESEN_HIP_CHECK(hipStreamSynchronize(st));
+  });
+}
+
+int eesen_op_weights_derived(int device, int n, const int* kinds, const float* const* mats_dev, const int* rows, const int* cols, const int* lds,
+                             float* const* out_a_dev, float* const* out_b_dev) {
+  return guard([&] {
+    EESEN_REQUIRE(n > 0, EESEN_ERR_INVALID, "no matrices");
+    REQ_PTR(kinds); REQ_PTR(mats_dev); REQ_PTR(rows); REQ_PTR(cols); REQ_PTR(lds); REQ_PTR(out_a_dev); REQ_PTR(out_b_dev);
+    EESEN_HIP_CHECK(hipSetDevice(device));
+    std::vector<DeriveDesc> tab((size_t)n);
+    std::vector<FillRange> zero;
+    for (int i = 0; i < n; ++i) {
+      EESEN_REQUIRE(mats_dev[i] && out_a_dev[i] && out_b_dev[i], EESEN_ERR_INVALID, "null matrix or output");
+      if (kinds[i] == 0) {
+        tab[i] = DeriveDesc{mats_dev[i], out_a_dev[i], nullptr, nullptr, reinterpret_cast<unsigned*>(out_b_dev[i]), rows[i], cols[i], lds[i], kDeriveTranspose, 0, 0};
+        zero.push_back(FillRange{out_b_dev[i], 1u, 0u});
+      } else {
+        tab[i] = DeriveDesc{mats_dev[i], nullptr, reinterpret_cast<unsigned*>(out_a_dev[i]), reinterpret_cast<unsigned*>(out_b_dev[i]), nullptr, rows[i], cols[i], lds[i], kDeriveBounds, 0, 0};
+        zero.push_back(FillRange{out_a_dev[i], (unsigned)std::max(0, rows[i]), 0u});
+        zero.push_back(FillRange{out_b_dev[i], (unsigned)std::max(0, cols[i]), 0u});
+      }
+    }
+    const int blocks = derive_layout(tab.data(), n);
+    DevBuf<DeriveDesc> dev;
+    dev.reserve((size_t)n);
+    EESEN_HIP_CHECK(hipMemcpy(dev.p, tab.data(), tab.size() * sizeof(DeriveDesc), hipMemcpyHostToDevice));
+    fill_ranges(nullptr, zero.data(), (int)zero.size());
+    weights_derived(nullptr, dev.p, n, blocks);
+    EESEN_HIP_CHECK(hipStreamSynchronize(nullptr));
+  });
+}
+
+}
diff --git a/eesen_amd/csrc/gemm.hip b/eesen_amd/csrc/gemm.hip
--- a/eesen_amd/csrc/gemm.hip
+++ b/eesen_amd/csrc/gemm.hip
@@ -791,15 +791,19 @@
   }
   check_launch("amax_abs");
 }
-void amax_rows_cols(hipStream_t st, const float* P, long rows, int cols, int ld, float* out_rows, float* out_cols, float* ws) {
+bool amax_rows_need_zero(int cols, int ld) {
+  const bool vec = (cols & 3) == 0 && (ld & 3) == 0;
+  return (vec && cols > 1024) || cols > kAmaxSlabCols;
+}
+void amax_rows_cols(hipStream_t st, const float* P, long rows, int cols, int ld, float* out_rows, float* out_cols, float* ws, bool rows_zeroed) {
   if (rows <= 0 || cols <= 0) return;
   EESEN_REQUIRE(!out_cols || ws, EESEN_ERR_INVALID, "amax: column bounds need a workspace");
   unsigned* r = reinterpret_cast<unsigned*>(out_rows);
   unsigned* w = reinterpret_cast<unsigned*>(ws);
   unsigned* a = nullptr;
   const bool vec = (cols & 3) == 0 && (ld & 3) == 0;
-  const bool multi = out_rows && ((vec && cols > 1024) || cols > kAmaxSlabCols);
-  if (multi) EESEN_HIP_CHECK(hipMemsetAsync(out_rows, 0, (size_t)rows * sizeof(float), st));
+  const bool multi = out_rows && amax_rows_need_zero(cols, ld);
+  if (multi && !rows_zeroed) EESEN_HIP_CHECK(hipMemsetAsync(out_rows, 0, (size_t)rows * sizeof(float), st));
   for (int c0 = 0; c0 < cols; c0 += kAmaxSlabCols) {
     const float* Pc = P + c0;
     const int cc = std::min(kAmaxSlabCols, cols - c0), racc = multi ? 1 : 0;
diff --git a/eesen_amd/csrc/kernels.h b/eesen_amd/csrc/kernels.h
--- a/eesen_amd/csrc/kernels.h
+++ b/eesen_amd/csrc/kernels.h
@@ -19,7 +19,9 @@
 void amax_abs(hipStream_t st, const float* P, long rows, int cols, int ld, float* out);
 void amax_abs_accumulate(hipStream_t st, const float* P, long rows, int cols, int ld, float* out);
 constexpr int kAmaxBlocks = 512;
-void amax_rows_cols(hipStream_t st, const float* P, long rows, int cols, int ld, float* out_rows, float* out_cols, float* ws);
+void amax_rows_cols(hipStream_t st, const float* P, long rows, int cols, int ld, float* out_rows, float* out_cols, float* ws,
+                    bool rows_zeroed = false);
+bool amax_rows_need_zero(int cols, int ld);
 
 #ifndef EESEN_SHARDS
 #define EESEN_SHARDS 8
@@ -36,6 +38,27 @@
 };
 void gemm_f32_nt_gated(hipStream_t st, int M, int N, int K, const float* A, int lda, const float* B, int ldb, float* C,
                        int ldc, const float* bias, const GemmGate& gate, GemmBound bound_a = {}, GemmBound bound_b = {});
+
+struct FillRange {
+  void* p;
+  unsigned dwords;
+  unsigned value;
+};
+constexpr int kFillMaxRanges = 24;
+void fill_ranges(hipStream_t st, const FillRange* ranges, int n);
+
+enum { kDeriveTranspose = 0, kDeriveBounds = 1 };
+struct DeriveDesc {
+  const float* src;
+  float* dst_t;
+  unsigned* out_rows;
+  unsigned* out_cols;
+  unsigned* out_all;
+  int rows, cols, ld, kind;
+  int first_block, blocks_c;
+};
+int derive_layout(DeriveDesc* d, int n);
+void weights_derived(hipStream_t st, const DeriveDesc* table_dev, int n, int blocks);
 
 struct LstmLayerDev {
   int T, S, H, ndir;
@@ -104,9 +127,11 @@
 RecPlan lstm_fwd_plan(const LstmLayerDev& L);
 RecPlan lstm_bwd_plan(const LstmLayerDev& L);
 void lstm_fwd_launch(hipStream_t st, const RecPlan& plan, const LstmLayerDev& L, unsigned* cnt, unsigned* err, int spin_limit,
-                     unsigned long long* trace = nullptr, hipEvent_t after_reset = nullptr);
+                     unsigned long long* trace = nullptr, hipEvent_t after_reset = nullptr, const FillRange* with_reset = nullptr,
+                     int n_with_reset = 0);
 void lstm_bwd_launch(hipStream_t st, const RecPlan& plan, const LstmLayerDev& L, const float* dY, int lddy, float* DG, unsigned* cnt,
-                     unsigned* err, int spin_limit, unsigned long long* trace = nullptr);
+                     unsigned* err, int spin_limit, unsigned long long* trace = nullptr, const FillRange* with_reset = nullptr,
+                     int n_with_reset = 0);
 void lstm_bias_peep_grads(hipStream_t st, const LstmLayerDev& L, const float* DG, float* bias_grad, float* peep_grad,
                           float* ws, size_t ws_floats);
 size_t lstm_bias_peep_ws_floats(int T, int S, int H, int ndir);
@@ -141,7 +166,6 @@
                      const float* live = nullptr);
 void tensor_moments(hipStream_t st, const float* base, long rows, int cols, long ld, double* out6, double* ws,
                     int nb = 0, int hf = 0, int hi = 0);
-void transpose2d(hipStream_t st, const float* src, int rows, int cols, float* dst);
 void copy2d(hipStream_t st, const float* src, int lds, float* dst, int ldd, int rows, int cols);
 
 }
diff --git a/eesen_amd/csrc/net.cpp b/eesen_amd/csrc/net.cpp
--- a/eesen_amd/csrc/net.cpp
+++ b/eesen_amd/csrc/net.cpp
@@ -110,6 +110,7 @@
   EESEN_HIP_CHECK(hipStreamCreateWithPriority(&st2, hipStreamNonBlocking, lo));
   EESEN_HIP_CHECK(hipEventCreateWithFlags(&ev_rec, hipEventDisableTiming));
   for (auto& e : ev_grad) EESEN_HIP_CHECK(hipEventCreateWithFlags(&e, hipEventDisableTiming));
+  for (auto& e : ev_aff) EESEN_HIP_CHECK(hipEventCreateWithFlags(&e, hipEventDisableTiming));
   EESEN_HIP_CHECK(hipEventCreateWithFlags(&ev_gate_reset, hipEventDisableTiming));
   EESEN_HIP_CHECK(hipEventCreateWithFlags(&ev_gate_done, hipEventDisableTiming));
   tn = Tuning::from_env();
@@ -177,6 +178,7 @@
   if (st2) { (void)hipStreamSynchronize(st2); (void)hipStreamDestroy(st2); }
   if (ev_rec) (void)hipEventDestroy(ev_rec);
   for (auto& e : ev_grad) if (e) (void)hipEventDestroy(e);
+  for (auto& e : ev_aff) if (e) (void)hipEventDestroy(e);
   if (ev_gate_reset) (void)hipEventDestroy(ev_gate_reset);
   if (ev_gate_done) (void)hipEventDestroy(ev_gate_done);
   for (auto& e : ev_ready) if (e) (void)hipEventDestroy(e);
@@ -322,16 +324,41 @@
   amax.reserve(1 + layers.size());
   EESEN_HIP_CHECK(hipMemsetAsync(amax.p, 0, amax.cap * sizeof(float), st));
   EESEN_HIP_CHECK(hipMemsetD32Async(reinterpret_cast<hipDeviceptr_t>(amax.p), 0x3f800000, 1, st));
+  std::vector<DeriveDesc> tab;
+  derive_zero.assign(1, FillRange{am_wm(0), (unsigned)layers.size(), 0u});
+  for (size_t li = 0; li < layers.size(); ++li)
+    if (Layer& L = layers[li]; L.is_lstm())
+      for (int dir = 0; dir < L.ndir; ++dir)
+        tab.push_back(DeriveDesc{params.p + L.p_off + L.off_wm + (size_t)dir * 4 * L.H * L.H, L.WmT.p + (size_t)dir * L.H * 4 * L.H, nullptr, nullptr,
+                                 reinterpret_cast<unsigned*>(am_wm((int)li)), 4 * L.H, L.H, L.H, kDeriveTranspose, 0, 0});
+  derive_n_wm = (int)tab.size();
+  for (Layer& L : layers) {
+    if (!L.is_lstm() && L.kind != EESEN_LAYER_AFFINE) continue;
+    const int nrows = L.is_lstm() ? L.ndir * 4 * L.H : L.dout, D4 = pad4(L.din);
+    L.bw.rows.reserve((size_t)nrows);
+    L.bw.cols.reserve((size_t)D4);
+    tab.push_back(DeriveDesc{params.p + L.p_off + (L.is_lstm() ? L.off_wx : L.off_w), nullptr, reinterpret_cast<unsigned*>(L.bw.rows.p),
+                             reinterpret_cast<unsigned*>(L.bw.cols.p), nullptr, nrows, D4, D4, kDeriveBounds, 0, 0});
+    derive_zero.push_back(FillRange{L.bw.rows.p, (unsigned)nrows, 0u});
+    derive_zero.push_back(FillRange{L.bw.cols.p, (unsigned)D4, 0u});
+  }
+  derive_n = (int)tab.size();
+  derive_blocks = derive_layout(tab.data(), derive_n);
+  derive_blocks_wm = derive_n_wm < derive_n ? tab[derive_n_wm].first_block : derive_blocks;
+  if (derive_n) {
+    derive_tab.reserve((size_t)derive_n);
+    EESEN_HIP_CHECK(hipMemcpy(derive_tab.p, tab.data(), tab.size() * sizeof(DeriveDesc), hipMemcpyHostToDevice));
+  }
   finalized = true;
   refresh_derived();
   sync();
 }
 
-void Net::measure(const float* Pm, long nrows, int cols, int ld, DevBuf<float>& out_rows, DevBuf<float>& out_cols) {
+void Net::measure(const float* Pm, long nrows, int cols, int ld, DevBuf<float>& out_rows, DevBuf<float>& out_cols, bool rows_zeroed) {
   out_rows.reserve((size_t)nrows);
   out_cols.reserve((size_t)cols);
   amax_ws.reserve((size_t)kAmaxBlocks * std::min(16384, (cols + 3) & ~3));
-  amax_rows_cols(st, Pm, nrows, cols, ld, out_rows.p, out_cols.p, amax_ws.p);
+  amax_rows_cols(st, Pm, nrows, cols, ld, out_rows.p, out_cols.p, amax_ws.p, rows_zeroed);
 }
 bool Net::x_is_bounded(int li) const {
   if (li == 0) return false;
@@ -369,11 +396,12 @@
 
 void Net::refresh_derived() {
   wamax_valid = wm_valid = false;
-  for (Layer& L : layers)
-    if (L.is_lstm())
-      for (int dir = 0; dir < L.ndir; ++dir)
-        transpose2d(st, params.p + L.p_off + L.off_wm + (size_t)dir * 4 * L.H * L.H, 4 * L.H, L.H,
-                    L.WmT.p + (size_t)dir * L.H * 4 * L.H);
+  if (!derive_n) return;
+  const bool half = gemm_mode() == 2;
+  fill_ranges(st, derive_zero.data(), half ? (int)derive_zero.size() : 1);
+  weights_derived(st, derive_tab.p, half ? derive_n : derive_n_wm, half ? derive_blocks : derive_blocks_wm);
+  wm_valid = true;
+  wamax_valid = half;
 }
 
 int Net::tensor_moments(int which, int layer, double* out6_host, int cap_tensors) {
@@ -649,6 +677,20 @@
   const bool half = gemm_mode() == 2;
   ensure_weight_amax();
   amx_valid = half;
+  {
+    std::vector<FillRange> zero;
+    for (Layer& L : layers) {
+      if (!L.is_lstm()) continue;
+      const int H = L.H, nd = L.ndir, ldY = nd * H;
+      const size_t state = (size_t)(T + 2) * S * ldY, blk = (size_t)S * ldY;
+      L.C.reserve(state);
+      L.Y.reserve(state);
+      if (persistent && H % 32 == 0) L.X.reserve((size_t)T * nd * ((S + 15) / 16) * (size_t)(H / 32) * 768);
+      for (float* base : {L.C.p, L.Y.p})
+        for (size_t at : {(size_t)0, (size_t)(T + 1) * S * ldY}) zero.push_back(FillRange{base + at, (unsigned)blk, 0u});
+    }
+    fill_ranges(st, zero.data(), (int)zero.size());
+  }
   for (Layer& L : layers) {
     const int li_ = (int)(&L - layers.data());
     GemmBound x_amax, w_amax;
@@ -660,15 +702,6 @@
     if (L.is_lstm()) {
       const int H = L.H, nd = L.ndir, ldY = nd * H, ldG = nd * 4 * H;
       L.G.reserve((size_t)rows * ldG);
-      const size_t state = (size_t)(T + 2) * S * ldY;
-      L.C.reserve(state);
-      L.Y.reserve(state);
-      if (persistent && H % 32 == 0) L.X.reserve((size_t)T * nd * ((S + 15) / 16) * (size_t)(H / 32) * 768);
-      const size_t blk = (size_t)S * ldY * sizeof(float);
-      EESEN_HIP_CHECK(hipMemsetAsync(L.C.p, 0, blk, st));
-      EESEN_HIP_CHECK(hipMemsetAsync(L.Y.p, 0, blk, st));
-      EESEN_HIP_CHECK(hipMemsetAsync(L.C.p + (size_t)(T + 1) * S * ldY, 0, blk, st));
-      EESEN_HIP_CHECK(hipMemsetAsync(L.Y.p + (size_t)(T + 1) * S * ldY, 0, blk, st));
       prepare_dropout(*this, L);
       if (g_gated) {
         if (gated_rows < rows) {
@@ -708,14 +741,14 @@
       { const int ti_ = timer.begin(st, 1);
       v.poll_delay = delay_fwd;
       v.poll_raw = poll_raw;
+      FillRange mile_reset{nullptr, 0u, 0u};
       if (plan_mid) {
         mile.reserve(32);
-        EESEN_HIP_CHECK(hipMemsetAsync(mile.p, 0, 2 * sizeof(unsigned), st));
-        EESEN_HIP_CHECK(hipEventRecord(ev_gate_reset, st));
+        mile_reset = FillRange{mile.p, 2u, 0u};
         v.milestone = mile.p;
         v.milestone_step = mile_step;
       }
-      if (pers) lstm_fwd_launch(st, fp, v, ctl.p, ctl.p + kCtlWords - 1, spin_limit, trace.p, plan_gate ? ev_gate_reset : nullptr);
+      if (pers) lstm_fwd_launch(st, fp, v, ctl.p, ctl.p + kCtlWords - 1, spin_limit, trace.p, plan_gate || plan_mid ? ev_gate_reset : nullptr, &mile_reset, plan_mid ? 1 : 0);
       else
         for (int step = 0; step < T; ++step) lstm_fwd_step(st, v, step);
       info_fwd_persistent += pers ? 1 : 0;
@@ -838,6 +871,11 @@
   ws2.reserve(need_ws);
   int dg_slot = 0;
   bool side_pending[2] = {false, false};
+  bool aff_pending[2] = {false, false};
+  auto before_write = [&](const float* buf) {
+    const int k = buf == dA.p ? 0 : 1;
+    if (aff_pending[k]) { EESEN_HIP_CHECK(hipStreamWaitEvent(st, ev_aff[k], 0)); aff_pending[k] = false; }
+  };
   deferred_buckets.clear();
   const std::vector<RecPlan> bwd = bwd_plans(T);
   const bool overlap = overlap_for_minibatch(bwd);
@@ -892,15 +930,31 @@
       { const int ti_ = timer.begin(st, 4);
       if (half) measure(d, rows, L.dout, ld_d, L.bd.rows, L.bd.cols);
       if (want_in) {
+        before_write(dn);
         if (ld_n != L.din) EESEN_HIP_CHECK(hipMemsetAsync(dn, 0, (size_t)rows * ld_n * sizeof(float), st));
         gemm_f32(st, true, false, rows, L.din, L.dout, 1.f, d, ld_d, params.p + L.p_off + L.off_w, pad4(L.din), 0.f, dn, ld_n,
                  nullptr, nullptr, 0, 0, false, half ? GemmBound{L.bd.rows.p, 1} : GemmBound{}, half ? GemmBound{L.bw.cols.p, 1} : GemmBound{});
       }
-      gemm_f32(st, false, false, L.dout, L.din, rows, 1.f, d, ld_d, x, ldx, 0.f, fr + L.off_w, pad4(L.din), nullptr, ws.p, ws_floats, 0, false,
+      timer.end(st, ti_); }
+      bool lstm_below = false;
+      for (int lj = 0; lj < li; ++lj) lstm_below |= layers[lj].is_lstm();
+      hipStream_t sg = overlap ? st2 : st;
+      const int side_lds = overlap && lstm_below ? (tn.side_lds_kb >= 0 ? tn.side_lds_kb : (gemm_mode() >= 1 ? 48 : 32)) * 1024 : 0;
+      if (overlap) {
+        EESEN_HIP_CHECK(hipEventRecord(ev_rec, st));
+        EESEN_HIP_CHECK(hipStreamWaitEvent(st2, ev_rec, 0));
+      }
+      { const int ti_ = timer.begin(sg, 4);
+      gemm_f32(sg, false, false, L.dout, L.din, rows, 1.f, d, ld_d, x, ldx, 0.f, fr + L.off_w, pad4(L.din), nullptr, overlap ? ws2.p : ws.p, ws_floats, side_lds, false,
                half ? GemmBound{L.bd.cols.p, 1} : GemmBound{}, x_cols(li));
-      col_sums(st, d, rows, L.dout, ld_d, fr + L.off_b, ws.p, ws_floats);
-      timer.end(st, ti_); }
-      bucket_allreduce(li, st);
+      col_sums(sg, d, rows, L.dout, ld_d, fr + L.off_b, overlap ? ws2.p : ws.p, ws_floats);
+      timer.end(sg, ti_); }
+      bucket_allreduce(li, sg);
+      if (overlap) {
+        const int k = d == dA.p ? 0 : 1;
+        EESEN_HIP_CHECK(hipEventRecord(ev_aff[k], st2));
+        aff_pending[k] = true;
+      }
     } else {
       const int H = L.H, nd = L.ndir, ldG = nd * 4 * H, ldY = nd * H;
       LstmLayerDev v = lstm_view(*this, L, T);
@@ -921,17 +975,21 @@
         EESEN_HIP_CHECK(hipStreamWaitEvent(st, ev_grad[dg_slot], 0));
         side_pending[dg_slot] = false;
       }
+      const bool pre_zero = half && bp.kind != kRecNone && amax_rows_need_zero(ldG, ldG);
+      FillRange bd_zero{nullptr, 0u, 0u};
+      if (pre_zero) { L.bd.rows.reserve((size_t)rows); bd_zero = FillRange{L.bd.rows.p, (unsigned)rows, 0u}; }
       { const int ti_ = timer.begin(st, 3);
       if (bp.kind != kRecNone) {
-        lstm_bwd_launch(st, bp, v, d, ld_d, DGl, ctl.p + kCtlHalf, ctl.p + kCtlWords - 1, spin_limit, trace.p ? trace.p + 640 : nullptr);
+        lstm_bwd_launch(st, bp, v, d, ld_d, DGl, ctl.p + kCtlHalf, ctl.p + kCtlWords - 1, spin_limit, trace.p ? trace.p + 640 : nullptr, &bd_zero, pre_zero ? 1 : 0);
         ++info_bwd_persistent;
       } else
         for (int step = 0; step < T; ++step) lstm_bwd_step(st, v, step, d, ld_d, DGl, DCF.p);
       check_launch("lstm_bwd");
       timer.end(st, ti_); }
-      if (half) { const int ti_ = timer.begin(st, 4); measure(DGl, rows, ldG, ldG, L.bd.rows, L.bd.cols); timer.end(st, ti_); }
+      if (half) { const int ti_ = timer.begin(st, 4); measure(DGl, rows, ldG, ldG, L.bd.rows, L.bd.cols, pre_zero); timer.end(st, ti_); }
       EESEN_HIP_CHECK(hipEventRecord(ev_rec, st));
       if (want_in) {
+        before_write(dn);
         const int ti_ = timer.begin(st, 4);
         if (ld_n != L.din) EESEN_HIP_CHECK(hipMemsetAsync(dn, 0, (size_t)rows * ld_n * sizeof(float), st));
         gemm_f32(st, true, false, rows, L.din, ldG, 1.f, DGl, ldG, params.p + L.p_off + L.off_wx, pad4(L.din), 0.f, dn, ld_n,
@@ -945,16 +1003,30 @@
       for (int lj = 0; lj < li; ++lj) lstm_below |= layers[lj].is_lstm();
       const int side_lds = overlap && lstm_below ? side_lds_env : 0;
       if (overlap) EESEN_HIP_CHECK(hipStreamWaitEvent(st2, ev_rec, 0));
+      const bool tail = overlap && !lstm_below;
+      auto wx_grad = [&] {
+        gemm_f32(sg, false, false, ldG, L.din, rows, 1.f, DGl, ldG, x, ldx, 0.f, fr + L.off_wx, pad4(L.din), nullptr, ws2.p, need_ws, side_lds, false,
+                 half ? GemmBound{L.bd.cols.p, 1} : GemmBound{}, x_cols(li));
+      };
       { const int ti_ = timer.begin(sg, 4);
-      gemm_f32(sg, false, false, ldG, L.din, rows, 1.f, DGl, ldG, x, ldx, 0.f, fr + L.off_wx, pad4(L.din), nullptr, ws2.p, need_ws, side_lds, false,
-               half ? GemmBound{L.bd.cols.p, 1} : GemmBound{}, x_cols(li));
+      if (!tail) wx_grad();
       for (int dir = 0; dir < nd; ++dir)
         gemm_f32(sg, false, false, 4 * H, H, rows, 1.f, DGl + (size_t)dir * 4 * H, ldG,
                  L.Y.p + (size_t)(dir == 0 ? 0 : 2 * S) * ldY + (size_t)dir * H, ldY, 0.f,
                  fr + L.off_wm + (size_t)dir * 4 * H * H, H, nullptr, ws2.p, need_ws, side_lds, false,
                  half ? GemmBound{L.bd.cols.p + (size_t)dir * 4 * H, 1} : GemmBound{}, half ? bound_one() : GemmBound{});
-      lstm_bias_peep_grads(sg, v, DGl, fr + L.off_bias, fr + L.off_peep, ws2.p, need_ws);
+      if (tail) wx_grad();
+      else lstm_bias_peep_grads(sg, v, DGl, fr + L.off_bias, fr + L.off_peep, ws2.p, need_ws);
       timer.end(sg, ti_); }
+      if (tail) {
+        const int ti_ = timer.begin(st, 4);
+        lstm_bias_peep_grads(st, v, DGl, fr + L.off_bias, fr + L.off_peep, ws.p, need_ws);
+        timer.end(st, ti_);
+        if (comm) {
+          EESEN_HIP_CHECK(hipEventRecord(ev_rec, st));
+          EESEN_HIP_CHECK(hipStreamWaitEvent(st2, ev_rec, 0));
+        }
+      }
       bucket_allreduce(li, sg);
       if (overlap) {
         EESEN_HIP_CHECK(hipEventRecord(ev_grad[dg_slot], st2));
@@ -969,8 +1041,10 @@
   }
   if (in_diff) copy2d(st, d, ld_d, in_diff, ldi, rows, layers[0].din);
   flush_deferred_buckets();
-  for (int k = 0; k < 2; ++k)
+  for (int k = 0; k < 2; ++k) {
     if (side_pending[k]) EESEN_HIP_CHECK(hipStreamWaitEvent(st, ev_grad[k], 0));
+    if (aff_pending[k]) EESEN_HIP_CHECK(hipStreamWaitEvent(st, ev_aff[k], 0));
+  }
 }
 
 std::vector<RecPlan> Net::bwd_plans(int T) const {
diff --git a/eesen_amd/csrc/net.h b/eesen_amd/csrc/net.h
--- a/eesen_amd/csrc/net.h
+++ b/eesen_amd/csrc/net.h
@@ -97,6 +97,7 @@
   DevBuf<float> bwd_dgh, bwd_ex;
   hipStream_t st2 = nullptr;
   hipEvent_t ev_rec = nullptr, ev_grad[2] = {nullptr, nullptr};
+  hipEvent_t ev_aff[2] = {nullptr, nullptr};
   bool overlap = true;
   hipEvent_t ev_gate_reset = nullptr, ev_gate_done = nullptr;
   DevBuf<unsigned> mile;
@@ -136,8 +137,11 @@
   float* am_wm(int li) { return amax.p + 1 + li; }
   GemmBound bound_one() const { return GemmBound{amax.p, 0}; }
   bool x_is_bounded(int li) const;
-  void measure(const float* P, long rows, int cols, int ld, DevBuf<float>& out_rows, DevBuf<float>& out_cols);
+  void measure(const float* P, long rows, int cols, int ld, DevBuf<float>& out_rows, DevBuf<float>& out_cols, bool rows_zeroed = false);
   void ensure_weight_amax();
+  DevBuf<DeriveDesc> derive_tab;
+  int derive_n = 0, derive_n_wm = 0, derive_blocks = 0, derive_blocks_wm = 0;
+  std::vector<FillRange> derive_zero;
   PhaseTimer timer;
   Comm* comm = nullptr;
   std::vector<hipEvent_t> ev_ready, ev_bucket;
diff --git a/eesen_amd/csrc/optim.hip b/eesen_amd/csrc/optim.hip
--- a/eesen_amd/csrc/optim.hip
+++ b/eesen_amd/csrc/optim.hip
@@ -59,21 +59,115 @@
   for (long i = (long)blockIdx.x * blockDim.x + threadIdx.x; i < n; i += stride) p[i] = 0.f;
 }
 
-__global__ __launch_bounds__(256) void transpose2d_kernel(const float* __restrict__ src, int rows, int cols,
-                                                          float* __restrict__ dst) {
-  __shared__ float tile[32][33];
-  const int tx = threadIdx.x & 31, ty = threadIdx.x >> 5;
-  const int c0 = blockIdx.x * 32, r0 = blockIdx.y * 32;
-#pragma unroll
-  for (int i = 0; i < 32; i += 8) {
-    const int r = r0 + ty + i, c = c0 + tx;
-    if (r < rows && c < cols) tile[ty + i][tx] = src[(size_t)r * cols + c];
-  }
-  __syncthreads();
-#pragma unroll
-  for (int i = 0; i < 32; i += 8) {
-    const int c = c0 + ty + i, r = r0 + tx;
-    if (r < rows && c < cols) dst[(size_t)c * rows + r] = tile[tx][ty + i];
+struct FillTable {
+  FillRange r[kFillMaxRanges];
+};
+__global__ __launch_bounds__(256) void fill_ranges_kernel(FillTable t) {
+  const FillRange r = t.r[blockIdx.y];
+  unsigned* p = static_cast<unsigned*>(r.p);
+  const unsigned n = r.dwords, v = r.value;
+  const unsigned tid = blockIdx.x * 256u + threadIdx.x, nt = gridDim.x * 256u;
+  const unsigned head = min(n, (unsigned)((16u - (unsigned)(reinterpret_cast<size_t>(p) & 15u)) & 15u) >> 2);
+  const unsigned nq = (n - head) >> 2, tail = head + (nq << 2);
+  if (tid < head) p[tid] = v;
+  uint4* q = reinterpret_cast<uint4*>(p + head);
+  const uint4 v4 = make_uint4(v, v, v, v);
+  for (unsigned i = tid; i < nq; i += nt) q[i] = v4;
+  if (tid < n - tail) p[tail + tid] = v;
+}
+
+__device__ __forceinline__ uint4 load_quad_or_zero(const float* p, bool in_range) {
+  uint4 v = make_uint4(0u, 0u, 0u, 0u);
+  if (in_range) v = *reinterpret_cast<const uint4*>(p);
+  return v;
+}
+__device__ __forceinline__ unsigned max4(const uint4& a) { return max(max(a.x, a.y), max(a.z, a.w)); }
+__device__ __forceinline__ void maxq(uint4& a, const uint4& b) { a.x = max(a.x, b.x); a.y = max(a.y, b.y); a.z = max(a.z, b.z); a.w = max(a.w, b.w); }
+__global__ __launch_bounds__(256) void weights_derived_kernel(const DeriveDesc* __restrict__ tab, int n) {
+  __shared__ unsigned tile[64][65];
+  __shared__ unsigned red[4][64];
+  int di = 0;
+  while (di + 1 < n && (int)blockIdx.x >= tab[di + 1].first_block) ++di;
+  const DeriveDesc d = tab[di];
+  const int b = (int)blockIdx.x - d.first_block;
+  const int R0 = (b / d.blocks_c) * 128, C0 = (b % d.blocks_c) * 128;
+  const int tid = threadIdx.x, tx = tid & 15, ty = tid >> 4, lane = tid & 63, wave = tid >> 6;
+  if (d.kind == kDeriveBounds) {
+    uint4 cm0 = make_uint4(0u, 0u, 0u, 0u), cm1 = cm0;
+#pragma unroll
+    for (int sr = 0; sr < 2; ++sr) {
+      unsigned rm[4] = {0u, 0u, 0u, 0u};
+#pragma unroll
+      for (int sc = 0; sc < 2; ++sc) {
+        const int c = C0 + sc * 64 + tx * 4;
+#pragma unroll
+        for (int i = 0; i < 4; ++i) {
+          const int r = R0 + sr * 64 + ty + 16 * i;
+          uint4 v = load_quad_or_zero(d.src + (size_t)r * d.ld + c, r < d.rows && c < d.cols);
+          v.x &= 0x7fffffffu; v.y &= 0x7fffffffu; v.z &= 0x7fffffffu; v.w &= 0x7fffffffu;
+          rm[i] = max(rm[i], max4(v));
+          if (sc == 0) maxq(cm0, v); else maxq(cm1, v);
+        }
+      }
+#pragma unroll
+      for (int i = 0; i < 4; ++i) {
+        unsigned m = rm[i];
+#pragma unroll
+        for (int o = 8; o > 0; o >>= 1) m = max(m, (unsigned)__shfl_xor((int)m, o));
+        const int r = R0 + sr * 64 + ty + 16 * i;
+        if (tx == 0 && r < d.rows && m) atomicMax(&d.out_rows[r], m);
+      }
+    }
+    auto fold_cols = [&](uint4 m, int sc) {
+      m.x = max(m.x, (unsigned)__shfl_xor((int)m.x, 16)); m.y = max(m.y, (unsigned)__shfl_xor((int)m.y, 16));
+      m.z = max(m.z, (unsigned)__shfl_xor((int)m.z, 16)); m.w = max(m.w, (unsigned)__shfl_xor((int)m.w, 16));
+      m.x = max(m.x, (unsigned)__shfl_xor((int)m.x, 32)); m.y = max(m.y, (unsigned)__shfl_xor((int)m.y, 32));
+      m.z = max(m.z, (unsigned)__shfl_xor((int)m.z, 32)); m.w = max(m.w, (unsigned)__shfl_xor((int)m.w, 32));
+      __syncthreads();
+      if (lane < 16) { red[wave][tx * 4 + 0] = m.x; red[wave][tx * 4 + 1] = m.y; red[wave][tx * 4 + 2] = m.z; red[wave][tx * 4 + 3] = m.w; }
+      __syncthreads();
+      if (tid < 64) {
+        const unsigned mm = max(max(red[0][tid], red[1][tid]), max(red[2][tid], red[3][tid]));
+        const int c = C0 + sc * 64 + tid;
+        if (c < d.cols && mm) atomicMax(&d.out_cols[c], mm);
+      }
+    };
+    fold_cols(cm0, 0);
+    fold_cols(cm1, 1);
+  } else {
+    unsigned all = 0u;
+#pragma unroll 1
+    for (int s = 0; s < 4; ++s) {
+      const int r0 = R0 + (s >> 1) * 64, c0 = C0 + (s & 1) * 64;
+      if (r0 >= d.rows || c0 >= d.cols) continue;
+      __syncthreads();
+#pragma unroll
+      for (int i = 0; i < 4; ++i) {
+        const int r = r0 + ty + 16 * i, c = c0 + tx * 4;
+        uint4 v = load_quad_or_zero(d.src + (size_t)r * d.ld + c, r < d.rows && c < d.cols);
+        tile[ty + 16 * i][tx * 4 + 0] = v.x; tile[ty + 16 * i][tx * 4 + 1] = v.y; tile[ty + 16 * i][tx * 4 + 2] = v.z; tile[ty + 16 * i][tx * 4 + 3] = v.w;
+        v.x &= 0x7fffffffu; v.y &= 0x7fffffffu; v.z &= 0x7fffffffu; v.w &= 0x7fffffffu;
+        all = max(all, max4(v));
+      }
+      __syncthreads();
+#pragma unroll
+      for (int i = 0; i < 4; ++i) {
+        const int cc = ty + 16 * i, c = c0 + cc, r = r0 + tx * 4;
+        if (c < d.cols && r < d.rows)
+          *reinterpret_cast<uint4*>(d.dst_t + (size_t)c * d.rows + r) = make_uint4(tile[tx * 4 + 0][cc], tile[tx * 4 + 1][cc], tile[tx * 4 + 2][cc], tile[tx * 4 + 3][cc]);
+      }
+    }
+    if (d.out_all) {
+#pragma unroll
+      for (int o = 32; o > 0; o >>= 1) all = max(all, (unsigned)__shfl_xor((int)all, o));
+      __syncthreads();
+      if (lane == 0) red[0][wave] = all;
+      __syncthreads();
+      if (tid == 0) {
+        const unsigned m = max(max(red[0][0], red[0][1]), max(red[0][2], red[0][3]));
+        if (m) atomicMax(d.out_all, m);
+      }
+    }
   }
 }
 
@@ -111,9 +205,50 @@
   check_launch("adaptive_update");
 }
 
-void transpose2d(hipStream_t st, const float* src, int rows, int cols, float* dst) {
-  hipLaunchKernelGGL(transpose2d_kernel, dim3(cdiv(cols, 32), cdiv(rows, 32)), dim3(256), 0, st, src, rows, cols, dst);
-  check_launch("transpose2d");
+void fill_ranges(hipStream_t st, const FillRange* ranges, int n) {
+  FillTable t;
+  int k = 0;
+  unsigned most = 0;
+  auto flush = [&] {
+    if (!k) return;
+    const unsigned bx = std::min(64u, std::max(1u, (most + 4095u) / 4096u));
+    for (int i = k; i < kFillMaxRanges; ++i) t.r[i] = FillRange{nullptr, 0u, 0u};
+    hipLaunchKernelGGL(fill_ranges_kernel, dim3(bx, k), dim3(256), 0, st, t);
+    check_launch("fill_ranges");
+    k = 0;
+    most = 0;
+  };
+  for (int i = 0; i < n; ++i) {
+    if (!ranges[i].dwords) continue;
+    EESEN_REQUIRE(ranges[i].p && (reinterpret_cast<size_t>(ranges[i].p) & 3) == 0, EESEN_ERR_INVALID, "fill_ranges: a range needs a 4-byte aligned address");
+    t.r[k++] = ranges[i];
+    most = std::max(most, ranges[i].dwords);
+    if (k == kFillMaxRanges) flush();
+  }
+  flush();
+}
+
+int derive_layout(DeriveDesc* d, int n) {
+  int blocks = 0;
+  for (int i = 0; i < n; ++i) {
+    EESEN_REQUIRE(d[i].rows > 0 && d[i].cols > 0 && d[i].cols % 4 == 0 && d[i].ld % 4 == 0 && d[i].ld >= d[i].cols &&
+                      (reinterpret_cast<size_t>(d[i].src) & 15) == 0,
+                  EESEN_ERR_INVALID, "derived weight data: rows of whole, aligned 16-byte words only");
+    if (d[i].kind == kDeriveTranspose)
+      EESEN_REQUIRE(d[i].dst_t && d[i].rows % 4 == 0 && (reinterpret_cast<size_t>(d[i].dst_t) & 15) == 0, EESEN_ERR_INVALID, "derived weight data: bad transpose target");
+    else
+      EESEN_REQUIRE(d[i].kind == kDeriveBounds && d[i].out_rows && d[i].out_cols, EESEN_ERR_INVALID, "derived weight data: bounds need both outputs");
+    d[i].first_block = blocks;
+    d[i].blocks_c = cdiv(d[i].cols, 128);
+    blocks += d[i].blocks_c * cdiv(d[i].rows, 128);
+  }
+  return blocks;
+}
+
+void weights_derived(hipStream_t st, const DeriveDesc* table_dev, int n, int blocks) {
+  if (n <= 0 || blocks <= 0) return;
+  hipLaunchKernelGGL(weights_derived_kernel, dim3(blocks), dim3(256), 0, st, table_dev, n);
+  check_launch("weights_derived");
 }
 
 void copy2d(hipStream_t st, const float* src, int lds, float* dst, int ldd, int rows, int cols) {
diff --git a/eesen_amd/csrc/rec_plan.cpp b/eesen_amd/csrc/rec_plan.cpp
--- a/eesen_amd/csrc/rec_plan.cpp
+++ b/eesen_amd/csrc/rec_plan.cpp
@@ -4,6 +4,7 @@
 #include <map>
 #include <mutex>
 #include <tuple>
+#include <vector>
 
 namespace eesen {
 namespace {
@@ -258,8 +259,16 @@
   return P;
 }
 
+static void reset_counters(hipStream_t st, unsigned* cnt, size_t words, const FillRange* more, int n_more) {
+  std::vector<FillRange> r;
+  r.reserve(1 + (size_t)n_more);
+  r.push_back(FillRange{cnt, (unsigned)words, 0u});
+  for (int i = 0; i < n_more; ++i) r.push_back(more[i]);
+  fill_ranges(st, r.data(), (int)r.size());
+}
+
 void lstm_fwd_launch(hipStream_t st, const RecPlan& P, const LstmLayerDev& L0, unsigned* cnt, unsigned* err, int spin_limit,
-                     unsigned long long* trace, hipEvent_t after_reset) {
+                     unsigned long long* trace, hipEvent_t after_reset, const FillRange* with_reset, int n_with_reset) {
   EESEN_REQUIRE(P.kind == kRecFwdBf || P.kind == kRecFwdMux || P.kind == kRecFwdF32, EESEN_ERR_STATE, "not a forward recurrence plan");
   const RecRole role{P.grid[0], P.grid[1], P.grid[2], L0.xcd_map};
   for (int w = 0; w < P.windows; ++w) {
@@ -267,7 +276,7 @@
     if (P.kind == kRecFwdMux) { L.s_begin = 0; L.s_count = 0; }
     else { L.s_count = L0.S / P.windows; L.s_begin = w * L.s_count; }
     if (P.kind != kRecFwdMux && P.wgs_per_cu >= 2 && !L0.poll_raw) L.poll_delay = L0.poll_delay * 7 / 4;
-    EESEN_HIP_CHECK(hipMemsetAsync(cnt, 0, sizeof(unsigned) * P.ctl_words, st));
+    reset_counters(st, cnt, P.ctl_words, w == 0 ? with_reset : nullptr, w == 0 ? n_with_reset : 0);
     if (after_reset && P.one_window) EESEN_HIP_CHECK(hipEventRecord(after_reset, st));
     if (P.kind == kRecFwdMux) plan_launch(st, P.fn, P.wgs, L, cnt, err, spin_limit, role);
     else plan_launch(st, P.fn, P.wgs, L, cnt, err, spin_limit, trace, role);
@@ -348,7 +357,7 @@
 }
 
 void lstm_bwd_launch(hipStream_t st, const RecPlan& P, const LstmLayerDev& L0, const float* dY, int lddy, float* DG, unsigned* cnt,
-                     unsigned* err, int spin_limit, unsigned long long* trace) {
+                     unsigned* err, int spin_limit, unsigned long long* trace, const FillRange* with_reset, int n_with_reset) {
   EESEN_REQUIRE(P.kind == kRecBwdQ4 || P.kind == kRecBwdKsplit || P.kind == kRecBwdKsplitMux || P.kind == kRecBwdGeneric, EESEN_ERR_STATE, "not a backward recurrence plan");
   EESEN_REQUIRE(!P.need_px || (L0.PX && L0.px_floats >= P.need_px), EESEN_ERR_STATE, "the backward plan's partial-sum exchange space (RecPlan::need_px) was not handed over");
   EESEN_REQUIRE(!P.need_dgh || (L0.DGH && L0.EX), EESEN_ERR_STATE, "the backward plan's plane and exponent buffers (RecPlan::need_dgh, need_ex) were not handed over");
@@ -360,7 +369,7 @@
     LstmLayerDev L = L0;
     if (whole_batch) { L.s_begin = 0; L.s_count = 0; }
     else { L.s_count = L0.S / P.windows; L.s_begin = w * L.s_count; }
-    EESEN_HIP_CHECK(hipMemsetAsync(cnt, 0, sizeof(unsigned) * P.ctl_words, st));
+    reset_counters(st, cnt, P.ctl_words, w == 0 ? with_reset : nullptr, w == 0 ? n_with_reset : 0);
     if (P.need_px) EESEN_HIP_CHECK(hipMemsetAsync(L.PX, 0, sizeof(float) * P.need_px, st));
     if (P.kind == kRecBwdQ4) plan_launch(st, P.fn, P.wgs, L, dY, lddy, DG, cnt, err, spin_limit, trace, role);
     else if (P.kind == kRecBwdKsplitMux) plan_launch(st, P.fn, P.wgs, L, dY, lddy, DG, px, cnt, err, spin_limit, role, chunk);
diff --git a/include/eesen_hip.h b/include/eesen_hip.h
--- a/include/eesen_hip.h
+++ b/include/eesen_hip.h
@@ -167,6 +167,11 @@
 
 int eesen_op_amax_rows_cols(int device, const float* m_dev, long rows, int cols, int ld, float* out_rows_dev, float* out_cols_dev);
 
+int eesen_op_fill_ranges(int device, void* stream, void* const* ptrs_dev, const long* dwords, const unsigned* values, int n);
+
+int eesen_op_weights_derived(int device, int n, const int* kinds, const float* const* mats_dev, const int* rows, const int* cols, const int* lds,
+                             float* const* out_a_dev, float* const* out_b_dev);
+
 #ifdef __cplusplus
 }
 #endif
```
